# agent-charon/MinGraph-UNet

Hardware: AMD Instinct MI355X
Metric: segmented Mpix/sec, full MinGraph-UNet forward (U-Net + patch-graph GAT), 512x512 batch (higher is better)
Workload: dtype f32

## Files before the change

### mingraph-unet_amd/csrc/asm/gen_wino_cp.py

```python
#!/usr/bin/env python3
import sys

def vr(b, n=1):
    return f"v{b}" if n == 1 else f"v[{b}:{b + n - 1}]"

CFG = {"ntb": 2, "nc": None}
def NTB(): return CFG["ntb"]
def ACC(jj, nt, mi): return ((jj * 2 + nt) * 2 + mi) * 16 if CFG["ntb"] == 2 else (jj * 2 + mi) * 16
def WN(c, jj, p): return 64 + ((c * 2 + jj) * 3 + p) * 4
def HSET(setn, i): return (232 if setn == 0 else 160) + i * 4
def BX(jj, nt, p): return 128 + ((jj * 2 + nt) * 3 + p) * 4
def PC(slot, p): return 176 + (slot * 3 + p) * 4
def RAW(hf, k): return 200 + (hf * 4 + k) * 4
def HREG(i): return 232 + i * 4
VA, VB = 244, 245
VHST = [246, 247, 248]
VHOFF = [249, 250, 251]
VLANE16 = 252
VTID = 253
VT0, VT1 = 230, 231
def VMASK(): return 254 if CFG["ntb"] == 2 else 172
def VSGN(): return 255 if CFG["ntb"] == 2 else 173

S_IN, S_WU, S_OUT, S_SCALE, S_SHIFT, S_POOL = 4, 6, 8, 10, 12, 14
S_H, S_W, S_LDIN, S_LDOUT, S_LDPOOL, S_NC, S_RELU, S_TX, S_TY, S_TOTAL, S_PPB, S_NGROUPS = 16, 17, 18, 19, 20, 21, 22, 23, 24, 25, 26, 27
S_NITEMS, S_PERXCD, S_MGNG, S_MGTX, S_MGTXTY, S_PAD = 28, 29, 30, 31, 32, 33
S_NBLOCK, S_PBEGIN, S_NPATCH, S_LC, S_LP, S_PI, S_C, S_LC64 = 34, 35, 36, 37, 38, 39, 40, 41
S_N64X4 = 42
S_SUMOFF = 43
S_INR = 44
S_UR = 48
S_SGN, S_W1, S_MASK, S_PERM, S_NTSTRIDE, S_TXTY, S_IMGB, S_OOB = 52, 53, 54, 55, 56, 57, 58, 59
S_T = [60, 61, 62, 63, 64, 65, 66, 67]
S_WI, S_JP = 68, 69
S_P, S_IMG, S_REM, S_PY, S_PX, S_Y0, S_X0 = 70, 71, 72, 73, 74, 75, 72
S_X0 = 88
S_M = 76
S_WO = [[78, 79], [90, 91]]
S_OUTR = 80
S_POOLR = 84
S_OUTIMGB = 89
S_SCR = 92
S_SHR = 96
S_LD4, S_SW4 = 100, 101

S1F, S2F, S3F = 17 * 20, 20, 17 * 20 + 20
BUFX = 0x20000
RAWB = 8192 * 4
ZBIAS = 57472

out = []
def E(s=""): out.append("\t" + s if s and not s.endswith(":") else s)
def L(s): out.append(s + ":")
_lbl = [0]
def newlabel(p="L"):
    _lbl[0] += 1
    return f".{p}_{_lbl[0]}"


def divmod_magic(n, d, mg, q, r, t0, t1):
    E(f"s_mul_hi_u32 s{q}, s{n}, s{mg}")
    E(f"s_mul_i32 s{t0}, s{q}, s{d}")
    E(f"s_sub_u32 s{r}, s{n}, s{t0}")
    E(f"s_add_u32 s{t0}, s{q}, 1")
    E(f"s_sub_u32 s{t1}, s{r}, s{d}")
    E(f"s_cmp_ge_u32 s{r}, s{d}")
    E(f"s_cselect_b32 s{q}, s{t0}, s{q}")
    E(f"s_cselect_b32 s{r}, s{t1}, s{r}")


def patch_coords(p):
    divmod_magic(p, S_TXTY, S_MGTXTY, S_IMG, S_REM, S_T[6], S_T[7])
    divmod_magic(S_REM, S_TX, S_MGTX, S_PY, S_PX, S_T[6], S_T[7])
    E(f"s_lshl_b32 s{S_Y0}, s{S_PY}, 3")
    E(f"s_lshl_b32 s{S_X0}, s{S_PX}, 5")


S_VHST = S_PAD


def setup_load():
    E(f"s_add_u32 s{S_P}, s{S_PBEGIN}, s{S_LP}")
    patch_coords(S_P)
    E(f"s_mul_i32 s{S_T[6]}, s{S_IMG}, s{S_IMGB}")
    E(f"s_mul_hi_u32 s{S_T[7]}, s{S_IMG}, s{S_IMGB}")
    E(f"s_add_u32 s{S_INR}, s{S_IN}, s{S_T[6]}")
    E(f"s_addc_u32 s{S_INR + 1}, s{S_IN + 1}, s{S_T[7]}")
    ledge, lvalu, ldone = newlabel("edge"), newlabel("hofs"), newlabel("hdone")
    E(f"s_add_u32 s{S_M}, s{S_Y0}, 8")
    E(f"s_cmp_eq_u32 s{S_M}, s{S_H}")
    E(f"s_cselect_b32 s{S_M + 1}, 1, 0")
    E(f"s_cmp_eq_u32 s{S_Y0}, 0")
    E(f"s_cselect_b32 s{S_M + 1}, 1, s{S_M + 1}")
    E(f"s_add_u32 s{S_M}, s{S_X0}, 32")
    E(f"s_cmp_eq_u32 s{S_M}, s{S_W}")
    E(f"s_cselect_b32 s{S_M + 1}, 1, s{S_M + 1}")
    E(f"s_cmp_eq_u32 s{S_X0}, 0")
    E(f"s_cselect_b32 s{S_M + 1}, 1, s{S_M + 1}")
    E(f"s_sub_u32 s{S_T[6]}, s{S_Y0}, 1")
    E(f"s_sub_u32 s{S_T[7]}, s{S_X0}, 1")
    E(f"s_cmp_lg_u32 s{S_M + 1}, 0")
    E(f"s_cbranch_scc1 {ledge}")
    E(f"s_mul_i32 s{S_M}, s{S_T[6]}, s{S_W}")
    E(f"s_add_u32 s{S_M}, s{S_M}, s{S_T[7]}")
    E(f"s_mul_i32 s{S_M}, s{S_M}, s{S_LDIN}")
    E(f"s_lshl_b32 s{S_M}, s{S_M}, 2")
    E(f"s_add_u32 s{S_INR}, s{S_INR}, s{S_M}")
    E(f"s_addc_u32 s{S_INR + 1}, s{S_INR + 1}, 0")
    E(f"s_and_b32 s{S_INR + 1}, s{S_INR + 1}, 0xffff")
    E(f"s_cmp_eq_u32 s{S_VHST}, 1")
    E(f"s_cbranch_scc1 {ldone}")
    E(f"s_mov_b32 s{S_T[6]}, 0")
    E(f"s_mov_b32 s{S_T[7]}, 0")
    E(f"s_mov_b32 s{S_VHST}, 1")
    E(f"s_branch {lvalu}")
    L(ledge)
    E(f"s_and_b32 s{S_INR + 1}, s{S_INR + 1}, 0xffff")
    E(f"s_mov_b32 s{S_VHST}, 0")
    L(lvalu)
    for i in range(3):
        d = VHOFF[i]
        E(f"v_lshrrev_b32_e32 v{VT0}, 2, v{VTID}")
        if i:
            E(f"v_add_u32_e32 v{VT0}, {128 * i}, v{VT0}")
        E(f"v_mul_u32_u24_e32 v{VT1}, 0x788, v{VT0}")
        E(f"v_lshrrev_b32_e32 v{VT1}, 16, v{VT1}")
        E(f"v_mul_u32_u24_e32 v{d}, 34, v{VT1}")
        E(f"v_sub_u32_e32 v{d}, v{VT0}, v{d}")
        E(f"v_cmp_gt_u32_e32 vcc, 0x154, v{VT0}")
        E(f"v_add_u32_e32 v{VT1}, s{S_T[6]}, v{VT1}")
        E(f"v_add_u32_e32 v{d}, s{S_T[7]}, v{d}")
        E(f"v_cmp_gt_u32_e64 s[{S_M}:{S_M + 1}], s{S_H}, v{VT1}")
        E(f"s_and_b64 vcc, vcc, s[{S_M}:{S_M + 1}]")
        E(f"v_cmp_gt_u32_e64 s[{S_M}:{S_M + 1}], s{S_W}, v{d}")
        E(f"s_and_b64 vcc, vcc, s[{S_M}:{S_M + 1}]")
        E(f"v_mad_u32_u24 v{VT1}, v{VT1}, s{S_W}, v{d}")
        E(f"v_mul_lo_u32 v{VT1}, v{VT1}, s{S_LDIN}")
        E(f"v_and_b32_e32 v{VT0}, 3, v{VTID}")
        E(f"v_lshl_add_u32 v{VT1}, v{VT0}, 2, v{VT1}")
        E(f"v_lshlrev_b32_e32 v{VT1}, 2, v{VT1}")
        E(f"v_mov_b32_e32 v{d}, s{S_OOB}")
        E("s_nop 1")
        E(f"v_cndmask_b32_e32 v{d}, v{d}, v{VT1}, vcc")
    L(ldone)


def halo_loads(setn=0):
    for i in range(3):
        E(f"buffer_load_dwordx4 {vr(HSET(setn, i), 4)}, v{VHOFF[i]}, s[{S_INR}:{S_INR + 3}], s{S_LC64} offen")
    E(f"s_add_u32 s{S_LC}, s{S_LC}, 1")
    E(f"s_cmp_eq_u32 s{S_LC}, s{S_NC}")
    E(f"s_cselect_b32 s{S_LC}, 0, s{S_LC}")
    E(f"s_cmp_eq_u32 s{S_LC}, 0")
    E(f"s_addc_u32 s{S_LP}, s{S_LP}, 0")
    E(f"s_lshl_b32 s{S_LC64}, s{S_LC}, 6")


def halo_stores(setn=0):
    for i in range(3):
# ... 318 lines not shown
            E(f"v_max_f32_e32 v{Z(0, 0, 1) + e}, v{ya1 + e}, v{yb1 + e}")
        for e in range(4):
            E(f"v_max_f32_e32 v{pm + e}, v{pm + e}, v{Z(0, 0, 1) + e}")
        E(f"buffer_store_dwordx4 {vr(pm, 4)}, v{VPOOL}, s[{S_POOLR}:{S_POOLR + 3}], 0 offen offset:{nt * 128}")
        L(lnp)
        E("s_waitcnt lgkmcnt(0)")
        E("s_barrier")


def mfmas_n(jj, mi, slot, c):
    acc = vr(ACC(jj, 0, mi), 16)
    return [f"v_mfma_f32_32x32x16_bf16 {acc}, {vr(PC(slot, pa), 4)}, {vr(WN(c, jj, pb), 4)}, {'0' if (c == 0 and k == 0) else acc}"
            for k, (pa, pb) in enumerate(((2, 0), (0, 2), (1, 1), (1, 0), (0, 1), (0, 0)))]


def emit_step_n(jp, s, c):
    jj, mi = step_jm(s)
    slot = s & 1
    n1, n2 = (s + 1) & 3, (s + 2) & 3
    if s == 2:
        E("s_waitcnt lgkmcnt(0)")
        E("s_barrier")
    E("s_nop 1")
    mf = mfmas_n(jj, mi, slot, c)
    v0 = form_valu(jp, step_jm(n1)[0], slot ^ 1, 0)
    v1 = form_valu(jp, step_jm(n1)[0], slot ^ 1, 1)
    r1 = raw_reads(jp, *step_jm(n1), 1)
    r2 = raw_reads(jp, *step_jm(n2), 0)
    per0, per1 = -(-len(v0) // 2), -(-len(v1) // 3)
    extra = {}
    if s == 0:
        hs = (c + 1) & 1
        E("s_waitcnt vmcnt(3)")
        for i in range(3):
            extra.setdefault(i, []).append(f"ds_write_b128 v{VHST[i]}, {vr(HSET(hs, i), 4)}")
        extra.setdefault(3, []).extend([f"v_xor_b32_e32 v{VHST[i]}, 0x{BUFX:x}, v{VHST[i]}" for i in range(3)])
        for i in range(3):
            extra.setdefault(3 + i, []).append(f"buffer_load_dwordx4 {vr(HSET(hs, i), 4)}, v{VHOFF[i]}, s[{S_INR}:{S_INR + 3}], s{S_LC64} offen")
        extra.setdefault(5, []).extend([
            f"s_add_u32 s{S_LC}, s{S_LC}, 1", f"s_cmp_eq_u32 s{S_LC}, s{S_NC}", f"s_cselect_b32 s{S_LC}, 0, s{S_LC}",
            f"s_cmp_eq_u32 s{S_LC}, 0", f"s_addc_u32 s{S_LP}, s{S_LP}, 0", f"s_lshl_b32 s{S_LC64}, s{S_LC}, 6"])
    def take(lst, n):
        for _ in range(min(n, len(lst))):
            E(lst.pop(0))
    nlds = 0
    for k in range(6):
        E(mf[k])
        for x in extra.get(k, []):
            E(x)
            nlds += x.startswith("ds_")
        if k in (0, 1):
            nlds += min(2, len(r1))
            take(r1, 2)
        if k == 1:
            E(f"s_waitcnt lgkmcnt({nlds})")
        if k in (1, 2):
            take(v0, per0)
        if k == 3:
            E("s_waitcnt lgkmcnt(0)")
            if s == 2:
                E(f"v_xor_b32_e32 v{VA}, 0x{BUFX:x}, v{VA}")
                E(f"v_xor_b32_e32 v{VB}, 0x{BUFX:x}, v{VB}")
        if k in (3, 4):
            take(r2, 2)
        if k >= 3:
            take(v1, per1)
    assert not v0 and not v1 and not r1 and not r2


def emit_chunk_n(jp, c):
    lskip = newlabel("nosetup")
    E(f"s_cmp_lg_u32 s{S_LC}, 0")
    E(f"s_cbranch_scc1 {lskip}")
    E(f"s_cmp_ge_u32 s{S_LP}, s{S_NPATCH}")
    E(f"s_cbranch_scc1 {lskip}")
    setup_load()
    L(lskip)
    E("s_waitcnt lgkmcnt(0)")
    E("s_barrier")
    for s in range(4):
        emit_step_n(jp, s, c)


def emit_epilogue_n(jp):
    CQ, VT = 228, 229
    VZ0, VZ1, VOUT, VPOOL = 188, 189, 190, 191
    e0, e1, e2, e3 = 192, 193, 194, 195
    SC4, SH4 = 196, 212
    TMP = [216 + i for i in range(8)]
    E("s_nop 7")
    E("s_nop 7")
    E("s_nop 7")
    E(f"s_add_u32 s{S_P}, s{S_PBEGIN}, s{S_PI}")
    patch_coords(S_P)
    E(f"s_mul_i32 s{S_T[6]}, s{S_IMG}, s{S_OUTIMGB}")
    E(f"s_mul_hi_u32 s{S_T[7]}, s{S_IMG}, s{S_OUTIMGB}")
    E(f"s_add_u32 s{S_OUTR}, s{S_OUT}, s{S_T[6]}")
    E(f"s_addc_u32 s{S_OUTR + 1}, s{S_OUT + 1}, s{S_T[7]}")
    E(f"s_and_b32 s{S_OUTR + 1}, s{S_OUTR + 1}, 0xffff")
    E(f"s_lshr_b32 s{S_T[4]}, s{S_H}, 1")
    E(f"s_lshr_b32 s{S_T[5]}, s{S_W}, 1")
    E(f"s_mul_i32 s{S_T[4]}, s{S_T[4]}, s{S_T[5]}")
    E(f"s_mul_i32 s{S_T[4]}, s{S_T[4]}, s{S_LDPOOL}")
    E(f"s_lshl_b32 s{S_T[4]}, s{S_T[4]}, 2")
    E(f"s_mov_b32 s{S_POOLR + 2}, s{S_T[4]}")
    E(f"s_mul_i32 s{S_T[6]}, s{S_IMG}, s{S_T[4]}")
    E(f"s_mul_hi_u32 s{S_T[7]}, s{S_IMG}, s{S_T[4]}")
    E(f"s_add_u32 s{S_POOLR}, s{S_POOL}, s{S_T[6]}")
    E(f"s_addc_u32 s{S_POOLR + 1}, s{S_POOL + 1}, s{S_T[7]}")
    E(f"s_and_b32 s{S_POOLR + 1}, s{S_POOLR + 1}, 0xffff")
    E(f"v_and_b32_e32 v{CQ}, 7, v{VTID}")
    E(f"v_lshrrev_b32_e32 v{VT}, 3, v{VTID}")
    E(f"v_lshlrev_b32_e32 v{e0}, 4, v{CQ}")
    for (ptr, rs, reg, dflt) in ((S_SCALE, S_SCR, SC4, "1.0"), (S_SHIFT, S_SHR, SH4, "0")):
        ln, ldn = newlabel("nul"), newlabel("nud")
        E(f"s_cmp_eq_u64 s[{ptr}:{ptr + 1}], 0")
        E(f"s_cbranch_scc1 {ln}")
        E(f"buffer_load_dwordx4 {vr(reg, 4)}, v{e0}, s[{rs}:{rs + 3}], s{S_N64X4} offen")
        E(f"s_branch {ldn}")
        L(ln)
        for e in range(4):
            E(f"v_mov_b32_e32 v{reg + e}, {dflt}")
        L(ldn)
    E(f"v_and_b32_e32 v{e0}, 32, v{VT}")
    E(f"v_and_b32_e32 v{e1}, 3, v{VT}")
    E(f"v_bfe_u32 v{e2}, v{VT}, 3, 2")
    E(f"v_lshl_add_u32 v{e1}, v{e2}, 2, v{e1}")
    E(f"v_lshl_add_u32 v{e0}, v{e1}, 1, v{e0}")
    E(f"v_bfe_u32 v{e2}, v{VT}, 2, 1")
    E(f"v_add_u32_e32 v{e0}, v{e0}, v{e2}")
    E(f"v_lshlrev_b32_e32 v{e0}, 7, v{e0}")
    E(f"v_lshl_add_u32 v{VZ0}, v{CQ}, 4, v{e0}")
    E(f"v_add_u32_e32 v{VZ1}, 0x10000, v{VZ0}")
    E(f"v_lshrrev_b32_e32 v{e1}, 4, v{VT}")
    E(f"v_lshl_add_u32 v{e1}, v{e1}, 1, s{S_Y0}")
    E(f"v_and_b32_e32 v{e2}, 15, v{VT}")
    E(f"v_lshl_add_u32 v{e2}, v{e2}, 1, s{S_X0}")
    E(f"v_mad_u32_u24 v{e3}, v{e1}, s{S_W}, v{e2}")
    E(f"v_mul_lo_u32 v{e3}, v{e3}, s{S_LDOUT}")
    E(f"v_lshl_add_u32 v{e3}, v{CQ}, 2, v{e3}")
    E(f"v_lshlrev_b32_e32 v{VOUT}, 2, v{e3}")
    E(f"v_add_u32_e32 v{VOUT}, s{S_N64X4}, v{VOUT}")
    E(f"v_lshrrev_b32_e32 v{e1}, 1, v{e1}")
    E(f"v_lshrrev_b32_e32 v{e2}, 1, v{e2}")
    E(f"v_mad_u32_u24 v{e3}, v{e1}, s{S_T[5]}, v{e2}")
    E(f"v_mul_lo_u32 v{e3}, v{e3}, s{S_LDPOOL}")
    E(f"v_lshl_add_u32 v{e3}, v{CQ}, 2, v{e3}")
    E(f"v_lshlrev_b32_e32 v{VPOOL}, 2, v{e3}")
    E(f"v_add_u32_e32 v{VPOOL}, s{S_N64X4}, v{VPOOL}")
    E(f"s_lshl_b32 s{S_T[0]}, s{S_WI}, 13")
    if jp:
        E(f"s_add_u32 s{S_T[0]}, s{S_T[0]}, 0x{RAWB:x}")
    E(f"s_lshl_b32 s{S_T[1]}, s{S_WI}, 13")
    E(f"s_add_u32 s{S_T[1]}, s{S_T[1]}, 0x{(2 + jp) * RAWB - ZBIAS:x}")
    E("s_waitcnt lgkmcnt(0)")
    E("s_barrier")
    for q in range(2):
        E(f"s_mov_b32 m0, s{S_T[q]}")
        E("s_nop 0")
        g = 0
        for mi in range(2):
            for r0 in range(0, 16, 4):
                ts = TMP[(g & 1) * 4:(g & 1) * 4 + 4]
                g += 1
                src = []
                for k in (0, 2):
                    m0, m1 = ACC(0, 0, mi) + r0 + k, ACC(1, 0, mi) + r0 + k
                    if jp == 0 and q == 0:
                        E(pk2("add", ts[k], m0, m1))
                        src += [ts[k], ts[k] + 1]
                    elif jp == 0:
                        src += [m1, m1 + 1]
                    elif q == 0:
                        src += [m0, m0 + 1]
                    else:
                        E(pk2("add", ts[k], m0, m1, neg_a=True, neg_b=True))
                        src += [ts[k], ts[k] + 1]
                E("s_nop 0")
                for k in range(4):
                    off = (32 * mi + 2 * (r0 + k)) * 128 + (ZBIAS if q else 0)
                    E(f"ds_write_addtid_b32 v{src[k]} offset:{off}")
    E("s_waitcnt lgkmcnt(0)")
    E("s_barrier")
    zb = [ACC(0, 0, 0), ACC(0, 0, 1), ACC(1, 0, 0), ACC(1, 0, 1)]
    def Z(q, j, i):
        k = (q * 2 + j) * 4 + i
        return zb[k // 4] + (k % 4) * 4
    for q in range(2):
        for j in range(2):
            for i in range(4):
                E(f"ds_read_b128 {vr(Z(q, j, i), 4)}, v{VZ1 if q else VZ0} offset:{j * RAWB + i * 8192}")
    E("s_waitcnt vmcnt(0) lgkmcnt(8)")
    emit_finish_math(Z, 0, SC4, SH4)
    E("s_waitcnt lgkmcnt(0)")
    emit_finish_math(Z, 1, SC4, SH4)
    lnr = newlabel("norelu")
    E(f"s_cmp_eq_u32 s{S_RELU}, 0")
    E(f"s_cbranch_scc1 {lnr}")
    for q in range(2):
        for y in (Z(q, 1, 0), Z(q, 1, 1)):
            for e in range(4):
                E(f"v_max_f32_e32 v{y + e}, 0, v{y + e}")
    L(lnr)
    ya0, yb0, ya1, yb1 = Z(0, 1, 0), Z(0, 1, 1), Z(1, 1, 0), Z(1, 1, 1)
    E(f"buffer_store_dwordx4 {vr(ya0, 4)}, v{VOUT}, s[{S_OUTR}:{S_OUTR + 3}], 0 offen nt")
    E(f"buffer_store_dwordx4 {vr(ya1, 4)}, v{VOUT}, s[{S_OUTR}:{S_OUTR + 3}], s{S_LD4} offen nt")
    E(f"buffer_store_dwordx4 {vr(yb0, 4)}, v{VOUT}, s[{S_OUTR}:{S_OUTR + 3}], s{S_SW4} offen nt")
    E(f"buffer_store_dwordx4 {vr(yb1, 4)}, v{VOUT}, s[{S_OUTR}:{S_OUTR + 3}], s{S_SUMOFF} offen nt")
    lnp = newlabel("nopool")
    E(f"s_cmp_eq_u64 s[{S_POOL}:{S_POOL + 1}], 0")
    E(f"s_cbranch_scc1 {lnp}")
    pm = Z(0, 0, 0)
    for e in range(4):
        E(f"v_max_f32_e32 v{pm + e}, v{ya0 + e}, v{yb0 + e}")
    for e in range(4):
        E(f"v_max_f32_e32 v{Z(0, 0, 1) + e}, v{ya1 + e}, v{yb1 + e}")
    for e in range(4):
        E(f"v_max_f32_e32 v{pm + e}, v{pm + e}, v{Z(0, 0, 1) + e}")
    E(f"buffer_store_dwordx4 {vr(pm, 4)}, v{VPOOL}, s[{S_POOLR}:{S_POOLR + 3}], 0 offen")
    L(lnp)
    E("s_waitcnt lgkmcnt(0)")
    E("s_barrier")


def emit_patch_loop_n(jp):
    lp = newlabel("patch")
    L(lp)
    for c in range(CFG["nc"]):
        emit_chunk_n(jp, c)
    emit_epilogue_n(jp)
    E(f"s_add_u32 s{S_PI}, s{S_PI}, 1")
    E(f"s_cmp_lt_u32 s{S_PI}, s{S_NPATCH}")
    E(f"s_cbranch_scc1 {lp}")
    E(f"s_branch {END_LABEL}")


def emit_patch_loop(jp):
    lp, lc = newlabel("patch"), newlabel("chunk")
    L(lp)
    E(f"s_mov_b32 s{S_C}, 0")
    FIRST_CHUNK[0] = True
    emit_chunk(jp)
    FIRST_CHUNK[0] = False
    E(f"s_mov_b32 s{S_C}, 1")
    L(lc)
    emit_chunk(jp)
    E(f"s_add_u32 s{S_C}, s{S_C}, 1")
    E(f"s_cmp_lt_u32 s{S_C}, s{S_NC}")
    E(f"s_cbranch_scc1 {lc}")
    emit_epilogue(jp)
    E(f"s_add_u32 s{S_PI}, s{S_PI}, 1")
    E(f"s_cmp_lt_u32 s{S_PI}, s{S_NPATCH}")
    E(f"s_cbranch_scc1 {lp}")
    E(f"s_branch {END_LABEL}")


def emit_prologue():
    E("s_load_dwordx16 s[4:19], s[0:1], 0x0")
    E("s_load_dwordx8 s[20:27], s[0:1], 0x40")
    E("s_load_dwordx4 s[28:31], s[0:1], 0x60")
    E("s_load_dwordx2 s[32:33], s[0:1], 0x70")
    E(f"v_mov_b32_e32 v{VTID}, v0")
    E("s_waitcnt lgkmcnt(0)")
    t = S_T
    E(f"s_and_b32 s{t[0]}, s2, 7")
    E(f"s_mul_i32 s{t[0]}, s{t[0]}, s{S_PERXCD}")
    E(f"s_lshr_b32 s{t[1]}, s2, 3")
    E(f"s_add_u32 s{t[0]}, s{t[0]}, s{t[1]}")
    E(f"s_cmp_ge_u32 s{t[0]}, s{S_NITEMS}")
    E(f"s_cbranch_scc1 {END_LABEL}")
    divmod_magic(t[0], S_NGROUPS, S_MGNG, S_NBLOCK, t[1], t[2], t[3])
    E(f"s_mul_i32 s{S_PBEGIN}, s{t[1]}, s{S_PPB}")
    E(f"s_sub_i32 s{t[2]}, s{S_TOTAL}, s{S_PBEGIN}")
    E(f"s_min_i32 s{S_NPATCH}, s{S_PPB}, s{t[2]}")
    E(f"s_cmp_lt_i32 s{S_NPATCH}, 1")
    E(f"s_cbranch_scc1 {END_LABEL}")
    E(f"s_mov_b32 s{S_MASK}, 0xffff0000")
    E(f"s_mov_b32 s{S_PERM}, 0x07060302")
    E(f"s_mov_b32 s{S_OOB}, 0x7fff0000")
    E(f"s_mul_i32 s{S_TXTY}, s{S_TX}, s{S_TY}")
    E(f"s_mul_i32 s{S_IMGB}, s{S_H}, s{S_W}")
    E(f"s_mul_i32 s{S_OUTIMGB}, s{S_IMGB}, s{S_LDOUT}")
    E(f"s_lshl_b32 s{S_OUTIMGB}, s{S_OUTIMGB}, 2")
    E(f"s_mul_i32 s{S_IMGB}, s{S_IMGB}, s{S_LDIN}")
    E(f"s_lshl_b32 s{S_IMGB}, s{S_IMGB}, 2")
    E(f"s_mul_i32 s{S_NTSTRIDE}, s{S_NC}, 0xc000")
    E(f"s_lshl_b32 s{S_N64X4}, s{S_NBLOCK}, {8 if NTB() == 2 else 7}")
    E(f"s_lshl_b32 s{S_LD4}, s{S_LDOUT}, 2")
    E(f"s_mul_i32 s{S_SW4}, s{S_W}, s{S_LD4}")
    E(f"s_add_u32 s{S_SUMOFF}, s{S_SW4}, s{S_LD4}")
    E(f"s_mov_b32 s{S_INR + 2}, s{S_IMGB}")
    E(f"s_mov_b32 s{S_INR + 3}, 0x00020000")
    E(f"s_mov_b32 s{S_OUTR + 2}, s{S_OUTIMGB}")
    E(f"s_mov_b32 s{S_OUTR + 3}, 0x00020000")
    E(f"s_mov_b32 s{S_POOLR + 3}, 0x00020000")
    for (r, p) in ((S_SCR, S_SCALE), (S_SHR, S_SHIFT)):
        E(f"s_mov_b32 s{r}, s{p}")
        E(f"s_and_b32 s{r + 1}, s{p + 1}, 0xffff")
        E(f"s_mov_b32 s{r + 2}, 0x7ffffff0")
        E(f"s_mov_b32 s{r + 3}, 0x00020000")
    E(f"v_lshrrev_b32_e32 v0, 6, v{VTID}")
    E("s_nop 3")
    E("v_readfirstlane_b32 s60, v0")
    E("s_nop 3")
    E(f"s_and_b32 s{S_WI}, s60, 3")
    E(f"s_lshr_b32 s{S_JP}, s60, 2")
    E(f"s_lshl_b32 s61, s{S_WI}, 1")
    E("s_lshr_b32 s62, 0x64, s61")
    E("s_and_b32 s62, s62, 3")
    E("s_lshr_b32 s63, 0xda, s61")
    E("s_and_b32 s63, s63, 3")
    E(f"s_cmp_eq_u32 s{S_WI}, 1")
    E(f"s_cselect_b32 s{S_SGN}, 1.0, -1.0")
    E(f"s_lshl_b32 s64, s{S_NTSTRIDE}, {1 if NTB() == 2 else 0}")
    E(f"s_mul_i32 s65, s{S_NBLOCK}, s64")
    E(f"s_lshl_b32 s66, s{S_WI}, 2")
    E(f"s_lshl_b32 s67, s{S_JP}, 1")
    E("s_add_u32 s66, s66, s67")
    E("s_mul_i32 s66, s66, 0xc00")
    E("s_add_u32 s65, s65, s66")
    E(f"s_add_u32 s{S_UR}, s{S_WU}, s65")
    E(f"s_addc_u32 s{S_UR + 1}, s{S_WU + 1}, 0")
    E(f"s_and_b32 s{S_UR + 1}, s{S_UR + 1}, 0xffff")
    E(f"s_mov_b32 s{S_UR + 2}, s64")
    E(f"s_mov_b32 s{S_UR + 3}, 0x00020000")
    E(f"v_and_b32_e32 v1, 63, v{VTID}")
    E(f"v_lshlrev_b32_e32 v{VLANE16}, 4, v1")
    E("v_and_b32_e32 v2, 31, v1")
    E("v_lshrrev_b32_e32 v3, 5, v1")
    E("v_and_b32_e32 v4, 15, v2")
    E("v_lshrrev_b32_e32 v5, 4, v2")
    E("v_lshlrev_b32_e32 v5, 1, v5")
    E("v_mul_u32_u24_e32 v4, 0x50, v4")
    E("v_lshl_add_u32 v4, v3, 5, v4")
    for (dst, srow) in ((VA, 62), (VB, 63)):
        E(f"v_add_u32_e32 v6, s{srow}, v5")
        E("v_mul_u32_u24_e32 v6, 0xaa0, v6")
        E("v_add_u32_e32 v6, v6, v4")
        E(f"v_add_u32_e32 v{dst}, 0x{BUFX:x}, v6")
    for i in range(3):
        E(f"v_lshrrev_b32_e32 v1, 2, v{VTID}")
        if i:
            E(f"v_add_u32_e32 v1, {128 * i}, v1")
        E("v_mul_u32_u24_e32 v2, 0x788, v1")
        E("v_lshrrev_b32_e32 v2, 16, v2")
        E("v_mul_u32_u24_e32 v3, 34, v2")
        E("v_sub_u32_e32 v3, v1, v3")
        E("v_and_b32_e32 v4, 1, v3")
        E("v_lshl_add_u32 v4, v2, 1, v4")
        E("v_mul_u32_u24_e32 v4, 17, v4")
        E("v_lshrrev_b32_e32 v3, 1, v3")
        E("v_add_u32_e32 v4, v4, v3")
        E("v_mul_u32_u24_e32 v4, 0x50, v4")
        E(f"v_and_b32_e32 v5, 3, v{VTID}")
        E(f"v_lshl_add_u32 v{VHST[i]}, v5, 4, v4")
    E(f"v_mov_b32_e32 v{VMASK()}, s{S_MASK}")
    E(f"v_mov_b32_e32 v{VSGN()}, s{S_SGN}")
    E(f"s_mov_b32 s{S_LC}, 0")
    E(f"s_mov_b32 s{S_LP}, 0")
    E(f"s_mov_b32 s{S_PI}, 0")
    E(f"s_mov_b32 s{S_LC64}, 0")
    if NTB() == 1:
        for c in range(CFG["nc"]):
            for jj in range(2):
                E(f"s_mov_b32 s{S_WO[0][0]}, 0x{c * 0xc000 + jj * 0xc00:x}")
                for pp in range(3):
                    E(f"buffer_load_dwordx4 {vr(WN(c, jj, pp), 4)}, v{VLANE16}, s[{S_UR}:{S_UR + 3}], s{S_WO[0][0]} offen offset:{pp * 1024}")
        setup_load()
        halo_loads(0)
        for i in range(3):
            E(f"v_xor_b32_e32 v{VHST[i]}, 0x{BUFX:x}, v{VHST[i]}")
        E("s_waitcnt vmcnt(0)")
        halo_stores(0)
        for i in range(3):
            E(f"v_xor_b32_e32 v{VHST[i]}, 0x{BUFX:x}, v{VHST[i]}")
        for setn in (1, 0):
            lsk = newlabel("nosetup")
            E(f"s_cmp_lg_u32 s{S_LC}, 0")
            E(f"s_cbranch_scc1 {lsk}")
            E(f"s_cmp_ge_u32 s{S_LP}, s{S_NPATCH}")
            E(f"s_cbranch_scc1 {lsk}")
            setup_load()
            L(lsk)
            halo_loads(setn)
        E("s_waitcnt lgkmcnt(0)")
        E("s_barrier")
        return
    setup_load()
    halo_loads()
    for i in range(3):
        E(f"v_xor_b32_e32 v{VHST[i]}, 0x{BUFX:x}, v{VHST[i]}")
    E("s_waitcnt vmcnt(0)")
    halo_stores()
    for i in range(3):
        E(f"v_xor_b32_e32 v{VHST[i]}, 0x{BUFX:x}, v{VHST[i]}")
    lskip = newlabel("nosetup")
    E(f"s_cmp_lg_u32 s{S_LC}, 0")
    E(f"s_cbranch_scc1 {lskip}")
    E(f"s_cmp_ge_u32 s{S_LP}, s{S_NPATCH}")
    E(f"s_cbranch_scc1 {lskip}")
    setup_load()
    L(lskip)
    halo_loads()
    E(f"s_mov_b32 s{S_WO[0][0]}, 0")
    E(f"s_mov_b32 s{S_WO[0][1]}, s{S_NTSTRIDE}")
    E(f"s_mov_b32 s{S_WO[1][0]}, 0xc00")
    E(f"s_add_u32 s{S_WO[1][1]}, s{S_NTSTRIDE}, 0xc00")
    for jj in range(2):
        for nt in range(2):
            for p in range(3):
                E(weight_load(jj, nt, p))
    E("s_waitcnt lgkmcnt(0)")
    E("s_barrier")


def emit_first_form(jp):
    for r in raw_reads(jp, 0, 0, 0) + raw_reads(jp, 0, 0, 1):
        E(r)
    E("s_waitcnt lgkmcnt(0)")
    for hf in range(2):
        for x in form_valu(jp, 0, 0, hf):
            E(x)
    for r in raw_reads(jp, *step_jm(1), 0):
        E(r)


def emit_kernel(name):
    _lbl[0] += 1000
    end = f".Lend_{name}"
    jp1 = f".Ljp1_{name}"
    fe = f".Lfunc_end_{name}"
    hdr = f"""\t.text
\t.protected\t{name}
\t.globl\t{name}
\t.p2align\t8
\t.type\t{name},@function
{name}:"""
    out.append(hdr)
    global END_LABEL
    END_LABEL = end
    emit_prologue()
    E(f"s_cmp_lg_u32 s{S_JP}, 0")
    E(f"s_cbranch_scc1 {jp1}")
    emit_first_form(0)
    (emit_patch_loop if NTB() == 2 else emit_patch_loop_n)(0)
    L(jp1)
    emit_first_form(1)
    (emit_patch_loop if NTB() == 2 else emit_patch_loop_n)(1)
    L(end)
    E("s_endpgm")
    out.append(f"""\t.section\t.rodata,"a",@progbits
\t.p2align\t6, 0x0
\t.amdhsa_kernel {name}
\t\t.amdhsa_group_segment_fixed_size 163840
\t\t.amdhsa_private_segment_fixed_size 0
\t\t.amdhsa_kernarg_size 120
\t\t.amdhsa_user_sgpr_count 2
\t\t.amdhsa_user_sgpr_dispatch_ptr 0
\t\t.amdhsa_user_sgpr_queue_ptr 0
\t\t.amdhsa_user_sgpr_kernarg_segment_ptr 1
\t\t.amdhsa_user_sgpr_dispatch_id 0
\t\t.amdhsa_user_sgpr_kernarg_preload_length 0
\t\t.amdhsa_user_sgpr_kernarg_preload_offset 0
\t\t.amdhsa_user_sgpr_private_segment_size 0
\t\t.amdhsa_uses_dynamic_stack 0
\t\t.amdhsa_enable_private_segment 0
\t\t.amdhsa_system_sgpr_workgroup_id_x 1
\t\t.amdhsa_system_sgpr_workgroup_id_y 0
\t\t.amdhsa_system_sgpr_workgroup_id_z 0
\t\t.amdhsa_system_sgpr_workgroup_info 0
\t\t.amdhsa_system_vgpr_workitem_id 0
\t\t.amdhsa_next_free_vgpr 256
\t\t.amdhsa_next_free_sgpr 102
\t\t.amdhsa_accum_offset 256
\t\t.amdhsa_reserve_vcc 1
\t\t.amdhsa_float_round_mode_32 0
\t\t.amdhsa_float_round_mode_16_64 0
\t\t.amdhsa_float_denorm_mode_32 3
\t\t.amdhsa_float_denorm_mode_16_64 3
\t\t.amdhsa_dx10_clamp 1
\t\t.amdhsa_ieee_mode 1
\t\t.amdhsa_fp16_overflow 0
\t\t.amdhsa_tg_split 0
\t.end_amdhsa_kernel
\t.text
{fe}:
\t.size\t{name}, {fe}-{name}
""")
    META.append(f"""  - .agpr_count:     0
    .args:
      - .offset:         0
        .size:           120
        .value_kind:     by_value
    .group_segment_fixed_size: 163840
    .kernarg_segment_align: 8
    .kernarg_segment_size: 120
    .max_flat_workgroup_size: 512
    .name:           {name}
    .private_segment_fixed_size: 0
    .sgpr_count:     108
    .sgpr_spill_count: 0
    .symbol:         {name}.kd
    .uniform_work_group_size: 1
    .uses_dynamic_stack: false
    .vgpr_count:     256
    .vgpr_spill_count: 0
    .wavefront_size: 64""")


META = []
END_LABEL = ".Lend"


def main():
    path = sys.argv[1]
    out.append('\t.amdgcn_target "amdgcn-amd-amdhsa--gfx950"')
    CFG.update(ntb=2, nc=None)
    emit_kernel("mgu_wino_cp2_gfx950")
    for nc in (2, 4):
        CFG.update(ntb=1, nc=nc)
        emit_kernel(f"mgu_wino_cp1r{nc}_gfx950")
    out.append("\t.amdgpu_metadata\n---\namdhsa.kernels:")
    out.extend(META)
    out.append("""amdhsa.target:   amdgcn-amd-amdhsa--gfx950
amdhsa.version:
  - 1
  - 2
...

\t.end_amdgpu_metadata
""")
    with open(path, "w") as f:
        f.write("\n".join(out) + "\n")


if __name__ == "__main__":
    main()
```

### mingraph-unet_amd/csrc/asm/lint_wino_asm.py

```python
#!/usr/bin/env python3
import re
import sys


def regs(tok):
    tok = tok.strip().lstrip("-").strip("|")
    m = re.match(r"v\[(\d+):(\d+)\]$", tok)
    if m:
        return set(range(int(m.group(1)), int(m.group(2)) + 1))
    m = re.match(r"v(\d+)$", tok)
    return {int(m.group(1))} if m else set()


def parse(line):
    line = line.split(";")[0].strip()
    if not line or line.endswith(":") or line.startswith("."):
        return None
    parts = line.split(None, 1)
    op = parts[0]
    args = []
    if len(parts) > 1:
        a = re.split(r",\s*", parts[1])
        args = [x.split()[0] if x.split() else x for x in a]
    return op, args, line


def classify(op, args):
    if op.startswith("v_mfma"):
        return regs(args[0]), regs(args[1]) | regs(args[2]) | regs(args[3]), "mfma"
    if op.startswith("ds_read"):
        return regs(args[0]), regs(args[1]), "lds_load"
    if op.startswith("ds_write_addtid"):
        return set(), regs(args[0]), "lds_store_addtid"
    if op.startswith("ds_write"):
        s = set()
        for a in args:
            s |= regs(a)
        return set(), s, "lds_store"
    if op.startswith("buffer_load") or op.startswith("global_load"):
        return regs(args[0]), regs(args[1]), "vm_load"
    if op.startswith("buffer_store") or op.startswith("global_store"):
        return set(), regs(args[0]) | regs(args[1]), "vm_store"
    if op.startswith("v_readfirstlane"):
        return set(), regs(args[1]), "readlane"
    if op.startswith("v_cmp"):
        s = set()
        for a in args:
            s |= regs(a)
        return set(), s, "valu"
    if op.startswith("v_"):
        s = set()
        for a in args[1:]:
            s |= regs(a)
        return regs(args[0]), s, "valu"
    return set(), set(), "other"


def kernels(text):
    out, cur, name = {}, None, None
    for ln in text.split("\n"):
        m = re.match(r"^(mgu_\w+):\s*$", ln)
        if m:
            name, cur = m.group(1), []
            out[name] = cur
            continue
        if ln.startswith(".Lfunc_end"):
            cur = None
            continue
        if cur is not None:
            cur.append(ln)
    return out


def loop_bodies(lines):
    lab = {}
    for i, ln in enumerate(lines):
        m = re.match(r"^(\.\w+):", ln)
        if m:
            lab[m.group(1)] = i
    bodies = []
    for i, ln in enumerate(lines):
        m = re.match(r"\s*s_cbranch_scc1\s+(\.\w+)", ln)
        if m and m.group(1) in lab and lab[m.group(1)] < i:
            bodies.append((m.group(1), lines[lab[m.group(1)]:i]))
    return bodies


def replay(stream, errors, where, prime=()):
    vm, lg = [], []
    valu_age = {}
    mfma_age = {}
    prev = None
    m0_fresh = False
    held = {}
    writes = {}

    def age(n):
        for d in (valu_age, mfma_age):
            for r in list(d):
                d[r] += n
                if d[r] > 40:
                    del d[r]

    skip_to = None
    labels = {}
    for i, ln in enumerate(stream):
        m = re.match(r"^(\.\w+):", ln)
        if m:
            labels.setdefault(m.group(1), []).append(i)
    for i, ln in enumerate(stream):
        if skip_to is not None:
            if re.match(r"^" + re.escape(skip_to) + ":", ln):
                skip_to = None
            continue
        p = parse(ln)
        if p is None:
            continue
        op, args, text = p
        if op == "s_branch" and any(j > i for j in labels.get(args[0], [])):
            skip_to = args[0]
            continue
        if op == "s_nop":
            age(int(args[0]) + 1)
            prev = ("nop", set(), text)
            m0_fresh = False
            continue
        if op == "s_waitcnt":
            m = re.search(r"vmcnt\((\d+)\)", text)
            if m:
                del vm[:max(0, len(vm) - int(m.group(1)))]
            m = re.search(r"lgkmcnt\((\d+)\)", text)
            if m:
                del lg[:max(0, len(lg) - int(m.group(1)))]
            age(1)
            prev = ("wait", set(), text)
            continue
        dst, src, kind = classify(op, args)
        touched = dst | src
        for q, nm in ((vm, "buffer load"), (lg, "LDS read")):
            for (d, t) in q:
                if d & src:
                    errors.append(f"{where}: `{text}` reads v{sorted(d & src)[0]} while `{t}` ({nm}) is outstanding")
                if d & dst and kind not in ("vm_load", "lds_load"):
                    errors.append(f"{where}: `{text}` writes v{sorted(d & dst)[0]}, destination of outstanding `{t}`")
        if kind == "mfma":
            for r in src:
                if valu_age.get(r, 99) < 2:
                    errors.append(f"{where}: `{text}` reads v{r} {valu_age[r]} wait state(s) after a VALU write (2 required)")
        else:
            for r in touched if kind in ("valu", "lds_store", "lds_store_addtid", "vm_store", "readlane") else src:
                if r in src and mfma_age.get(r, 99) < 18:
                    errors.append(f"{where}: `{text}` reads MFMA result v{r} after {mfma_age[r]} wait states (18 required)")
        if kind == "valu" and prev and prev[0] in ("lds_store", "vm_store") and len(prev[1]) >= 4 and (dst & prev[1]):
            errors.append(f"{where}: `{text}` overwrites store data of the previous instruction `{prev[2]}`")
        if kind == "lds_store_addtid" and m0_fresh:
            errors.append(f"{where}: `{text}` directly behind the write of M0")
        if kind == "readlane" and any(valu_age.get(r, 99) < 1 for r in src):
            errors.append(f"{where}: `{text}` directly behind the VALU write of its source")
        if op in ("v_add_f32_e32", "v_sub_f32_e32"):
            hs = [held.get(r) for a in args[1:3] for r in sorted(regs(a))]
            if len(hs) == 2 and any(h and h[0] == "sum" for h in hs):
                if hs[0] and hs[1] and hs[0] != hs[1]:
                    o = hs[1] if hs[0][0] == "sum" else hs[0]
                    why = f"holds what `{o[1]}` wrote" if o[0] == "other" else \
                          "holds an LDS read, not an inner sum" if o[0] == "lds" else "holds an inner sum of another read base"
                    errors.append(f"{where}: `{text}` combines an inner sum with a register that {why}")
        age(1)
        if kind == "valu":
            for r in dst:
                valu_age[r] = 0
                mfma_age.pop(r, None)
        if kind == "mfma":
            for r in dst:
                mfma_age[r] = 0
                valu_age.pop(r, None)
        if kind == "lds_load":
            ver = min(writes.get(r, 0) for r in src) if src else 0
            for r in dst:
                held[r] = ("lds", ver)
        elif op == "v_fmac_f32_e32":
            for r in dst:
                h = held.get(r, ("",))
                held[r] = ("sum", h[1] if h[0] == "lds" else None)
        else:
            for r in dst:
                held[r] = ("other", text)
        for r in dst:
            writes[r] = writes.get(r, 0) + 1
        if kind == "vm_load":
            vm.append((dst, text))
        elif kind == "vm_store":
            vm.append((set(), text))
        elif kind == "lds_load":
            lg.append((dst, text))
        elif kind in ("lds_store", "lds_store_addtid"):
            lg.append((set(), text))
        m0_fresh = op == "s_mov_b32" and args and args[0] == "m0"
        data = set()
        if kind in ("lds_store", "vm_store"):
            data = regs(args[1]) if kind == "lds_store" else regs(args[0])
        prev = (kind, data, text)


def check(text):
    errors = []
    ks = kernels(text)
    for name, lines in ks.items():
        replay(lines, errors, f"{name} (straight line)")
        for lab, body in loop_bodies(lines):
            replay(body * 3, errors, f"{name} loop {lab}")
    return errors, len(ks)


if __name__ == "__main__":
    errs, n = check(open(sys.argv[1]).read())
    for e in errs[:40]:
        print(e)
    print(f"{n} kernels, {len(errs)} finding(s)")
    sys.exit(1 if errs else 0)
```

### mingraph-unet_amd/csrc/common.h

```cpp
#pragma once
#include <hip/hip_runtime.h>
#include <stdint.h>

#include "device.h"

namespace mgu {

inline int grid_for(int64_t work, int threads, int cap) {
  int64_t b = (work + threads - 1) / threads;
  if (b < 1) b = 1;
  if (b > cap) b = cap;
  return (int)b;
}
inline bool aligned16(const void* p) { return ((uintptr_t)p & 15) == 0; }

struct Tuning {
  bool first_mfma = true;
  bool use_wino = true;
  int wino_prec = 1;
  bool convt_frag = true;
  bool wino_cp = true;
  int wino_ppb_cap = 32;
  bool wgrad_halo = true;
  bool wino_wgrad = true;
  bool convt_dgrad_x3 = true;
  bool wgrad_x3 = true;
  bool wgrad_thin = true;
  bool wino_dgrad = true;
  bool gat_fused = true;
  bool wino_asm = true;
};
const Tuning& default_tuning();
hipError_t ensure_dyn_lds(const void* func, size_t bytes, bool (&done)[64]);

struct IgemmDesc {
  const Tuning* tn;
  const float* in;
  const float* w;
  const float* wu;
  const float* scale;
  const float* shift;
  float* out;
  int M;
  int H, W;
  int Cp;
  int ldin;
  int KS;
  int K;
  int Kp;
  int N;
  int ldout;
  int coff;
  int relu;
  int out_mode;
  int ct_cout;
  int Hout, Wout;
  float* pool;
  int ldpool;
  double* stat_slots;
  int split_n;
  float* out2;
  int ld2;
};

inline const Tuning& tun(const IgemmDesc& d) { return d.tn ? *d.tn : default_tuning(); }
enum class ConvKernel {
  None,
  WinoAsmWide, WinoAsmCp1r2, WinoAsmCp1r4,
  WinoCp2, WinoCp1, WinoCp2Stats, WinoCp1Stats,
  WinoF32Wide, WinoF32Narrow,
  WinoX3Wide, WinoX3Narrow,
  HaloF32, HaloBf16Np8, HaloBf16Np4,
  TilesF32, TilesBf16,
  ConvtX3, ConvtBf16f, ConvtX3Dgrad,
};
ConvKernel pick_conv(const IgemmDesc& d, int dtype);
hipError_t launch_conv(const IgemmDesc& d, ConvKernel k, int dtype, hipStream_t s);
inline hipError_t launch_igemm_f32(const IgemmDesc& d, hipStream_t s) { return launch_conv(d, pick_conv(d, 0), 0, s); }
inline hipError_t launch_igemm_bf16(const IgemmDesc& d, hipStream_t s) { return launch_conv(d, pick_conv(d, 1), 1, s); }
const char* conv_kernel_name(ConvKernel k, const IgemmDesc& d);
const char* conv_dgrad_name(ConvKernel k, const IgemmDesc& d);
struct ConvCost {
  double mfma;
  int pipe;
};
ConvCost conv_cost(ConvKernel k, const IgemmDesc& d);
inline bool conv_is_wino(ConvKernel k) { return k >= ConvKernel::WinoAsmWide && k <= ConvKernel::WinoX3Narrow; }
inline bool conv_fuses_pool(ConvKernel k) {
  return conv_is_wino(k) || (k >= ConvKernel::HaloF32 && k <= ConvKernel::HaloBf16Np4);
}
inline bool conv_reads_panel(ConvKernel k) {
  return !conv_is_wino(k) && k != ConvKernel::ConvtX3 && k != ConvKernel::ConvtBf16f && k != ConvKernel::ConvtX3Dgrad;
}
bool wino_layer(const Tuning& t, int KS, int Cp);
bool wino_dgrad_layer(const Tuning& t, int KS, int Cop);
bool convt_x3_layer(const Tuning& t, int Cin, int Cout);
bool convt_x3_dgrad_layer(const Tuning& t, int Cin, int Cout);
bool convt_bf16f_layer(const Tuning& t, int Cin, int Cout);
inline bool wino_wide(const IgemmDesc& d) { return d.N > 32; }
struct WinoPlan {
  int tiles_x, tiles_y, total, nblk, ppb, ngroups, per_xcd;
};
WinoPlan wino_plan(const IgemmDesc& d);
int wino_grid_blocks(const IgemmDesc& d);
size_t convt_x3_floats(int Cin, int Cout);
hipError_t launch_pack_convt_x3(const float* w, float* Wx, int Cin, int Cout, hipStream_t s);
hipError_t launch_convt_x3(const IgemmDesc& d, hipStream_t s);
size_t convt_bf16f_floats(int Cin, int Cout);
hipError_t launch_pack_convt_bf16f(const float* w, float* Wf, int Cin, int Cout, hipStream_t s);
hipError_t launch_convt_bf16f(const IgemmDesc& d, hipStream_t s);
size_t convt_x3_dgrad_floats(int Cin, int Cout);
hipError_t launch_pack_convt_x3_dgrad(const float* w, float* Wx, int Cin, int Cout, hipStream_t s);
hipError_t launch_convt_x3_dgrad(const IgemmDesc& d, hipStream_t s);
hipError_t launch_pack_first_w(const float* w, float* wf, int Cout, int Cin, hipStream_t s);
size_t first_mfma_floats();
bool first_mfma_applicable(int dtype, int Cin, int Cp, int Cout, int ldout, int coff, int64_t H, int64_t W);
hipError_t launch_pack_first_mfma(const float* w, float* wfm, int Cout, int Cin, hipStream_t s);
hipError_t launch_first_mfma(int dtype, const void* in, const float* wfm, const float* scale, const float* shift, void* out, int B, int H,
                             int W, int ldout, int coff, int relu, hipStream_t s);
hipError_t launch_first_mfma_direct(int dtype, const float* x, int64_t sn, int64_t sc, int64_t sh, int64_t sw, int cin, const float* wfm,
                                    const float* scale, const float* shift, void* out, int B, int H, int W, int ldout, int coff, int relu,
                                    hipStream_t s);
bool first_conv_applicable(int dtype, int Cin, int Cp, int Cout, int ldout, int coff);
hipError_t launch_first_conv(int dtype, const void* in, const float* wf, const float* scale, const float* shift, void* out, int B, int H, int W,
                             int Cin, int Cout, int ldout, int coff, int relu, hipStream_t s);
size_t wino_u_floats(int Cout, int Cp);
hipError_t launch_pack_wino_w(const float* w, float* U, int Cout, int Cin, int Cp, int dgrad, int prec, hipStream_t s);
enum { PACK_WINO = 0, PACK_FIRST_W = 1, PACK_CONVT_X3 = 2, PACK_BIAS_TILE = 3, PACK_DGRAD_W = 4, PACK_FIRST_MFMA = 5 };
struct WinoPackItem {
  const float* w;
  float* U;
  int Cout, Cin, Cp, Np, dgrad;
  unsigned blk0;
  int kind;
  int reserved;
};
static_assert(sizeof(WinoPackItem) == 48, "WinoPackItem must have no padding");
constexpr int WINO_PACK_MAX = 64;
struct WinoPackBatch {
  int n, prec;
  unsigned total_blocks;
  WinoPackItem it[WINO_PACK_MAX];
};
bool wino_pack_batch_prepare(WinoPackBatch& b);
hipError_t launch_pack_wino_w_multi(const WinoPackBatch* batch_dev, unsigned total_blocks, hipStream_t s);
hipError_t launch_wino_f32(const IgemmDesc& d, ConvKernel k, hipStream_t s);
hipError_t launch_wino_cp_asm(const IgemmDesc& d, ConvKernel k, hipStream_t s);

struct WgradDesc {
  const Tuning* tn;
  const float* z;
  int ldz, zoff;
  const float* in;
  int ldin, inoff, Cp;
  int KS;
  int M, H, W;
  int Hs, Ws;
  int N, K, Kp;
  float* dw;
  size_t dw_capacity;
  int groups;
  int rows_per_split;
};
inline const Tuning& tun(const WgradDesc& d) { return d.tn ? *d.tn : default_tuning(); }
enum class WgradKernel {
  Thin,
  WinoX3,
  Wino,
  Halo,
  Tiles,
};
WgradKernel pick_wgrad(const WgradDesc& d);
const char* wgrad_kernel_name(WgradKernel k);
struct WgradCost {
  double mfma;
  int pipe;
};
WgradCost wgrad_cost(WgradKernel k, double alg);
hipError_t launch_wgrad_f32(WgradDesc& d, hipStream_t s);
hipError_t launch_wino_wgrad_f32(WgradDesc& d, bool x3, hipStream_t s);
hipError_t launch_wgrad_thin(WgradDesc& d, hipStream_t s);

constexpr int STAT_ROWS = 576;
constexpr int CHAN_REDUCE_ROWS = 512;
size_t chan_reduce_work_bytes(int Cmax);
hipError_t launch_bn_stats(const float* z, int ldz, int64_t M, int C, double* work, double* sums, hipStream_t s);
hipError_t launch_bn_finalize(const double* sum, const double* sumsq, int64_t M, float eps, float momentum,
                              const float* gamma, const float* beta, float* mean, float* invstd, float* scale,
                              float* shift, float* run_mean, float* run_var, int C, hipStream_t s);
hipError_t launch_bn_finalize_slots(double* slots, int nrows, double* sums, int64_t M, float eps, float momentum, const float* gamma,
                                    const float* beta, float* mean, float* invstd, float* scale, float* shift, float* run_mean,
                                    float* run_var, int C, hipStream_t s);
hipError_t launch_bn_apply_relu(const float* z, const float* scale, const float* shift, float* y, int ldy, int64_t M, int C,
                                hipStream_t s);
hipError_t launch_bn_apply_relu_pool(const float* z, const float* scale, const float* shift, float* y, int ldy, float* pooled, int B, int H,
                                     int W, int C, hipStream_t s);
hipError_t launch_bn_bwd_reduce(const float* dy, int lddy, const float* fwd_scale, const float* fwd_shift, const float* z, int ldz,
                                const float* mean, const float* invstd, int64_t M, int C, double* work, double* sums,
                                float* dbeta, float* dgamma, hipStream_t s);
hipError_t launch_bn_bwd_apply(const float* dy, int lddy, const float* fwd_scale, const float* fwd_shift, const float* z, const float* mean,
                               const float* invstd, const float* gamma, const double* sums, int64_t M, int C, float* dz,
                               double* work, float* dbias, hipStream_t s);
hipError_t launch_bn_bwd_apply_deferred(const float* dy, int lddy, const float* fsc, const float* fsh, const float* z, const float* mean,
                                        const float* invstd, const float* gamma, const double* sums, int64_t M, int C, float* dz,
                                        double* work, int* rows, hipStream_t s);
hipError_t launch_colsum(const float* z, int ldz, int64_t M, int C, double* work, float* out, hipStream_t s);
hipError_t launch_maxpool2_bwd_add(const float* y, int ldy, const float* dpool, float* dskip, int ldd, int B, int H, int W,
                                   int C, hipStream_t s);
hipError_t launch_zero_pad_region(float* buf, int ld, int coff, int C, int B, int H, int W, int h2, int w2, hipStream_t s);
hipError_t launch_ce(const float* logits, const int64_t* labels, int64_t M, int C, long long ignore_index, float grad_scale,
                     float* dlogits, int ldd, double* acc, int* err_word, float* loss_out, hipStream_t s);
hipError_t launch_pack_dgrad_w(const float* w, float* wp, int Cout, int Cin, int Cop, int KS, int Kp, hipStream_t s);
hipError_t launch_pack_convt_dgrad_w(const float* w, float* wp, int Cin, int Cout, int Kp, hipStream_t s);
hipError_t launch_unpack_conv_grad(const float* dwp, int groups, size_t panel_stride, float* g, int Cout, int Cin, int Cp, int KS,
                                   int Kp, hipStream_t s, double* fold_slots = nullptr, int fold_rows = 0, int fold_n = 0, float* fold_out = nullptr);
hipError_t launch_unpack_convt_grad(const float* dwp, int groups, size_t panel_stride, float* g, int Cin, int Cout, int Kp, hipStream_t s);
hipError_t launch_sgd(float* p, const float* g, float* buf, int64_t n, float lr, float momentum, float wd, int step, float grad_scale,
                      hipStream_t s);
hipError_t launch_adam(float* p, const float* g, float* m, float* v, int64_t n, float lr, float b1, float b2, float eps,
                       float wd, int step, float grad_scale, hipStream_t s);

hipError_t launch_pack_input(const float* x, void* out, int dtype, int B, int C, int Cp, int H, int W, int64_t sn, int64_t sc,
                             int64_t sh, int64_t sw, hipStream_t s);
hipError_t launch_maxpool2(const void* in, int ldin, void* out, int dtype, int B, int H, int W, int C, hipStream_t s);
bool patch_mean_head_fusable(int dtype, int C, int ncls);
hipError_t launch_patch_mean(const void* feat, int dtype, float* out, int B, int H, int W, int C, int patch, hipStream_t s,
                             const float* head_w = nullptr, const float* head_b = nullptr, float* logits = nullptr, int ncls = 0);
hipError_t launch_pack_conv_w(const float* w_oihw, void* wp, int dtype, int Cout, int Cin, int Cp, int KS, int Kp, hipStream_t s);
hipError_t launch_pack_convt_w(const float* w_iohw, void* wp, int dtype, int Cin, int Cout, int Kp, hipStream_t s);
hipError_t launch_bn_fold(const float* bias, const float* gamma, const float* beta, const float* mean, const float* var,
// ... 25 lines not shown
```

### mingraph-unet_amd/csrc/ctx.h

```cpp
#pragma once
#include <stdarg.h>
#include <stdio.h>
#include <stdlib.h>
#include <string.h>

#include <map>
#include <string>
#include <vector>

#include "../../include/mgunet.h"
#include "common.h"

struct Layer {
  std::string prefix;
  std::string conv;
  std::string bn;
  int Cin = 0, Cp = 0, Cout = 0, KS = 3;
  bool convt = false;
  int K = 0, Kp = 0, N = 0, Np = 0;
  float *wp = nullptr, *scale = nullptr, *shift = nullptr;
  bool first = false;
  bool ctb = false;
  bool ctx3 = false;
  bool wino = false;
  mutable bool wp_dirty = false;
  float* wu = nullptr;
  float* wug = nullptr;
  mutable bool wug_valid = false;
  float* wf = nullptr;
  float* wfm = nullptr;
  float* wxg = nullptr;
  mutable bool wxg_valid = false;
  const float *w_src = nullptr, *b_src = nullptr, *gamma = nullptr, *beta = nullptr;
  float *run_mean = nullptr, *run_var = nullptr;
  int64_t off_w = 0, off_b = 0, off_gamma = 0, off_beta = 0;
  float *mean = nullptr, *invstd = nullptr, *tscale = nullptr, *tshift = nullptr;
  const float* t_in = nullptr;
  int t_ldin = 0;
  float* t_z = nullptr;
  float* t_y = nullptr;
  int t_ldy = 0;
  int t_B = 0, t_H = 0, t_W = 0;
  int level = 0;
};

struct Block {
  int up = -1;
  int conv1 = 0, conv2 = 0;
  int level = 0;
};

struct mgu_ctx {
  int device = 0;
  mgu::Tuning tn;
  std::string err;
  bool configured = false, loaded = false;
  std::vector<mgu::WinoPackBatch> pack_host;
  mgu::WinoPackBatch* pack_dev = nullptr;
  int pack_dev_cap = 0;
  bool want_train = false;
  bool fold_dirty = false;
  int* err_word = nullptr;
  void* redws = nullptr;
  size_t redws_bytes = 0;
  int last_stat_rows = 0;
  void* pm_out = nullptr;
  int pm_patch = 0;
  void* wuws = nullptr;
  size_t wuws_bytes = 0;
  unsigned long long* gmaxbuf = nullptr;
  int gmax_cap = 0;
  unsigned gmax_gen = 0;
  struct mgu_gat_weights* gat_tmp = nullptr;
  void* lossws = nullptr;
  size_t lossws_bytes = 0;
  void* imgws = nullptr;
  size_t imgws_bytes = 0;
  void* ncws = nullptr;
  size_t ncws_bytes = 0;
  void* objws = nullptr;
  size_t objws_bytes = 0;
  int in_ch = 0, ncls = 0, feat = 0, depth = 0, dtype = 0, Cp0 = 0;
  std::vector<Layer> layers;
  std::vector<Block> enc, dec;
  Block bott;
  int head = 0;
  int64_t nparams = 0;
  float* arena = nullptr;
  size_t arena_floats = 0;
  void* ws = nullptr;
  size_t ws_bytes = 0;
  void* gbws = nullptr;
  size_t gbws_bytes = 0;
  void* gws = nullptr;
  size_t gws_bytes = 0;
  void* tws = nullptr;
  size_t tws_bytes = 0;
  bool have_train_fwd = false;
  int tB = 0, tH = 0, tW = 0;
  std::vector<float*> t_cat, t_feat, t_pooled;
  float* t_logits = nullptr;
  void* comm = nullptr;
  int comm_world = 1, comm_rank = 0;
  hipStream_t comm_stream = nullptr;
  hipEvent_t comm_ev[16] = {};
  int comm_ev_next = 0;
  bool prof = false;
  std::vector<hipEvent_t> ev;
  struct ProfRec {
    const char* name;
    double alg, mfma;
    int pipe;
  };
  std::vector<ProfRec> prec;
  int ev_used = 0;
  hipEvent_t ev_total[2] = {nullptr, nullptr};
};

namespace mgud {

inline int rup(int v, int m) { return (v + m - 1) / m * m; }
extern std::string g_create_err;

inline int fail(mgu_ctx* c, int code, const char* fmt, ...) {
  char buf[512];
  va_list ap;
  va_start(ap, fmt);
  vsnprintf(buf, sizeof buf, fmt, ap);
  va_end(ap);
  if (c) c->err = buf; else g_create_err = buf;
  return code;
}

#define HIPCHK(c, call)                                                                                       \
  do {                                                                                                        \
    hipError_t e_ = (call);                                                                                   \
    if (e_ != hipSuccess) return mgud::fail(c, MGU_ERR_HIP, "%s failed: %s", #call, hipGetErrorString(e_));   \
  } while (0)

inline int ensure(mgu_ctx* c, void** p, size_t* have, size_t need) {
  if (*have >= need) return MGU_OK;
  if (*p) {
    HIPCHK(c, hipDeviceSynchronize());
    HIPCHK(c, hipFree(*p));
    *p = nullptr;
    *have = 0;
  }
  hipError_t e = hipMalloc(p, need);
  if (e != hipSuccess) return fail(c, MGU_ERR_NOMEM, "hipMalloc(%zu) failed: %s", need, hipGetErrorString(e));
  *have = need;
// ... 30 lines not shown
  int idx = -1;
  ProfScope(mgu_ctx* c_, hipStream_t s_, const char* name = "conv/GEMM", double alg = 0, double mfma = 0, int pipe = -1) : c(c_), s(s_) {
    if (!c || !c->prof) return;
    if ((size_t)c->ev_used >= c->prec.size()) c->prec.resize(c->ev_used + 1);
    c->prec[c->ev_used] = {name, alg, mfma, pipe};
    if ((size_t)(2 * c->ev_used + 2) > c->ev.size()) {
      hipEvent_t a, b;
      if (hipEventCreate(&a) != hipSuccess || hipEventCreate(&b) != hipSuccess) return;
      c->ev.push_back(a);
      c->ev.push_back(b);
    }
    idx = c->ev_used++;
    (void)hipEventRecord(c->ev[2 * idx], s);
  }
  ~ProfScope() {
    if (idx >= 0) (void)hipEventRecord(c->ev[2 * idx + 1], s);
  }
};

inline void level_dims(int H, int W, int depth, std::vector<int>& hs, std::vector<int>& wsz) {
  hs.assign(depth + 1, 0);
  wsz.assign(depth + 1, 0);
  hs[0] = H;
  wsz[0] = W;
  for (int i = 1; i <= depth; ++i) {
    hs[i] = hs[i - 1] / 2;
    wsz[i] = wsz[i - 1] / 2;
  }
}

inline mgu::IgemmDesc layer_desc(const mgu_ctx* c, const Layer& L, const void* in, int ldin, int B, int H, int W, void* out, int ldout, int coff) {
  mgu::IgemmDesc d;
  memset(&d, 0, sizeof d);
  d.tn = &c->tn;
  d.in = (const float*)in;
  d.w = L.wp, d.wu = L.wu, d.out = (float*)out;
  d.M = B * H * W, d.H = H, d.W = W;
  d.Cp = L.Cp, d.ldin = ldin, d.KS = L.KS, d.K = L.K, d.Kp = L.Kp;
  d.N = L.N, d.ldout = ldout, d.coff = coff;
  d.out_mode = L.convt ? 1 : 0, d.ct_cout = L.Cout;
  return d;
}
inline mgu::IgemmDesc dgrad_desc(const mgu_ctx* c, const Layer& L, const float* dz, int lddz, const float* panel, float* out, int ldout,
                            int Hout = 0, int Wout = 0) {
  const int KS = L.convt ? 2 : L.KS, Cop = rup(L.Cout, 4);
  mgu::IgemmDesc d;
  memset(&d, 0, sizeof d);
  d.tn = &c->tn;
  d.in = dz, d.w = panel, d.out = out;
  d.M = L.t_B * L.t_H * L.t_W, d.H = L.t_H, d.W = L.t_W;
  d.Cp = Cop, d.ldin = lddz, d.KS = KS, d.K = KS * KS * Cop, d.Kp = rup(d.K, 32);
  d.N = L.Cin, d.ldout = ldout, d.Hout = Hout, d.Wout = Wout;
  return d;
}
inline mgu::IgemmDesc gemm_desc(const mgu_ctx* c, const float* in, int M, int K, const float* panel, int Kp, int N, float* out, int ldout,
                           int split_n, float* out2, int ld2) {
  mgu::IgemmDesc d;
  memset(&d, 0, sizeof d);
  d.tn = &c->tn;
  d.in = in, d.w = panel, d.out = out;
  d.M = M, d.H = 1, d.W = M;
  d.Cp = K, d.ldin = K, d.KS = 1, d.K = K, d.Kp = Kp;
  d.N = N, d.ldout = ldout;
  d.split_n = split_n, d.out2 = out2, d.ld2 = ld2;
  return d;
}
inline mgu::WgradDesc wgrad_desc(const mgu_ctx* c, const float* z, int ldz, const float* in, int ldin, int inoff, int Cp, int KS, int B, int H,
                            int W, int Hs, int Ws, int N, float* dw, size_t dw_capacity) {
  mgu::WgradDesc d;
  memset(&d, 0, sizeof d);
  d.tn = &c->tn;
  d.z = z, d.ldz = ldz;
  d.in = in, d.ldin = ldin, d.inoff = inoff, d.Cp = Cp;
  d.KS = KS;
  d.M = B * H * W, d.H = H, d.W = W, d.Hs = Hs, d.Ws = Ws;
  d.N = N, d.K = KS * KS * Cp, d.Kp = rup(d.K, 32);
  d.dw = dw, d.dw_capacity = dw_capacity;
  return d;
}

int run_layer(mgu_ctx* c, const Layer& L, const void* in, int ldin, int B, int H, int W, void* out, int ldout, int coff,
              int relu, const float* scale, const float* shift, int Hout, int Wout, hipStream_t s,
              void* pool = nullptr, int ldpool = 0, bool* pool_fused = nullptr,
              double* stat_slots = nullptr, bool* stat_fused = nullptr);

void gat_destroy(mgu_ctx* c);
int gat_check_layer(mgu_ctx* c, const char* fn, int Fin, int heads, int Fh, bool train = false, int N = 0);
int gmax_buffer(mgu_ctx* c, const int32_t** graph_ptr, int* num_graphs, int heads, unsigned long long** buf, unsigned* gen);
size_t gat_panel_floats(int heads, int Fh, int Fin);
int gat_pack_panel(mgu_ctx* c, const float* W, const float* a, float* panel, int heads, int Fh, int Fin, bool clear, hipStream_t s);
int gat_prologue(mgu_ctx* c, const float* X, int N, int Fin, const float* panel, int heads, int Fh, const int32_t* rowptr, const int32_t* col,
                 int64_t E, const int32_t* gp, int G, float alpha, unsigned long long* gmax, unsigned gen, float* wh, float* st,
                 int32_t* node_graph, float* gm, bool record, hipStream_t s);

int comm_bucket(mgu_ctx* c, float* flat, int64_t lo, int64_t hi, hipStream_t s);
int comm_join(mgu_ctx* c, hipStream_t s);

int repack_weights(mgu_ctx* c, hipStream_t s);
struct BwdScratch {
  float *dwp = nullptr, *dgp = nullptr;
  size_t dwp_floats = 0, dgp_floats = 0;
  double *red = nullptr, *sums = nullptr;
  bool clear = false;
};
int conv_dgrad(mgu_ctx* c, const Layer& L, const float* dz, float* out, int ldout, const BwdScratch& w, bool record, hipStream_t s);
int convt_dgrad(mgu_ctx* c, const Layer& U, const float* dout, int ld_d, int Hout, int Wout, float* out, const BwdScratch& w, bool record,
                hipStream_t s);
int conv_wgrad(mgu_ctx* c, const Layer& L, const float* dz, float* dw, const BwdScratch& w, bool record, hipStream_t s,
               int* fold_rows = nullptr, float* dbias = nullptr);
int convt_wgrad(mgu_ctx* c, const Layer& U, const float* dout, int ld_d, int c_off, int Hout, int Wout, float* dw, const BwdScratch& w,
                hipStream_t s);
size_t train_ws_bytes(const mgu_ctx* c, int B, int H, int W);
int unet_forward_train(mgu_ctx* c, const float* x, int64_t xs_n, int64_t xs_c, int64_t xs_h, int64_t xs_w, int B, int H,
                       int W, float* logits, void* const* cat_dev, void* const* feat_dev, hipStream_t s);

}
```

### mingraph-unet_amd/csrc/igemm.hip

```cpp
#include "common.h"
#include <algorithm>
#include <type_traits>

namespace mgu {


const Tuning& default_tuning() {
  static const Tuning t;
  return t;
}

hipError_t ensure_dyn_lds(const void* func, size_t bytes, bool (&done)[64]) {
  if (bytes <= 65536) return hipSuccess;
  int dev = 0;
  hipError_t e = hipGetDevice(&dev);
  if (e != hipSuccess) return e;
  if (dev < 0 || dev >= 64) return hipFuncSetAttribute(func, hipFuncAttributeMaxDynamicSharedMemorySize, (int)bytes);
  if (done[dev]) return hipSuccess;
  e = hipFuncSetAttribute(func, hipFuncAttributeMaxDynamicSharedMemorySize, (int)bytes);
  if (e == hipSuccess) done[dev] = true;
  return e;
}

template <typename T> struct Elem;
// ... 529 lines not shown
        else store_patch(std::true_type{});
        w0 = interior ? 1 : 0;
      }
      pi += patch_done ? 1 : 0;
      c = patch_done ? 0 : c + 1;
    }
  };
  for (int item = 0; item < nitems; item += NSETH) {
    do_item(Set0{});
    if constexpr (DEEPH) {
      if (item + 1 < nitems) do_item(Set1{});
    }
  }
}

template <typename T, int NP, int TH, int WAVES_M, int WAVES_N, int WMT, int WNT, int TPS>
static hipError_t launch_halo(const IgemmDesc& d, hipStream_t s) {
  constexpr int BN = WAVES_N * WNT * 32;
  constexpr int HP = (TH + 2) * 18;
  const int tiles_x = (d.W + 15) / 16, tiles_y = (d.H + TH - 1) / TH;
  const int B = d.M / (d.H * d.W);
  const int total = tiles_x * tiles_y * B, ntn = (d.N + BN - 1) / BN;
  const int ppb = std::min(std::max((int)(((long)total * ntn) / (256 * 4)), 1), 16);
  dim3 grid((total + ppb - 1) / ppb, ntn);
  size_t lds = (size_t)(HP + 2 * TPS * BN) * (NP * 16 + 16);
  if (NP == 8 && BN % 32 == 0 && (size_t)HP * (NP * 16 + 16) + (size_t)3 * TPS * BN * NP * 16 <= 80 * 1024)
    lds = (size_t)HP * (NP * 16 + 16) + (size_t)3 * TPS * BN * NP * 16;
  static bool attr_done[64] = {};
  hipError_t ae = ensure_dyn_lds(reinterpret_cast<const void*>(&conv3x3_halo_kernel<T, NP, TH, WAVES_M, WAVES_N, WMT, WNT, TPS>), lds, attr_done);
  if (ae != hipSuccess) return ae;
  hipLaunchKernelGGL((conv3x3_halo_kernel<T, NP, TH, WAVES_M, WAVES_N, WMT, WNT, TPS>), grid, dim3(256), lds, s, d, tiles_x,
                     tiles_y, total, ppb);
  return hipGetLastError();
}

template <typename T>
static int halo_np(const IgemmDesc& d) {
  constexpr int VEC = Elem<T>::VEC;
  if (!(d.KS == 3 && d.out_mode == 0 && d.K == 9 * d.Cp && d.ldin == d.Cp && (long)d.H * d.W * d.ldin * (long)sizeof(T) < 0x7fff0000l &&
        (long)d.H * d.W * d.ldout * (long)sizeof(T) < 0x7ffffff0l))
    return 0;
  if (d.Cp % (8 * VEC) == 0) return 8;
  if (sizeof(T) == 2 && d.Cp % (4 * VEC) == 0) return 4;
  return 0;
}

template <typename T, int KS, int OUTMODE, int WAVES_M, int WAVES_N, int WMT, int WNT>
static hipError_t launch_cfg(const IgemmDesc& d, hipStream_t s) {
  constexpr int BM = WAVES_M * WMT * 32;
  constexpr int BN = WAVES_N * WNT * 32;
  dim3 grid((d.M + BM - 1) / BM, (d.N + BN - 1) / BN);
  const size_t lds = (size_t)(BM + BN) * 144;
  hipLaunchKernelGGL((igemm_kernel<T, KS, OUTMODE, WAVES_M, WAVES_N, WMT, WNT>), grid, dim3(256), lds, s, d);
  return hipGetLastError();
}

template <typename T, int KS, int OUTMODE>
static hipError_t launch_tiles(const IgemmDesc& d, hipStream_t s) {
  if (d.N > 64) return launch_cfg<T, KS, OUTMODE, 2, 2, 2, 2>(d, s);
  if (d.N > 32) return launch_cfg<T, KS, OUTMODE, 4, 1, 2, 2>(d, s);
  return launch_cfg<T, KS, OUTMODE, 4, 1, 2, 1>(d, s);
}

template <typename T, int NP>
static hipError_t launch_halo_tiles(const IgemmDesc& d, hipStream_t s) {
  if (d.N > 64) return launch_halo<T, NP, 8, 2, 2, 2, 2, 1>(d, s);
  if (d.N > 32) return launch_halo<T, NP, 16, 4, 1, 2, 2, 1>(d, s);
  return launch_halo<T, NP, 16, 4, 1, 2, 1, 3>(d, s);
}

bool wino_layer(const Tuning& t, int KS, int Cp) { return t.use_wino && KS == 3 && Cp % 16 == 0; }
bool wino_dgrad_layer(const Tuning& t, int KS, int Cop) { return t.wino_dgrad && wino_layer(t, KS, Cop); }
bool convt_x3_layer(const Tuning& t, int Cin, int Cout) { return t.wino_prec != 0 && t.convt_frag && Cin % 32 == 0 && Cout % 32 == 0; }
bool convt_x3_dgrad_layer(const Tuning& t, int Cin, int Cout) {
  return t.wino_prec != 0 && t.convt_dgrad_x3 && Cin % 64 == 0 && Cout % 32 == 0;
}
bool convt_bf16f_layer(const Tuning& t, int Cin, int Cout) { return t.convt_frag && Cin % 64 == 0 && Cout % 32 == 0; }

static bool wino_applicable(const IgemmDesc& d) {
  return wino_layer(tun(d), d.KS, d.Cp) && d.wu && d.out_mode == 0 && d.split_n == 0 && d.K == 9 * d.Cp && (d.ldin & 3) == 0 &&
         (long)d.H * d.W * d.ldin < (1l << 31) && (long)d.H * d.W * d.ldout < (1l << 31);
}

static bool wino_asm_applicable(const IgemmDesc& d) {
  if (!tun(d).wino_asm) return false;
  if (d.stat_slots) return false;
  if (wino_wide(d)) {
    if (d.N & 63) return false;
  } else {
    if (d.N != 32 || !(d.Cp == 32 || d.Cp == 64)) return false;
  }
  if ((d.H & 7) || (d.W & 31) || (d.Cp & 31) || (d.ldin & 3) || (d.ldout & 3) || (d.coff & 3)) return false;
  if (d.pool && ((d.ldpool & 3) || (d.H & 1) || (d.W & 1))) return false;
  if ((long)d.H * d.W * d.ldin * 4 >= 0x7fff0000l || (long)d.H * d.W * d.ldout * 4 >= 0x7fff0000l) return false;
  const WinoPlan p = wino_plan(d);
  if ((long)p.total * p.tiles_x * p.tiles_y >= (1l << 32) || (long)p.ngroups * p.nblk * p.ngroups >= (1l << 32)) return false;
  return true;
}

static bool convt_x3_applicable(const IgemmDesc& d) {
  return convt_x3_layer(tun(d), d.Cp, d.ct_cout) && d.wu && d.KS == 1 && d.K == d.Cp && d.N == 4 * d.ct_cout && (d.ldin & 3) == 0 &&
         !d.scale && !d.relu && !d.split_n && (9l * 128 + 8l * d.Wout) * d.ldout < (1l << 31);
}

static bool convt_bf16f_applicable(const IgemmDesc& d) {
  return convt_bf16f_layer(tun(d), d.Cp, d.ct_cout) && d.wu && d.KS == 1 && d.K == d.Cp && d.N == 4 * d.ct_cout && (d.ldin & 7) == 0 &&
         (d.ldout & 7) == 0 && (d.coff & 7) == 0 && !d.scale && !d.relu && !d.split_n &&
         (9l * 128 + 8l * d.Wout) * d.ldout < (1l << 31);
}

static bool convt_x3_dgrad_applicable(const IgemmDesc& d) {
  return convt_x3_dgrad_layer(tun(d), d.N, d.Cp) && d.KS == 2 && d.wu && d.K == 4 * d.Cp && (d.ldin & 3) == 0 && !d.scale && !d.shift &&
         !d.relu && !d.split_n && !d.pool && (long)d.M * d.ldout < (1l << 31) && (long)d.Hout * d.Wout * d.ldin < (1l << 31);
}

ConvKernel pick_conv(const IgemmDesc& d, int dtype) {
  using K = ConvKernel;
  if (d.M <= 0 || d.N <= 0) return K::None;
  if (dtype == 1) {
    if (d.out_mode == 1) return d.KS != 1 ? K::None : convt_bf16f_applicable(d) ? K::ConvtBf16f : K::TilesBf16;
    const int np = halo_np<__bf16>(d);
    if (np) return np == 8 ? K::HaloBf16Np8 : K::HaloBf16Np4;
    return d.KS == 3 || d.KS == 1 ? K::TilesBf16 : K::None;
  }
  if (d.out_mode == 1) return d.KS != 1 ? K::None : convt_x3_applicable(d) ? K::ConvtX3 : K::TilesF32;
  if (convt_x3_dgrad_applicable(d)) return K::ConvtX3Dgrad;
  if (wino_applicable(d)) {
    const Tuning& t = tun(d);
    const bool wide = wino_wide(d);
    if (!t.wino_prec) return wide ? K::WinoF32Wide : K::WinoF32Narrow;
    if (!t.wino_cp || (long)d.H * d.W * d.ldin * 4 >= 0x7fff0000l) return wide ? K::WinoX3Wide : K::WinoX3Narrow;
    if (d.stat_slots) return wide ? K::WinoCp2Stats : K::WinoCp1Stats;
    if (wino_asm_applicable(d)) return wide ? K::WinoAsmWide : d.Cp == 32 ? K::WinoAsmCp1r2 : K::WinoAsmCp1r4;
    return wide ? K::WinoCp2 : K::WinoCp1;
  }
  if (halo_np<float>(d) == 8) return K::HaloF32;
  return d.KS >= 1 && d.KS <= 3 ? K::TilesF32 : K::None;
}

const char* conv_kernel_name(ConvKernel k, const IgemmDesc& d) {
  switch (k) {
    case ConvKernel::WinoAsmWide: return "mgu_wino_cp2_gfx950 (asm form of wino3x3_cp_kernel<2>)";
    case ConvKernel::WinoAsmCp1r2: return "mgu_wino_cp1r2_gfx950 (asm form of wino3x3_cp_kernel<1>)";
    case ConvKernel::WinoAsmCp1r4: return "mgu_wino_cp1r4_gfx950 (asm form of wino3x3_cp_kernel<1>)";
    case ConvKernel::WinoCp2: case ConvKernel::WinoCp2Stats: return "wino3x3_cp_kernel<2>";
    case ConvKernel::WinoCp1: case ConvKernel::WinoCp1Stats: return "wino3x3_cp_kernel<1>";
    case ConvKernel::WinoF32Wide: return "wino3x3_f32_kernel<0,0>";
    case ConvKernel::WinoF32Narrow: return "wino3x3_f32_kernel<1,0>";
    case ConvKernel::WinoX3Wide: return "wino3x3_f32_kernel<0,1>";
    case ConvKernel::WinoX3Narrow: return "wino3x3_f32_kernel<1,1>";
    case ConvKernel::HaloF32: return "conv3x3_halo_kernel<f32>";
    case ConvKernel::HaloBf16Np8: case ConvKernel::HaloBf16Np4: return "conv3x3_halo_kernel<bf16>";
    case ConvKernel::TilesBf16: return d.out_mode == 1 ? "igemm_kernel<bf16> (ConvTranspose)" : "igemm_kernel<bf16>";
    case ConvKernel::ConvtX3: return "convt2x2_x3_kernel";
    case ConvKernel::ConvtBf16f: return "convt2x2_bf16_kernel";
    case ConvKernel::ConvtX3Dgrad: return "convt2x2_x3_kernel<dgrad>";
    case ConvKernel::TilesF32: case ConvKernel::None: break;
  }
  return d.out_mode == 1 ? "igemm_kernel<f32> (ConvTranspose)" : d.KS == 2 ? "igemm_kernel<f32> (ConvTranspose dgrad)" : "igemm_kernel<f32>";
}

const char* conv_dgrad_name(ConvKernel k, const IgemmDesc& d) {
  switch (k) {
    case ConvKernel::WinoAsmWide: case ConvKernel::WinoCp2: case ConvKernel::WinoCp2Stats: return "wino3x3_cp_kernel<2> (dgrad)";
    case ConvKernel::WinoAsmCp1r2: case ConvKernel::WinoAsmCp1r4: case ConvKernel::WinoCp1: case ConvKernel::WinoCp1Stats:
      return "wino3x3_cp_kernel<1> (dgrad)";
    case ConvKernel::WinoX3Wide: case ConvKernel::WinoX3Narrow: return "wino3x3_f32_kernel<*,1> (dgrad)";
    case ConvKernel::WinoF32Wide: case ConvKernel::WinoF32Narrow: return "wino3x3_f32_kernel<*,0> (dgrad)";
    case ConvKernel::ConvtX3Dgrad: return "convt2x2_x3_kernel (dgrad)";
    default: return d.KS == 2 ? "igemm_kernel<f32> (ConvTranspose dgrad)" : "igemm/halo (dgrad)";
  }
}

ConvCost conv_cost(ConvKernel k, const IgemmDesc& d) {
  const double direct = 2.0 * d.M * (double)d.K * d.N;
  switch (k) {
    case ConvKernel::WinoF32Wide: case ConvKernel::WinoF32Narrow:
      return {2.0 * (d.M / (d.H * d.W)) * ((d.H + 1) / 2) * ((d.W + 1) / 2) * 16.0 * d.Cp * d.N, 0};
    case ConvKernel::ConvtX3: case ConvKernel::ConvtX3Dgrad: return {6.0 * direct, 1};
    case ConvKernel::HaloBf16Np8: case ConvKernel::HaloBf16Np4: case ConvKernel::TilesBf16: case ConvKernel::ConvtBf16f: return {direct, 1};
    case ConvKernel::HaloF32: case ConvKernel::TilesF32: case ConvKernel::None: return {direct, 0};
    default:
      return {2.0 * (d.M / (d.H * d.W)) * ((d.H + 1) / 2) * ((d.W + 1) / 2) * 16.0 * d.Cp * d.N * 6.0, 1};
  }
}

hipError_t launch_conv(const IgemmDesc& d, ConvKernel k, int dtype, hipStream_t s) {
  if (d.M <= 0 || d.N <= 0) return hipSuccess;
  if (dtype == 1) {
    if ((d.Cp & 7) || (d.ldin & 7) || (d.Kp % 64) || d.K > d.Kp || d.split_n) return hipErrorInvalidValue;
  } else {
    if ((d.Cp & 3) || (d.ldin & 3) || (d.Kp % 32) || d.K > d.Kp) return hipErrorInvalidValue;
  }
  switch (k) {
    case ConvKernel::WinoAsmWide: case ConvKernel::WinoAsmCp1r2: case ConvKernel::WinoAsmCp1r4: return launch_wino_cp_asm(d, k, s);
    case ConvKernel::WinoCp2: case ConvKernel::WinoCp1: case ConvKernel::WinoCp2Stats: case ConvKernel::WinoCp1Stats:
    case ConvKernel::WinoF32Wide: case ConvKernel::WinoF32Narrow: case ConvKernel::WinoX3Wide: case ConvKernel::WinoX3Narrow:
      return launch_wino_f32(d, k, s);
    case ConvKernel::HaloF32: return launch_halo_tiles<float, 8>(d, s);
    case ConvKernel::HaloBf16Np8: return launch_halo_tiles<__bf16, 8>(d, s);
    case ConvKernel::HaloBf16Np4: return launch_halo_tiles<__bf16, 4>(d, s);
    case ConvKernel::TilesF32:
      if (d.out_mode == 1) return launch_tiles<float, 1, 1>(d, s);
      if (d.KS == 3) return launch_tiles<float, 3, 0>(d, s);
      if (d.KS == 1) return launch_tiles<float, 1, 0>(d, s);
      return launch_tiles<float, 2, 0>(d, s);
    case ConvKernel::TilesBf16:
      if (d.out_mode == 1) return launch_tiles<__bf16, 1, 1>(d, s);
      if (d.KS == 3) return launch_tiles<__bf16, 3, 0>(d, s);
      return launch_tiles<__bf16, 1, 0>(d, s);
    case ConvKernel::ConvtX3: return launch_convt_x3(d, s);
    case ConvKernel::ConvtBf16f: return launch_convt_bf16f(d, s);
    case ConvKernel::ConvtX3Dgrad: return launch_convt_x3_dgrad(d, s);
    case ConvKernel::None: break;
  }
  return hipErrorInvalidValue;
}

}
```

### mingraph-unet_amd/csrc/mgunet_api.hip

```cpp
#include "ctx.h"

#include <algorithm>

using namespace mgu;
using namespace mgud;

namespace mgud {
std::string g_create_err;
}

namespace {

struct WsPlan {
  size_t xin, tmp, bott, total;
  std::vector<size_t> pooled;
};

WsPlan plan_ws(const mgu_ctx* c, int B, int H, int W) {
  std::vector<int> hs, wsz;
  level_dims(H, W, c->depth, hs, wsz);
  auto out = [&](const Block& b, int l) { return (size_t)B * hs[l] * wsz[l] * c->layers[b.conv2].Cout; };
  WsPlan p;
  Carve k;
  const size_t es = c->dtype == MGU_DTYPE_BF16 ? 2 : 4;
  p.xin = k.take((size_t)B * H * W * c->Cp0 * es);
  size_t tmax = out(c->bott, c->bott.level);
  for (const Block& b : c->enc) tmax = std::max(tmax, out(b, b.level));
  p.tmp = k.take(tmax * es);
  for (const Block& b : c->enc) p.pooled.push_back(k.take(out(b, b.level + 1) * es));
  p.bott = k.take(out(c->bott, c->bott.level) * es);
  p.total = k.off;
  return p;
}

template <class F>
void weight_forms(const mgu_ctx* c, Layer& L, F form) {
  const int dtype = c->dtype;
  L.wino = dtype == MGU_DTYPE_F32 && !L.convt && wino_layer(c->tn, L.KS, L.Cp);
  L.ctx3 = dtype == MGU_DTYPE_F32 && L.convt && convt_x3_layer(c->tn, L.Cin, L.Cout);
  L.ctb = dtype == MGU_DTYPE_BF16 && L.convt && convt_bf16f_layer(c->tn, L.Cin, L.Cout);
  L.first = !L.convt && L.KS == 3 && first_conv_applicable(dtype, L.Cin, L.Cp, L.Cout, 8, 0);
  form(L.wp, (size_t)L.Np * L.Kp);
  form(L.scale, (size_t)L.Np);
  form(L.shift, (size_t)L.Np);
  if (L.wino) form(L.wu, wino_u_floats(L.Cout, L.Cp));
  if (L.wino && rup(L.Cout, 4) % 16 == 0) form(L.wug, wino_u_floats(L.Cin, rup(L.Cout, 4)));
  if (L.ctx3) form(L.wu, convt_x3_floats(L.Cin, L.Cout));
  if (L.ctb) form(L.wu, convt_bf16f_floats(L.Cin, L.Cout));
  if (L.ctx3) form(L.wxg, convt_x3_dgrad_floats(L.Cin, L.Cout));
  if (dtype == MGU_DTYPE_F32 && !L.convt && L.bn.empty())
    form(L.wxg, (size_t)rup(L.Cin, 128) * rup(L.KS * L.KS * rup(L.Cout, 4), 32));
  if (L.first) form(L.wf, 9 * 4 * (size_t)L.Cout);
  if (L.first) form(L.wfm, first_mfma_floats());
  if (!L.bn.empty()) {
    form(L.mean, (size_t)L.Np);
    form(L.invstd, (size_t)L.Np);
    form(L.tscale, (size_t)L.Np);
    form(L.tshift, (size_t)L.Np);
  }
}

}

extern "C" {

const char* mgu_version(void) { return "mgunet 0.2 (gfx950: fp32 Winograd / bf16 MFMA forward, fp32 training step, GAT, RCCL gradient exchange)"; }

int mgu_create(int device_id, mgu_ctx** out) {
  if (!out) return fail(nullptr, MGU_ERR_INVALID, "out == NULL");
  int n = 0;
  hipError_t e = hipGetDeviceCount(&n);
  if (e != hipSuccess || n <= 0)
    return fail(nullptr, MGU_ERR_HIP, "no HIP device available (%s): libmgunet has no CPU fallback",
                e != hipSuccess ? hipGetErrorString(e) : "device count 0");
  if (device_id < 0 || device_id >= n) return fail(nullptr, MGU_ERR_INVALID, "device %d out of range [0,%d)", device_id, n);
  e = hipSetDevice(device_id);
  if (e != hipSuccess) return fail(nullptr, MGU_ERR_HIP, "hipSetDevice: %s", hipGetErrorString(e));
  mgu_ctx* c = new mgu_ctx();
  c->device = device_id;
  auto flag = [](const char* name) { const char* v = getenv(name); return v && v[0] == '1'; };
  auto num = [](const char* name, int dflt) { const char* v = getenv(name); return v && v[0] ? atoi(v) : dflt; };
  Tuning& t = c->tn;
  t.first_mfma = !flag("MGU_NO_FIRST_MFMA");
  t.use_wino = !flag("MGU_NO_WINOGRAD");
  t.wino_prec = num("MGU_WINO_PREC", t.wino_prec) ? 1 : 0;
  t.wino_cp = !flag("MGU_NO_WINO_CP");
  t.convt_frag = !flag("MGU_NO_CONVT_FRAG");
  t.wino_ppb_cap = std::max(1, num("MGU_WINO_PPB_CAP", 32));
  t.wgrad_halo = !flag("MGU_NO_WGRAD_HALO");
  t.wino_wgrad = !flag("MGU_NO_WINO_WGRAD");
  t.wgrad_x3 = !flag("MGU_NO_WGRAD_X3");
  t.convt_dgrad_x3 = !flag("MGU_NO_CONVT_DGRAD_X3");
  t.wgrad_thin = !flag("MGU_NO_THIN_WGRAD");
  t.wino_dgrad = !flag("MGU_NO_WINO_DGRAD");
  t.gat_fused = !flag("MGU_NO_GAT_FUSED");
  t.wino_asm = num("MGU_WINO_ASM", 1) > 0;
  *out = c;
  return MGU_OK;
}

void mgu_destroy(mgu_ctx* c) {
  if (!c) return;
  (void)hipSetDevice(c->device);
  (void)hipDeviceSynchronize();
  (void)mgu_comm_destroy(c);
  if (c->arena) (void)hipFree(c->arena);
  if (c->ws) (void)hipFree(c->ws);
  if (c->gws) (void)hipFree(c->gws);
  if (c->gbws) (void)hipFree(c->gbws);
  if (c->pack_dev) (void)hipFree(c->pack_dev);
  if (c->tws) (void)hipFree(c->tws);
  if (c->redws) (void)hipFree(c->redws);
  if (c->wuws) (void)hipFree(c->wuws);
  if (c->ncws) (void)hipFree(c->ncws);
  if (c->objws) (void)hipFree(c->objws);
  if (c->lossws) (void)hipFree(c->lossws);
  if (c->imgws) (void)hipFree(c->imgws);
  gat_destroy(c);
  if (c->err_word) (void)hipHostFree(c->err_word);
  for (auto e : c->ev) (void)hipEventDestroy(e);
  for (auto e : c->ev_total)
    if (e) (void)hipEventDestroy(e);
  delete c;
}

const char* mgu_last_error(mgu_ctx* c) { return c ? c->err.c_str() : g_create_err.c_str(); }

int mgu_unet_configure(mgu_ctx* c, int in_ch, int ncls, int feat, int depth, int dtype) {
  if (!c) return MGU_ERR_INVALID;
  if (in_ch < 1 || ncls < 1 || feat < 4 || (feat & 3) || depth < 1 || depth > 8)
    return fail(c, MGU_ERR_INVALID, "unsupported UNet(%d,%d,%d,%d): init_features must be a positive multiple of 4, depth 1..8",
                in_ch, ncls, feat, depth);
  if (dtype != MGU_DTYPE_F32 && dtype != MGU_DTYPE_BF16) return fail(c, MGU_ERR_INVALID, "unknown dtype %d", dtype);
  if (dtype == MGU_DTYPE_BF16 && ((feat & 7) || ncls > 4))
    return fail(c, MGU_ERR_INVALID, "bf16 storage needs init_features %% 8 == 0 (16-byte lanes of 8 bf16) and <= 4 classes");
  HIPCHK(c, hipSetDevice(c->device));
  c->in_ch = in_ch, c->ncls = ncls, c->feat = feat, c->depth = depth, c->dtype = dtype;
  c->Cp0 = rup(in_ch, dtype == MGU_DTYPE_BF16 ? 8 : 4);
  c->layers.clear();
  c->enc.clear();
  c->dec.clear();
  auto add = [&](const std::string& prefix, const char* conv, const char* bn, int cin, int cp, int cout, int KS, bool convt, int level) {
    Layer L;
    L.prefix = prefix, L.conv = conv, L.bn = bn;
    L.Cin = cin, L.Cp = cp, L.Cout = cout, L.KS = KS, L.convt = convt, L.level = level;
    c->layers.push_back(L);
    return (int)c->layers.size() - 1;
  };
  auto add_block = [&](const std::string& prefix, int cin, int cp, int cout, int level, int up) {
    Block b;
    b.up = up, b.level = level;
    b.conv1 = add(prefix, "conv1", "bn1", cin, cp, cout, 3, false, level);
    b.conv2 = add(prefix, "conv2", "bn2", cout, cout, cout, 3, false, level);
    return b;
  };
  int cin = in_ch, cp = c->Cp0, f = feat;
  for (int i = 0; i < depth; ++i) {
    c->enc.push_back(add_block("encoder.encoder_blocks." + std::to_string(i) + ".", cin, cp, f, i, -1));
    cin = cp = f;
    f *= 2;
  }
  c->bott = add_block("encoder.bottleneck.", cin, cp, f, depth, -1);
  int prev = f;
  for (int b = 0; b < depth; ++b) {
    const int i = depth - 1 - b, ci = feat << i;
    const std::string prefix = "decoder.decoder_blocks." + std::to_string(b) + ".";
    const int up = add(prefix, "upsample", "", prev, prev, prev / 2, 1, true, i + 1);
    c->dec.push_back(add_block(prefix + "conv_block.", ci + prev / 2, ci + prev / 2, ci, i, up));
    prev = ci;
  }
  c->head = add("decoder.", "final_conv", "", prev, prev, ncls, 1, false, 0);
  for (auto& L : c->layers) {
    L.K = L.KS * L.KS * L.Cp;
    L.Kp = rup(L.K, dtype == MGU_DTYPE_BF16 ? 64 : 32);
    L.N = L.convt ? 4 * L.Cout : L.Cout;
    L.Np = rup(L.N, 128);
  }
  {
    int64_t off = 0;
    auto conv = [&](Layer& L) {
      L.off_w = off, off += (int64_t)L.Cout * L.Cin * L.KS * L.KS * (L.convt ? 4 : 1);
      L.off_b = off, off += L.Cout;
    };
    auto bn = [&](Layer& L) {
      L.off_gamma = off, off += L.Cout;
      L.off_beta = off, off += L.Cout;
    };
    auto block = [&](const Block& b) {
      if (b.up >= 0) conv(c->layers[b.up]);
      conv(c->layers[b.conv1]), conv(c->layers[b.conv2]);
      bn(c->layers[b.conv1]), bn(c->layers[b.conv2]);
// ... 97 lines not shown
  if (!c || !out) return MGU_ERR_INVALID;
  if (!c->configured) return fail(c, MGU_ERR_STATE, "not configured");
  *out = training ? train_ws_bytes(c, B, H, W) : plan_ws(c, B, H, W).total;
  return MGU_OK;
}

int mgu_unet_reserve(mgu_ctx* c, int B, int H, int W, int training) {
  size_t need = 0;
  int rc = mgu_unet_workspace_bytes(c, B, H, W, training, &need);
  if (rc) return rc;
  HIPCHK(c, hipSetDevice(c->device));
  return training ? ensure(c, &c->tws, &c->tws_bytes, need) : ensure(c, &c->ws, &c->ws_bytes, need);
}

}

int mgud::repack_weights(mgu_ctx* c, hipStream_t s) {
  std::vector<WinoPackItem> items;
  for (auto& L : c->layers) {
    const float *w = L.w_src, *b = L.b_src;
    L.wxg_valid = false;
    if (L.convt) {
      L.wp_dirty = L.ctx3;
      if (!L.ctx3) HIPCHK(c, launch_pack_convt_w(w, L.wp, c->dtype, L.Cin, L.Cout, L.Kp, s));
      if (L.ctb) HIPCHK(c, launch_pack_convt_bf16f(w, L.wu, L.Cin, L.Cout, s));
      if (L.ctx3) items.push_back(WinoPackItem{w, L.wu, L.Cout, L.Cin, 0, 0, 0, 0, PACK_CONVT_X3});
      items.push_back(WinoPackItem{b, L.shift, L.Cout, 4, 0, 0, 0, 0, PACK_BIAS_TILE});
      if (L.wxg && c->want_train && convt_x3_dgrad_layer(c->tn, L.Cin, L.Cout)) {
        items.push_back(WinoPackItem{w, L.wxg, L.Cout, L.Cin, 0, 0, 1, 0, PACK_CONVT_X3});
        L.wxg_valid = true;
      }
    } else {
      L.wp_dirty = true;
      if (L.wu) items.push_back(WinoPackItem{w, L.wu, L.Cout, L.Cin, L.Cp, 0, 0, 0, PACK_WINO});
      L.wug_valid = false;
      if (L.wug && c->want_train && wino_dgrad_layer(c->tn, L.KS, rup(L.Cout, 4))) {
        items.push_back(WinoPackItem{w, L.wug, L.Cin, L.Cout, rup(L.Cout, 4), 0, 1, 0, PACK_WINO});
        L.wug_valid = true;
      }
      const bool head_kernel = L.bn.empty() && c->ncls <= 4;
      if (!L.wu && !L.first && !head_kernel) {
        HIPCHK(c, launch_pack_conv_w(w, L.wp, c->dtype, L.Cout, L.Cin, L.Cp, L.KS, L.Kp, s));
        L.wp_dirty = false;
      }
      if (L.wf) items.push_back(WinoPackItem{w, L.wf, L.Cout, L.Cin, 0, 0, 0, 0, PACK_FIRST_W});
      if (L.wfm && L.Cout == 32 && L.Cin <= 3) items.push_back(WinoPackItem{w, L.wfm, L.Cout, L.Cin, 0, 0, 0, 0, PACK_FIRST_MFMA});
      if (!L.bn.empty()) c->fold_dirty = true;
      else items.push_back(WinoPackItem{b, L.shift, L.Cout, 1, 0, 0, 0, 0, PACK_BIAS_TILE});
      if (L.bn.empty() && L.wxg && c->want_train) {
        const int Cop = rup(L.Cout, 4);
        items.push_back(WinoPackItem{w, L.wxg, L.Cout, L.Cin, Cop, rup(L.KS * L.KS * Cop, 32), L.KS, 0, PACK_DGRAD_W});
        L.wxg_valid = true;
      }
    }
  }
  std::vector<WinoPackBatch> batches;
  for (size_t i0 = 0; i0 < items.size(); i0 += WINO_PACK_MAX) {
    WinoPackBatch b;
    memset(&b, 0, sizeof b);
    b.n = (int)std::min<size_t>(WINO_PACK_MAX, items.size() - i0), b.prec = c->tn.wino_prec;
    for (int i = 0; i < b.n; ++i) b.it[i] = items[i0 + i];
    if (!wino_pack_batch_prepare(b)) return fail(c, MGU_ERR_STATE, "internal: a Winograd layer is not packable");
    batches.push_back(b);
  }
  const bool same = batches.size() == c->pack_host.size() &&
                    (batches.empty() || memcmp(batches.data(), c->pack_host.data(), batches.size() * sizeof(WinoPackBatch)) == 0);
  if (!same) {
    if ((int)batches.size() > c->pack_dev_cap) {
      if (c->pack_dev) HIPCHK(c, hipFree(c->pack_dev));
      c->pack_dev = nullptr;
      HIPCHK(c, hipMalloc((void**)&c->pack_dev, batches.size() * sizeof(WinoPackBatch)));
      c->pack_dev_cap = (int)batches.size();
    }
    HIPCHK(c, hipStreamSynchronize(s));
    HIPCHK(c, hipMemcpy(c->pack_dev, batches.data(), batches.size() * sizeof(WinoPackBatch), hipMemcpyHostToDevice));
    c->pack_host = batches;
  }
  for (size_t k = 0; k < batches.size(); ++k) HIPCHK(c, launch_pack_wino_w_multi(c->pack_dev + k, batches[k].total_blocks, s));
  return MGU_OK;
}

int mgud::run_layer(mgu_ctx* c, const Layer& L, const void* in_v, int ldin, int B, int H, int W, void* out_v, int ldout,
                    int coff, int relu, const float* scale, const float* shift, int Hout, int Wout, hipStream_t s,
                    void* pool, int ldpool, bool* pool_fused, double* stat_slots, bool* stat_fused) {
  IgemmDesc d = layer_desc(c, L, in_v, ldin, B, H, W, out_v, ldout, coff);
  d.scale = scale, d.shift = shift, d.relu = relu, d.Hout = Hout, d.Wout = Wout;
  if (pool_fused) *pool_fused = false;
  if (stat_fused) *stat_fused = false;
  if (L.wfm && c->tn.first_mfma && ldin == L.Cp && first_mfma_applicable(c->dtype, L.Cin, L.Cp, L.Cout, ldout, coff, H, W)) {
    const double alg = 2.0 * d.M * 9.0 * L.Cin * L.Cout;
    ProfScope ps(c, s, "conv3x3_first_mfma_kernel", alg, 2.0 * d.M * 32.0 * 32.0 * (c->dtype == MGU_DTYPE_F32 ? 6.0 : 3.0), 1);
    HIPCHK(c, launch_first_mfma(c->dtype, in_v, L.wfm, scale, shift, out_v, B, H, W, ldout, coff, relu, s));
    return MGU_OK;
  }
  if (L.wf && ldin == L.Cp && first_conv_applicable(c->dtype, L.Cin, L.Cp, L.Cout, ldout, coff) &&
      (int64_t)B * H * W * std::max(ldout, 8) < (1ll << 31)) {
    ProfScope ps(c, s, "conv3x3_first_kernel", 2.0 * d.M * 9.0 * L.Cin * L.Cout, 0, -1);
    HIPCHK(c, launch_first_conv(c->dtype, in_v, L.wf, scale, shift, out_v, B, H, W, L.Cin, L.Cout, ldout, coff, relu, s));
    return MGU_OK;
  }
  ConvKernel k = pick_conv(d, c->dtype);
  if (stat_slots && conv_is_wino(k) && wino_grid_blocks(d) <= STAT_ROWS) {
    d.stat_slots = stat_slots;
    c->last_stat_rows = wino_grid_blocks(d);
    if (stat_fused) *stat_fused = true;
  }
  if (pool && conv_fuses_pool(k)) {
    d.pool = (float*)pool, d.ldpool = ldpool;
    if (pool_fused) *pool_fused = true;
  }
  if (d.stat_slots || d.pool) k = pick_conv(d, c->dtype);
  if (L.wp_dirty && conv_reads_panel(k)) {
    if (L.convt) HIPCHK(c, launch_pack_convt_w(L.w_src, L.wp, c->dtype, L.Cin, L.Cout, L.Kp, s));
    else HIPCHK(c, launch_pack_conv_w(L.w_src, L.wp, c->dtype, L.Cout, L.Cin, L.Cp, L.KS, L.Kp, s));
    L.wp_dirty = false;
  }
  const double alg = L.convt ? 2.0 * d.M * (double)L.Cin * L.Cout * 4.0 : 2.0 * d.M * (double)L.KS * L.KS * L.Cin * L.Cout;
  const ConvCost cost = conv_cost(k, d);
  ProfScope ps(c, s, conv_kernel_name(k, d), alg, cost.mfma, cost.pipe);
  HIPCHK(c, launch_conv(d, k, c->dtype, s));
  return MGU_OK;
}

static int run_conv(mgu_ctx* c, const Layer& L, const void* in, int ldin, int B, int H, int W, void* out, int ldout,
                    int coff, int relu, int Hout, int Wout, hipStream_t s, void* pool = nullptr, int ldpool = 0,
                    bool* pool_fused = nullptr) {
  return run_layer(c, L, in, ldin, B, H, W, out, ldout, coff, relu, L.bn.empty() ? nullptr : L.scale, L.shift, Hout, Wout, s,
                   pool, ldpool, pool_fused, nullptr, nullptr);
}

extern "C" {

int mgu_unet_forward(mgu_ctx* c, const void* x_dev, int B, int H, int W, int64_t xs_n, int64_t xs_c, int64_t xs_h,
                     int64_t xs_w, void* logits_dev, void* const* cat_dev, void* const* feat_dev, int training,
                     void* hip_stream) {
  if (!c) return MGU_ERR_INVALID;
  if (!c->configured || !c->loaded) return fail(c, MGU_ERR_STATE, "configure + load_weights must precede forward");
  if (!x_dev || !logits_dev || !cat_dev || !feat_dev) return fail(c, MGU_ERR_INVALID, "NULL buffer");
  const int depth = c->depth;
  if (B < 1 || H < (1 << depth) || W < (1 << depth))
    return fail(c, MGU_ERR_INVALID, "input %dx%dx%d too small for depth %d", B, H, W, depth);
  if ((int64_t)B * H * W >= (1ll << 31)) return fail(c, MGU_ERR_INVALID, "B*H*W must be < 2^31");
  for (int i = 0; i < depth; ++i)
    if (!cat_dev[i] || !feat_dev[i]) return fail(c, MGU_ERR_INVALID, "NULL cat/feat buffer %d", i);
  HIPCHK(c, hipSetDevice(c->device));
  hipStream_t s = (hipStream_t)hip_stream;
  if (training && c->dtype != MGU_DTYPE_F32)
    return fail(c, MGU_ERR_STATE, "training runs in fp32 only (bf16 storage is an inference mode)");
  if (training) {
    int rc = unet_forward_train(c, (const float*)x_dev, xs_n, xs_c, xs_h, xs_w, B, H, W, (float*)logits_dev, cat_dev, feat_dev, s);
    if (rc == MGU_OK && c->pm_out) {
      HIPCHK(c, launch_patch_mean(feat_dev[0], 0, (float*)c->pm_out, B, H, W, c->feat, c->pm_patch, s));
      c->pm_out = nullptr;
    }
    return rc;
  }
  const WsPlan plan = plan_ws(c, B, H, W);
  int rc = ensure(c, &c->ws, &c->ws_bytes, plan.total);
  if (rc) return rc;
  if (c->fold_dirty) {
    for (auto& L : c->layers)
      if (!L.bn.empty()) HIPCHK(c, launch_bn_fold(L.b_src, L.gamma, L.beta, L.run_mean, L.run_var, 1e-5f, L.scale, L.shift, L.Cout, s));
    c->fold_dirty = false;
  }
  char* ws = (char*)c->ws;
  const size_t es = c->dtype == MGU_DTYPE_BF16 ? 2 : 4;
  void* xin = ws + plan.xin;
  void* tmp = ws + plan.tmp;
  void* bott = ws + plan.bott;
  std::vector<int> hs, wsz;
  level_dims(H, W, depth, hs, wsz);

  if (c->prof) {
    for (auto& e : c->ev_total)
      if (!e) HIPCHK(c, hipEventCreate(&e));
    HIPCHK(c, hipEventRecord(c->ev_total[0], s));
  }

  for (const Block& b : c->enc) {
    const int i = b.level;
    if (2 * hs[i + 1] != hs[i] || 2 * wsz[i + 1] != wsz[i])
      HIPCHK(c, hipMemsetAsync(cat_dev[i], 0, (size_t)B * hs[i] * wsz[i] * 2 * c->layers[b.conv2].Cout * es, s));
  }

  const Layer& L0 = c->layers[c->enc[0].conv1];
  const bool first_direct = L0.wfm && c->tn.first_mfma && first_mfma_applicable(c->dtype, L0.Cin, L0.Cp, L0.Cout, c->feat, 0, H, W) &&
                            (int64_t)B * H * W < (1ll << 31);
  if (!first_direct) HIPCHK(c, launch_pack_input((const float*)x_dev, xin, c->dtype, B, c->in_ch, c->Cp0, H, W, xs_n, xs_c, xs_h, xs_w, s));

  const void* cur = xin;
  int cur_ld = c->Cp0;
  for (const Block& b : c->enc) {
    const int i = b.level, C = c->layers[b.conv1].Cout;
    if (&b == &c->enc.front() && first_direct) {
      if (c->fold_dirty) return fail(c, MGU_ERR_STATE, "internal: eval scale/shift not folded");
      const double alg = 2.0 * B * H * W * 9.0 * L0.Cin * L0.Cout;
      ProfScope ps(c, s, "conv3x3_first_mfma_kernel", alg, 2.0 * B * H * W * 32.0 * 32.0 * (c->dtype == MGU_DTYPE_F32 ? 6.0 : 3.0), 1);
      HIPCHK(c, launch_first_mfma_direct(c->dtype, (const float*)x_dev, xs_n, xs_c, xs_h, xs_w, c->in_ch, L0.wfm, L0.bn.empty() ? nullptr : L0.scale,
                                         L0.shift, tmp, B, H, W, C, 0, 1, s));
    } else if ((rc = run_conv(c, c->layers[b.conv1], cur, cur_ld, B, hs[i], wsz[i], tmp, C, 0, 1, 0, 0, s))) return rc;
    void* pooled = ws + plan.pooled[i];
    bool fused = false;
    if ((rc = run_conv(c, c->layers[b.conv2], tmp, C, B, hs[i], wsz[i], cat_dev[i], 2 * C, 0, 1, 0, 0, s, pooled, C, &fused))) return rc;
    if (!fused) HIPCHK(c, launch_maxpool2(cat_dev[i], 2 * C, pooled, c->dtype, B, hs[i], wsz[i], C, s));
    cur = pooled;
    cur_ld = C;
  }
  {
    const Block& b = c->bott;
    const int i = b.level, C = c->layers[b.conv1].Cout;
    if ((rc = run_conv(c, c->layers[b.conv1], cur, cur_ld, B, hs[i], wsz[i], tmp, C, 0, 1, 0, 0, s))) return rc;
    if ((rc = run_conv(c, c->layers[b.conv2], tmp, C, B, hs[i], wsz[i], bott, C, 0, 1, 0, 0, s))) return rc;
    cur = bott;
    cur_ld = C;
  }
  for (const Block& b : c->dec) {
    const int i = b.level, C = c->layers[b.conv1].Cout;
    if ((rc = run_conv(c, c->layers[b.up], cur, cur_ld, B, hs[i + 1], wsz[i + 1], cat_dev[i], 2 * C, C, 0, hs[i], wsz[i], s)))
      return rc;
    if ((rc = run_conv(c, c->layers[b.conv1], cat_dev[i], 2 * C, B, hs[i], wsz[i], tmp, C, 0, 1, 0, 0, s))) return rc;
    if ((rc = run_conv(c, c->layers[b.conv2], tmp, C, B, hs[i], wsz[i], feat_dev[i], C, 0, 1, 0, 0, s))) return rc;
    cur = feat_dev[i];
    cur_ld = C;
  }
  const Layer& F = c->layers[c->head];
  {
    const int pm_dtype = c->dtype;
    if (c->pm_out && F.w_src && F.b_src && patch_mean_head_fusable(pm_dtype, F.Cin, c->ncls) && F.Cin <= 256) {
      ProfScope ps(c, s, "patch_mean_kernel (1x1 head + patch means)", 2.0 * B * H * W * F.Cin * c->ncls, 0, -1);
      HIPCHK(c, launch_patch_mean(cur, pm_dtype, (float*)c->pm_out, B, H, W, F.Cin, c->pm_patch, s, F.w_src, F.b_src,
                                  (float*)logits_dev, c->ncls));
      c->pm_out = nullptr;
    } else if (c->ncls <= 4 && F.w_src && F.b_src) {
      ProfScope ps(c, s, "conv1x1_head_kernel", 2.0 * B * H * W * F.Cin * c->ncls, 0, -1);
      HIPCHK(c, launch_conv1x1_head(cur, c->dtype, cur_ld, F.Cin, F.w_src, F.b_src, (float*)logits_dev, c->ncls, c->ncls,
                                    (int64_t)B * H * W, s));
    } else if ((rc = run_conv(c, F, cur, cur_ld, B, H, W, logits_dev, c->ncls, 0, 0, 0, 0, s))) {
      return rc;
    }
  }
  if (c->pm_out) {
    HIPCHK(c, launch_patch_mean(cur, c->dtype, (float*)c->pm_out, B, H, W, F.Cin, c->pm_patch, s));
    c->pm_out = nullptr;
  }
  if (c->prof) HIPCHK(c, hipEventRecord(c->ev_total[1], s));
  return MGU_OK;
}

int mgu_unet_request_patch_mean(mgu_ctx* c, int patch, void* out_dev) {
  if (!c) return MGU_ERR_INVALID;
  if (!c->configured) return fail(c, MGU_ERR_STATE, "not configured");
  if (!out_dev) {
    c->pm_out = nullptr;
    return MGU_OK;
  }
  if (patch < 1) return fail(c, MGU_ERR_INVALID, "bad patch_mean request");
  const int C = c->layers[c->head].Cin, vec = c->dtype == MGU_DTYPE_BF16 ? 8 : 4;
  if ((C % vec) || C > 256) return fail(c, MGU_ERR_INVALID, "patch means need init_features %% %d == 0 and <= 256 (got %d)", vec, C);
  c->pm_patch = patch;
  c->pm_out = out_dev;
  return MGU_OK;
}

struct mgu_conv_weights {
  Layer L;
};

static Layer block_layer(int Cin, int Cout, int ksize, bool convt) {
  Layer L;
  L.Cin = L.Cp = Cin, L.Cout = Cout, L.KS = ksize, L.convt = convt;
  L.K = ksize * ksize * Cin, L.Kp = rup(L.K, 32), L.N = convt ? 4 * Cout : Cout, L.Np = rup(L.N, 128);
  return L;
}

static int conv2d_launch(mgu_ctx* c, const Layer& L, const void* in_dev, int B, int H, int W, const void* bias_dev, const void* scale_dev,
                         const void* shift_dev, int relu, void* out_dev, int ld_out, int c_off, hipStream_t s) {
  IgemmDesc d = layer_desc(c, L, in_dev, L.Cin, B, H, W, out_dev, ld_out, c_off);
  d.relu = relu;
  if (scale_dev && shift_dev) {
    d.scale = (const float*)scale_dev;
    d.shift = (const float*)shift_dev;
  } else if (bias_dev) {
    HIPCHK(c, launch_bias_tile((const float*)bias_dev, L.shift, L.Cout, 1, s));
    d.shift = L.shift;
  }
  const ConvKernel k = pick_conv(d, 0);
  ProfScope ps(c, s, conv_kernel_name(k, d));
  HIPCHK(c, launch_conv(d, k, 0, s));
  return MGU_OK;
}

int mgu_conv2d_prepare(mgu_ctx* c, const void* w_dev, int Cout, int Cin, int ksize, mgu_conv_weights** out, void* hip_stream) {
  if (!c) return MGU_ERR_INVALID;
  if (!w_dev || !out || Cout < 1 || (ksize != 1 && ksize != 3)) return fail(c, MGU_ERR_INVALID, "bad conv2d_prepare args (ksize must be 1 or 3)");
  if (Cin < 4 || (Cin & 3)) return fail(c, MGU_ERR_INVALID, "conv2d needs Cin %% 4 == 0 (got %d)", Cin);
  HIPCHK(c, hipSetDevice(c->device));
  hipStream_t s = (hipStream_t)hip_stream;
  mgu_conv_weights* p = new mgu_conv_weights();
  Layer& L = p->L;
  L = block_layer(Cin, Cout, ksize, false);
  const bool wino = wino_layer(c->tn, ksize, Cin);
  const size_t panel = (size_t)L.Np * L.Kp, total = panel + L.Np + (wino ? wino_u_floats(Cout, Cin) : 0);
  hipError_t e = hipMalloc((void**)&L.wp, total * sizeof(float));
  if (e != hipSuccess) {
    delete p;
    return fail(c, MGU_ERR_NOMEM, "hipMalloc(%zu) failed: %s", total * sizeof(float), hipGetErrorString(e));
  }
  L.shift = L.wp + panel;
  e = hipMemsetAsync(L.wp, 0, (panel + L.Np) * sizeof(float), s);
  if (e == hipSuccess) e = launch_pack_conv_w((const float*)w_dev, L.wp, 0, Cout, Cin, Cin, ksize, L.Kp, s);
  if (e == hipSuccess && wino) {
    L.wu = L.shift + L.Np;
    e = launch_pack_wino_w((const float*)w_dev, L.wu, Cout, Cin, Cin, 0, c->tn.wino_prec, s);
  }
  if (e != hipSuccess) {
    (void)hipFree(L.wp);
    delete p;
    return fail(c, MGU_ERR_HIP, "conv2d_prepare: %s", hipGetErrorString(e));
  }
  *out = p;
  return MGU_OK;
}

void mgu_conv2d_release(mgu_ctx* c, mgu_conv_weights* p) {
// ... 174 lines not shown
```

### mingraph-unet_amd/csrc/wino_asm.hip

```cpp
#include "common.h"
#include <mutex>

extern "C" const unsigned char mgu_wino_cp2_hsaco[];
extern "C" const unsigned mgu_wino_cp2_hsaco_len;

namespace mgu {

namespace {
struct WinoAsmArgs {
  const float* in;
  const void* wu;
  float* out;
  const float* scale;
  const float* shift;
  float* pool;
  int H, W, ldin, ldout;
  int ldpool, nC, relu, tiles_x;
  int tiles_y, total, ppb, ngroups;
  int nitems, per_xcd;
  unsigned mg_ngroups, mg_tx;
  unsigned mg_txty, pad;
};
static_assert(sizeof(WinoAsmArgs) == 120, "kernarg layout of mgu_wino_cp2_gfx950");

unsigned magic(unsigned d) { return d <= 1 ? 0xffffffffu : (unsigned)((1ull << 32) / d); }

const char* const kNames[3] = {"mgu_wino_cp2_gfx950", "mgu_wino_cp1r2_gfx950", "mgu_wino_cp1r4_gfx950"};
std::mutex g_mu;
hipModule_t g_mod[64] = {};
hipFunction_t g_fn[64][3] = {};
}

hipError_t launch_wino_cp_asm(const IgemmDesc& d, ConvKernel kind, hipStream_t s) {
  int dev = 0;
  hipError_t e = hipGetDevice(&dev);
  if (e != hipSuccess) return e;
  if (dev < 0 || dev >= 64) return hipErrorInvalidDevice;
  hipFunction_t fn;
  const int k = kind == ConvKernel::WinoAsmWide ? 0 : kind == ConvKernel::WinoAsmCp1r2 ? 1 : 2;
  {
    std::lock_guard<std::mutex> lk(g_mu);
    if (!g_mod[dev]) {
      e = hipModuleLoadData(&g_mod[dev], mgu_wino_cp2_hsaco);
      if (e != hipSuccess) return e;
    }
    if (!g_fn[dev][k]) {
      e = hipModuleGetFunction(&g_fn[dev][k], g_mod[dev], kNames[k]);
      if (e != hipSuccess) return e;
    }
    fn = g_fn[dev][k];
  }
  const WinoPlan p = wino_plan(d);
  WinoAsmArgs a;
  a.in = d.in, a.wu = d.wu, a.out = d.out + d.coff, a.scale = d.scale, a.shift = d.shift, a.pool = d.pool;
  a.H = d.H, a.W = d.W, a.ldin = d.ldin, a.ldout = d.ldout;
  a.ldpool = d.pool ? d.ldpool : 0, a.nC = d.Cp >> 4, a.relu = d.relu, a.tiles_x = p.tiles_x;
  a.tiles_y = p.tiles_y, a.total = p.total, a.ppb = p.ppb, a.ngroups = p.ngroups;
  a.nitems = p.ngroups * p.nblk, a.per_xcd = p.per_xcd;
  a.mg_ngroups = magic((unsigned)p.ngroups), a.mg_tx = magic((unsigned)p.tiles_x);
  a.mg_txty = magic((unsigned)(p.tiles_x * p.tiles_y)), a.pad = 0;
  size_t sz = sizeof(a);
  void* extra[] = {HIP_LAUNCH_PARAM_BUFFER_POINTER, &a, HIP_LAUNCH_PARAM_BUFFER_SIZE, &sz, HIP_LAUNCH_PARAM_END};
  return hipModuleLaunchKernel(fn, (unsigned)(8 * p.per_xcd), 1, 1, 512, 1, 1, 0, s, nullptr, extra);
}

}
```

### mingraph-unet_amd/csrc/wino_f32.hip

```cpp
#include "common.h"
#include "pack_small.h"
#include <algorithm>
#include <cstdlib>
#include <type_traits>

namespace mgu {



__device__ __forceinline__ float relu_1op(const float x) {
  float r;
  asm("v_max_f32_e32 %0, 0, %1" : "=v"(r) : "v"(x));
  return r;
}

template <int OFF>
__device__ __forceinline__ void lds_store4_addtid(const unsigned m0v, const float a, const float b, const float c, const float e) {
  static_assert(OFF >= 0 && OFF + 768 <= 65535 && (OFF & 3) == 0, "ds_write_addtid_b32 offset is 16 bits");
  asm volatile("s_mov_b32 m0, %4\n\ts_nop 0\n\t"
               "ds_write_addtid_b32 %0 offset:%5\n\t"
               "ds_write_addtid_b32 %1 offset:%6\n\t"
               "ds_write_addtid_b32 %2 offset:%7\n\t"
               "ds_write_addtid_b32 %3 offset:%8"
               :
// ... 535 lines not shown
      for (int k = 0; k < UPT; ++k) {
        const int u = tid + k * 512;
        const int T = u / QPT;
        const float* zp = Zx + T * ZP + cq * 4;
        const f32x4 z0 = *reinterpret_cast<const f32x4*>(zp);
        const f32x4 z1 = *reinterpret_cast<const f32x4*>(zp + 64 * ZP);
        const f32x4 z2 = *reinterpret_cast<const f32x4*>(zp + 128 * ZP);
        const f32x4 z3 = *reinterpret_cast<const f32x4*>(zp + 192 * ZP);
        f32x4 ya = (z0 + z1 + z2) * sc4 + sh4;
        f32x4 yb = (z1 - z2 - z3) * sc4 + sh4;
        if (d.relu) {
#pragma unroll
          for (int e = 0; e < 4; ++e) ya[e] = fmaxf(ya[e], 0.f), yb[e] = fmaxf(yb[e], 0.f);
        }
        const int oy = y0 + 2 * (T >> 4), ox = x0 + 2 * (T & 15) + q;
        if (d.stat_slots) {
          const float ma = (interior || (ox < d.W && oy < d.H)) ? 1.f : 0.f;
          const float mb = (interior || (ox < d.W && oy + 1 < d.H)) ? 1.f : 0.f;
          st1 += ma * ya + mb * yb;
          st2 += ma * ya * ya + mb * yb * yb;
        }
        const unsigned idx = (unsigned)((oy * d.W + ox) * d.ldout + n0);
        if (interior) {
          *reinterpret_cast<f32x4*>(img_out + idx) = ya;
          *reinterpret_cast<f32x4*>(img_out + idx + sW) = yb;
        } else if (ox < d.W) {
#pragma unroll
          for (int e = 0; e < 4; ++e)
            if (n0 + e < d.N) {
              if (oy < d.H) img_out[idx + e] = ya[e];
              if (oy + 1 < d.H) img_out[idx + sW + e] = yb[e];
            }
        }
        if (d.pool) {
          f32x4 m;
#pragma unroll
          for (int e = 0; e < 4; ++e) m[e] = fmaxf(ya[e], yb[e]);
          if (q == 0) {
            pmax[k] = m;
          } else {
#pragma unroll
            for (int e = 0; e < 4; ++e) m[e] = fmaxf(m[e], pmax[k][e]);
            const int py = oy >> 1, px = ox >> 1;
            if (oy + 1 < d.H && ox < d.W) {
              float* pp = pool_out + (size_t)(py * (d.W >> 1) + px) * d.ldpool + n0;
              if (fast_n) {
                *reinterpret_cast<f32x4*>(pp) = m;
              } else {
#pragma unroll
                for (int e = 0; e < 4; ++e)
                  if (n0 + e < d.N) pp[e] = m[e];
              }
            }
          }
        }
      }
      lds_barrier();
    }
#pragma unroll
    for (int j = 0; j < 4; ++j)
#pragma unroll
      for (int mi = 0; mi < MT; ++mi)
#pragma unroll
        for (int r = 0; r < 16; ++r) acc[j][mi][r] = 0.f;
  }
  if (d.stat_slots) {
    float* red = smem;
    lds_barrier();
    *reinterpret_cast<f32x4*>(red + tid * 8) = st1;
    *reinterpret_cast<f32x4*>(red + tid * 8 + 4) = st2;
    lds_barrier();
    if (tid < 8 * QPT) {
      const int which = tid / (4 * QPT), rem = tid - which * 4 * QPT, qd = rem >> 2, e = rem & 3;
      double sum = 0.0;
      for (int k = qd; k < 512; k += QPT) sum += (double)red[k * 8 + which * 4 + e];
      const int n = nblock * NC + qd * 4 + e;
      if (n < d.N) atomicAdd(d.stat_slots + (size_t)(blockIdx.x % STAT_ROWS) * 2 * d.N + which * d.N + n, sum);
    }
  }
}

constexpr int WINO_CP_RAWF = 8192;

template <int NTB, bool STATS, bool DEEP, bool URES = false>
__global__ __launch_bounds__(512) void wino3x3_cp_kernel(const IgemmDesc d, const int tiles_x, const int tiles_y, const int total_patches,
                        const int patches_per_block, const int ngroups, const int nitems, const int per_xcd) {
  constexpr int NWAVES = 8;
  constexpr int MT = 2;
  constexpr int NC = 32 * NTB;
  constexpr int ZP = 32;
  constexpr int RH = 10, RW = 34, HPIX = RH * RW;
  constexpr int PLD = 20;
  constexpr int HSTRIDE = NWAVES * 16;
  constexpr int HR = (HPIX + HSTRIDE - 1) / HSTRIDE;
  constexpr int S1 = 17 * PLD, S2 = PLD, S3 = 17 * PLD + PLD;
  constexpr int RAWF = WINO_CP_RAWF;
  static_assert(RAWF >= HR * HSTRIDE / RW * 34 * PLD + 34 * PLD && RAWF >= 4 * 64 * ZP, "raw buffer too small");
  extern __shared__ __attribute__((aligned(16))) float smem[];
  constexpr int BUFSTEP = 4 * RAWF;

  const int tid = threadIdx.x, lane = tid & 63;
  const int wave = __builtin_amdgcn_readfirstlane(tid >> 6);
  const int wi = wave & 3, jp = wave >> 2;
  const int lr = lane & 31, lh = lane >> 5;
  const int tx = lr & 15, ty = lr >> 4;
  const int item = (int)(blockIdx.x & 7) * per_xcd + (int)(blockIdx.x >> 3);
  if (item >= nitems) return;
  const int nblock = item / ngroups;
  const int p_begin = (item - nblock * ngroups) * patches_per_block;
  const int npatch = min(patches_per_block, total_patches - p_begin);
  if (npatch <= 0) return;
  const int ra = wi == 0 ? 0 : (wi == 2 ? 2 : 1);
  const int rb = wi == 0 ? 2 : (wi == 1 ? 2 : (wi == 2 ? 1 : 3));
  const float sgn = wi == 1 ? 1.f : -1.f;
  int offA[MT], offB[MT];
#pragma unroll
  for (int mi = 0; mi < MT; ++mi) {
    const int rowbase = 2 * (2 * mi + ty);
    offA[mi] = ((rowbase + ra) * 34 + tx) * PLD + lh * 8;
    offB[mi] = ((rowbase + rb) * 34 + tx) * PLD + lh * 8;
  }
  const int nC = d.Cp >> 4;
  const size_t u_base = ((size_t)(nblock * NTB) * nC * 16 + wi * 4 + 2 * jp) * 192 * sizeof(u32x4);
  const size_t u_bytes = (size_t)NTB * nC * 16 * 192 * sizeof(u32x4);
  const auto u_rsrc = __builtin_amdgcn_make_buffer_rsrc(const_cast<char*>(reinterpret_cast<const char*>(d.wu)) + u_base, 0,
                                                         (int)u_bytes, 0x00020000);
  const unsigned nt_stride = (unsigned)nC * 16 * 192 * (unsigned)sizeof(u32x4);
  const unsigned lane16 = (unsigned)lane * 16u;
  const int kq = tid & 3, hp0 = tid >> 2;
  int hoff[HR];
  unsigned hmask = 0u, hmask_next = 0u;
  auto in_rsrc = __builtin_amdgcn_make_buffer_rsrc(const_cast<float*>(d.in), 0, 0x7ffffff0, 0x00020000);
  const int img_bytes = d.H * d.W * d.ldin * (int)sizeof(float);
  auto setup_patch = [&](int p, int& img, int& y0, int& x0) {
    const int py = (p / tiles_x) % tiles_y;
    const int px = p % tiles_x;
    img = p / (tiles_x * tiles_y);
    y0 = py * 8;
    x0 = px * 32;
  };
  auto setup_load = [&](int p) {
    int img, y0, x0;
    setup_patch(p, img, y0, x0);
    in_rsrc = __builtin_amdgcn_make_buffer_rsrc(const_cast<float*>(d.in) + (size_t)img * d.H * d.W * d.ldin, 0, img_bytes, 0x00020000);
    unsigned mk = 0u;
#pragma unroll
    for (int i = 0; i < HR; ++i) {
      const int hp = hp0 + HSTRIDE * i;
      const int r = hp / RW, cc = hp - r * RW;
      const int y = y0 - 1 + r, x = x0 - 1 + cc;
      const bool ok = hp < HPIX && y >= 0 && y < d.H && x >= 0 && x < d.W;
      hoff[i] = (NTB == 1 && !ok) ? 0x7fff0000 : ((ok ? (y * d.W + x) * d.ldin : 0) + kq * 4) * (int)sizeof(float);
      mk |= ok ? (1u << i) : 0u;
    }
    hmask_next = mk;
  };
  constexpr int NSET = DEEP ? 2 : 1;
  f32x4 hreg[NSET][HR];
  unsigned hmask_set[NSET];
  (void)hmask;
  auto load_halo = [&](int c, auto set_c) {
    constexpr int set = decltype(set_c)::value;
    hmask_set[set] = hmask_next;
#pragma unroll
    for (int i = 0; i < HR; ++i)
      hreg[set][i] = __builtin_bit_cast(f32x4, __builtin_amdgcn_raw_buffer_load_b128(in_rsrc, hoff[i], c * 64, 0));
  };
  auto store_halo = [&](float* Hs, auto set_c) {
    constexpr int set = decltype(set_c)::value;
// ... 202 lines not shown
#pragma unroll
    for (int nt = 0; nt < NTB; ++nt) {
      const int n0 = nblock * NC + nt * 32 + cq * 4;
      {
        auto write_shares = [&](auto JP0) {
          constexpr bool jp0 = decltype(JP0)::value;
          auto share = [&](const int q, const int mi, const int r) {
            const float m0 = acc[0][nt][mi][r], m1 = acc[1][nt][mi][r];
            if constexpr (RSC) return q == 0 ? (jp0 ? m0 + m1 : m0) : (jp0 ? m1 : -m0 - m1);
            else return q == 0 ? (jp0 ? m0 + m1 : m0) * scw[nt] + shw[nt] : (jp0 ? m1 : -m0 - m1) * scw[nt] + shw[nt];
          };
          if (!(jp0 && top0)) {
            static_for<0, MT * 4>([&](auto G) {
              constexpr int mi = decltype(G)::value >> 2, r = 4 * (decltype(G)::value & 3);
              lds_store4_addtid<(32 * mi + 2 * r) * ZP * 4>(mz0, share(0, mi, r), share(0, mi, r + 1), share(0, mi, r + 2), share(0, mi, r + 3));
            });
          } else {
            float* const z0p = zreg0 + (wi * 64 + ((et >> 5) & 1)) * ZP + (et & 31);
#pragma unroll
            for (int mi = 0; mi < MT; ++mi)
#pragma unroll
              for (int r = 0; r < 16; ++r) z0p[(32 * mi + 2 * r) * ZP] = share(0, mi, r);
          }
          static_for<0, MT * 4>([&](auto G) {
            constexpr int mi = decltype(G)::value >> 2, r = 4 * (decltype(G)::value & 3);
            lds_store4_addtid<ZBIAS + (32 * mi + 2 * r) * ZP * 4>(mz1, share(1, mi, r), share(1, mi, r + 1), share(1, mi, r + 2), share(1, mi, r + 3));
          });
        };
        if (jp == 0) write_shares(std::true_type{});
        else write_shares(std::false_type{});
      }
      lds_barrier();
      f32x4 ya[2], yb[2];
      f32x4 zs[2][2][4];
#pragma unroll
      for (int q = 0; q < 2; ++q)
#pragma unroll
        for (int j = 0; j < 2; ++j)
#pragma unroll
          for (int i = 0; i < 4; ++i) zs[q][j][i] = *reinterpret_cast<const f32x4*>(zregion(q, j) + (i * 64 + Tslot) * ZP + cq * 4);
      __builtin_amdgcn_sched_barrier(0);
#pragma unroll
      for (int q = 0; q < 2; ++q) {
        const f32x4 z0 = zs[q][0][0] + zs[q][1][0];
        const f32x4 z1 = zs[q][0][1] + zs[q][1][1];
        const f32x4 z2 = zs[q][0][2] + zs[q][1][2];
        const f32x4 z3 = zs[q][0][3] + zs[q][1][3];
        ya[q] = z0 + z1 + z2;
        yb[q] = z1 - z2 - z3;
        if constexpr (RSC) ya[q] = ya[q] * sc4[nt] + sh4[nt], yb[q] = yb[q] * sc4[nt] + sh4[nt];
        if (d.relu) {
#pragma unroll
          for (int e = 0; e < 4; ++e) ya[q][e] = relu_1op(ya[q][e]), yb[q][e] = relu_1op(yb[q][e]);
        }
      }
      const int oy = y0 + 2 * (T >> 4), ox = x0 + 2 * (T & 15);
      if (STATS) {
#pragma unroll
        for (int q = 0; q < 2; ++q) {
          const float ma = (interior || (ox + q < d.W && oy < d.H)) ? 1.f : 0.f;
          const float mb = (interior || (ox + q < d.W && oy + 1 < d.H)) ? 1.f : 0.f;
          st1[nt] += ma * ya[q] + mb * yb[q];
          st2[nt] += ma * ya[q] * ya[q] + mb * yb[q] * yb[q];
        }
      }
      const unsigned idx = (unsigned)((oy * d.W + ox) * d.ldout + n0);
      if (interior) {
        __builtin_nontemporal_store(ya[0], reinterpret_cast<f32x4*>(img_out + idx));
        __builtin_nontemporal_store(ya[1], reinterpret_cast<f32x4*>(img_out + idx + d.ldout));
        __builtin_nontemporal_store(yb[0], reinterpret_cast<f32x4*>(img_out + idx + sW));
        __builtin_nontemporal_store(yb[1], reinterpret_cast<f32x4*>(img_out + idx + sW + d.ldout));
      } else {
#pragma unroll
        for (int q = 0; q < 2; ++q)
          if (ox + q < d.W) {
#pragma unroll
            for (int e = 0; e < 4; ++e)
              if (n0 + e < d.N) {
                if (oy < d.H) img_out[idx + q * d.ldout + e] = ya[q][e];
                if (oy + 1 < d.H) img_out[idx + q * d.ldout + sW + e] = yb[q][e];
              }
          }
      }
      if (d.pool) {
        f32x4 m;
#pragma unroll
        for (int e = 0; e < 4; ++e) m[e] = fmaxf(fmaxf(ya[0][e], yb[0][e]), fmaxf(ya[1][e], yb[1][e]));
        const int py = oy >> 1, px = ox >> 1;
        if (oy + 1 < d.H && ox + 1 < d.W) {
          float* pp = pool_out + (size_t)(py * (d.W >> 1) + px) * d.ldpool + n0;
          if (fast_n) {
            *reinterpret_cast<f32x4*>(pp) = m;
          } else {
#pragma unroll
            for (int e = 0; e < 4; ++e)
              if (n0 + e < d.N) pp[e] = m[e];
          }
        }
      }
      lds_barrier();
    }
#pragma unroll
    for (int jj = 0; jj < 2; ++jj)
#pragma unroll
      for (int nt = 0; nt < NTB; ++nt)
#pragma unroll
        for (int mi = 0; mi < MT; ++mi)
#pragma unroll
          for (int r = 0; r < 16; ++r) acc[jj][nt][mi][r] = 0.f;
  }
  if (STATS) {
    float* red = smem;
    lds_barrier();
#pragma unroll
    for (int nt = 0; nt < NTB; ++nt) {
      *reinterpret_cast<f32x4*>(red + (nt * 512 + tid) * 8) = st1[nt];
      *reinterpret_cast<f32x4*>(red + (nt * 512 + tid) * 8 + 4) = st2[nt];
    }
    lds_barrier();
    if (tid < 64 * NTB) {
      const int nt = tid >> 6, rem = tid & 63, which = rem >> 5, qd = (rem >> 2) & 7, e = rem & 3;
      double sum = 0.0;
      for (int k = qd; k < 512; k += 8) sum += (double)red[(nt * 512 + k) * 8 + which * 4 + e];
      const int n = nblock * NC + nt * 32 + qd * 4 + e;
      if (n < d.N) atomicAdd(d.stat_slots + (size_t)(blockIdx.x % STAT_ROWS) * 2 * d.N + which * d.N + n, sum);
    }
  }
}

WinoPlan wino_plan(const IgemmDesc& d) {
  WinoPlan p;
  p.tiles_x = (d.W + 31) / 32, p.tiles_y = (d.H + 7) / 8;
  const int B = d.M / (d.H * d.W);
  const int nc = wino_wide(d) ? 64 : 32;
  p.total = p.tiles_x * p.tiles_y * B, p.nblk = (d.N + nc - 1) / nc;
  p.ppb = std::min(std::max((int)(((long)p.total * p.nblk) / 256), 1), tun(d).wino_ppb_cap);
  p.ngroups = (p.total + p.ppb - 1) / p.ppb;
  p.per_xcd = (p.ngroups * p.nblk + 7) / 8;
  return p;
}

int wino_grid_blocks(const IgemmDesc& d) { return 8 * wino_plan(d).per_xcd; }

template <int NTB, bool STATS, bool DEEP = false, bool URES = false>
static hipError_t launch_wino_cp(const IgemmDesc& d, hipStream_t s) {
  constexpr int NWAVES = 8;
  const WinoPlan p = wino_plan(d);
  dim3 grid(8 * p.per_xcd, 1);
  if (d.stat_slots && grid.x > (unsigned)STAT_ROWS) return hipErrorInvalidValue;
  const size_t lds = (size_t)(5 * WINO_CP_RAWF) * sizeof(float);
  static bool attr_done[64] = {};
  hipError_t ae = ensure_dyn_lds(reinterpret_cast<const void*>(&wino3x3_cp_kernel<NTB, STATS, DEEP, URES>), lds, attr_done);
  if (ae != hipSuccess) return ae;
  hipLaunchKernelGGL((wino3x3_cp_kernel<NTB, STATS, DEEP, URES>), grid, dim3(64 * NWAVES), lds, s, d, p.tiles_x, p.tiles_y, p.total,
                     p.ppb, p.ngroups, p.ngroups * p.nblk, p.per_xcd);
  return hipGetLastError();
}

template <int MODE, int PREC>
static hipError_t launch_wino_mode(const IgemmDesc& d, hipStream_t s) {
  constexpr int NTB = MODE == 0 ? 2 : 1, NWAVES = 8;
  const WinoPlan p = wino_plan(d);
  dim3 grid(8 * p.per_xcd, 1);
  if (d.stat_slots && grid.x > (unsigned)STAT_ROWS) return hipErrorInvalidValue;
  constexpr int HSTRIDE = NWAVES * 16, HR = (340 + HSTRIDE - 1) / HSTRIDE;
  constexpr int RAWF = HR * HSTRIDE / 34 * 34 * 20 + 34 * 20;
  const size_t lds = (size_t)(2 * RAWF + 4 * 64 * (32 * NTB + 8)) * sizeof(float);
  static bool attr_done[64] = {};
  hipError_t ae = ensure_dyn_lds(reinterpret_cast<const void*>(&wino3x3_f32_kernel<MODE, PREC>), lds, attr_done);
  if (ae != hipSuccess) return ae;
  hipLaunchKernelGGL((wino3x3_f32_kernel<MODE, PREC>), grid, dim3(64 * NWAVES), lds, s, d, p.tiles_x, p.tiles_y, p.total, p.ppb,
                     p.ngroups, p.ngroups * p.nblk, p.per_xcd);
  return hipGetLastError();
}

hipError_t launch_wino_f32(const IgemmDesc& d, ConvKernel k, hipStream_t s) {
  switch (k) {
    case ConvKernel::WinoCp2Stats: return launch_wino_cp<2, true>(d, s);
    case ConvKernel::WinoCp1Stats: return launch_wino_cp<1, true>(d, s);
    case ConvKernel::WinoCp2: return launch_wino_cp<2, false>(d, s);
    case ConvKernel::WinoCp1: {
      const int nC = d.Cp >> 4;
      if (nC & 1) return launch_wino_cp<1, false>(d, s);
      return nC == 2 ? launch_wino_cp<1, false, true, true>(d, s) : launch_wino_cp<1, false, true>(d, s);
    }
    case ConvKernel::WinoX3Wide: return launch_wino_mode<0, 1>(d, s);
    case ConvKernel::WinoX3Narrow: return launch_wino_mode<1, 1>(d, s);
    case ConvKernel::WinoF32Wide: return launch_wino_mode<0, 0>(d, s);
    case ConvKernel::WinoF32Narrow: return launch_wino_mode<1, 0>(d, s);
    default: return hipErrorInvalidValue;
  }
}

}
```

Before: 789.2.

## Fuse 1x1 segmentation head and patch-sum pooling into final Winograd conv epilogue

Adds head-fused variants of the last 3x3 Winograd conv, in both the hand-written gfx950 assembly and the HIP kernel. In the epilogue each wave computes the 1x1 classifier logits with a cross-lane shuffle/DPP reduction and writes per-row partial patch sums for the graph nodes. A small combine kernel then averages those partials into node features. This is meant to avoid re-reading the full-resolution decoder output for a separate head conv and patch-pooling pass. The cost is extra epilogue ALU and LDS-permute work, more register pressure, and added host plumbing for a second asm module and a larger kernarg block.

```diff
diff --git a/mingraph-unet_amd/csrc/asm/gen_wino_cp.py b/mingraph-unet_amd/csrc/asm/gen_wino_cp.py
--- a/mingraph-unet_amd/csrc/asm/gen_wino_cp.py
+++ b/mingraph-unet_amd/csrc/asm/gen_wino_cp.py
@@ -4,8 +4,9 @@
 def vr(b, n=1):
     return f"v{b}" if n == 1 else f"v[{b}:{b + n - 1}]"
 
-CFG = {"ntb": 2, "nc": None}
+CFG = {"ntb": 2, "nc": None, "head": False}
 def NTB(): return CFG["ntb"]
+def HEAD(): return CFG["head"]
 def ACC(jj, nt, mi): return ((jj * 2 + nt) * 2 + mi) * 16 if CFG["ntb"] == 2 else (jj * 2 + mi) * 16
 def WN(c, jj, p): return 64 + ((c * 2 + jj) * 3 + p) * 4
 def HSET(setn, i): return (232 if setn == 0 else 160) + i * 4
@@ -75,6 +76,17 @@
     E(f"s_lshl_b32 s{S_Y0}, s{S_PY}, 3")
     E(f"s_lshl_b32 s{S_X0}, s{S_PX}, 5")
 
+
+def WQ(k, e): return 112 + k * 4 + e
+def BL(k): return 128 + k
+def DL(k, p): return 132 + k * 4 + p
+def SS(j): return 148 + j
+VLG, VPS, VBP16, VBP32 = 156, 157, 158, 159
+S_LOGP = 14
+S_LGR = 84
+S_PSR = 48
+S_NCLS, S_NCLS4, S_WNCLS4, S_LOGIMGB, S_NPW, S_NPIMG, S_NODE0 = 40, 52, 53, 54, 56, 78, 79
+HEAD_KERNARG = 160
 
 S_VHST = S_PAD
 
@@ -559,6 +571,71 @@
         emit_step_n(jp, s, c)
 
 
+def emit_head_math(Y, P, Q, CQ):
+    def fold_add():
+        E("s_waitcnt lgkmcnt(0)")
+        for e in (0, 2):
+            E(pk2("add", P + e, P + e, Q + e))
+    def fold_issue(vb):
+        for e in range(4):
+            E(f"ds_bpermute_b32 v{Q + e}, v{vb}, v{P + e}")
+    for e in (0, 2):
+        E(pk2("add", P + e, Y[0] + e, Y[1] + e))
+    for e in (0, 2):
+        E(pk2("add", Q + e, Y[2] + e, Y[3] + e))
+    for e in (0, 2):
+        E(pk2("add", P + e, P + e, Q + e))
+    E("s_nop 1")
+    for e in range(4):
+        E(f"v_add_f32_dpp v{P + e}, v{P + e}, v{P + e} row_ror:8 row_mask:0xf bank_mask:0xf")
+    fold_issue(VBP16)
+    lst = newlabel("hstore")
+    for k in range(4):
+        if k:
+            E(f"s_cmp_lt_u32 s{S_NCLS}, {k + 1}")
+            E(f"s_cbranch_scc1 {lst}")
+        for p in range(4):
+            E(f"v_fma_f32 v{DL(k, p)}, v{Y[p]}, v{WQ(k, 0)}, v{BL(k)}")
+        for e in range(1, 4):
+            for p in range(4):
+                E(f"v_fmac_f32_e32 v{DL(k, p)}, v{Y[p] + e}, v{WQ(k, e)}")
+        for ctl in ("quad_perm:[1,0,3,2]", "quad_perm:[2,3,0,1]", "row_half_mirror"):
+            for p in range(4):
+                E(f"v_add_f32_dpp v{DL(k, p)}, v{DL(k, p)}, v{DL(k, p)} {ctl} row_mask:0xf bank_mask:0xf")
+        if k == 0:
+            fold_add()
+            fold_issue(VBP32)
+    L(lst)
+    E(f"v_cmp_eq_u32_e32 vcc, 1, v{CQ}")
+    ldone = newlabel("hdone")
+    for n in range(1, 5):
+        lnext = newlabel("hn")
+        if n < 4:
+            E(f"s_cmp_lg_u32 s{S_NCLS}, {n}")
+            E(f"s_cbranch_scc1 {lnext}")
+        for pp in range(2):
+            for k in range(n):
+                E(f"v_cndmask_b32_e32 v{SS(pp * (4 if n == 3 else n) + k)}, v{DL(k, pp)}, v{DL(k, 2 + pp)}, vcc")
+        d = f"v{VLG}, s[{S_LGR}:{S_LGR + 3}], 0 offen"
+        if n == 1:
+            E(f"buffer_store_dwordx2 {vr(SS(0), 2)}, {d}")
+        elif n == 2:
+            E(f"buffer_store_dwordx4 {vr(SS(0), 4)}, {d}")
+        elif n == 3:
+            E(f"buffer_store_dwordx3 {vr(SS(0), 3)}, {d}")
+            E(f"buffer_store_dwordx3 {vr(SS(4), 3)}, {d} offset:12")
+        else:
+            E(f"buffer_store_dwordx4 {vr(SS(0), 4)}, {d}")
+            E(f"buffer_store_dwordx4 {vr(SS(4), 4)}, {d} offset:16")
+        if n < 4:
+            E(f"s_branch {ldone}")
+            L(lnext)
+    L(ldone)
+    fold_add()
+    E("s_nop 0")
+    E(f"buffer_store_dwordx4 {vr(P, 4)}, v{VPS}, s[{S_PSR}:{S_PSR + 3}], 0 offen")
+
+
 def emit_epilogue_n(jp):
     CQ, VT = 228, 229
     VZ0, VZ1, VOUT, VPOOL = 188, 189, 190, 191
@@ -575,17 +652,29 @@
     E(f"s_add_u32 s{S_OUTR}, s{S_OUT}, s{S_T[6]}")
     E(f"s_addc_u32 s{S_OUTR + 1}, s{S_OUT + 1}, s{S_T[7]}")
     E(f"s_and_b32 s{S_OUTR + 1}, s{S_OUTR + 1}, 0xffff")
-    E(f"s_lshr_b32 s{S_T[4]}, s{S_H}, 1")
-    E(f"s_lshr_b32 s{S_T[5]}, s{S_W}, 1")
-    E(f"s_mul_i32 s{S_T[4]}, s{S_T[4]}, s{S_T[5]}")
-    E(f"s_mul_i32 s{S_T[4]}, s{S_T[4]}, s{S_LDPOOL}")
-    E(f"s_lshl_b32 s{S_T[4]}, s{S_T[4]}, 2")
-    E(f"s_mov_b32 s{S_POOLR + 2}, s{S_T[4]}")
-    E(f"s_mul_i32 s{S_T[6]}, s{S_IMG}, s{S_T[4]}")
-    E(f"s_mul_hi_u32 s{S_T[7]}, s{S_IMG}, s{S_T[4]}")
-    E(f"s_add_u32 s{S_POOLR}, s{S_POOL}, s{S_T[6]}")
-    E(f"s_addc_u32 s{S_POOLR + 1}, s{S_POOL + 1}, s{S_T[7]}")
-    E(f"s_and_b32 s{S_POOLR + 1}, s{S_POOLR + 1}, 0xffff")
+    if HEAD():
+        E("; only-head {")
+        E(f"s_mul_i32 s{S_T[6]}, s{S_IMG}, s{S_LOGIMGB}")
+        E(f"s_mul_hi_u32 s{S_T[7]}, s{S_IMG}, s{S_LOGIMGB}")
+        E(f"s_add_u32 s{S_LGR}, s{S_LOGP}, s{S_T[6]}")
+        E(f"s_addc_u32 s{S_LGR + 1}, s{S_LOGP + 1}, s{S_T[7]}")
+        E(f"s_and_b32 s{S_LGR + 1}, s{S_LGR + 1}, 0xffff")
+        E(f"s_mul_i32 s{S_NODE0}, s{S_IMG}, s{S_NPIMG}")
+        E("; }")
+    else:
+        E("; only-plain {")
+        E(f"s_lshr_b32 s{S_T[4]}, s{S_H}, 1")
+        E(f"s_lshr_b32 s{S_T[5]}, s{S_W}, 1")
+        E(f"s_mul_i32 s{S_T[4]}, s{S_T[4]}, s{S_T[5]}")
+        E(f"s_mul_i32 s{S_T[4]}, s{S_T[4]}, s{S_LDPOOL}")
+        E(f"s_lshl_b32 s{S_T[4]}, s{S_T[4]}, 2")
+        E(f"s_mov_b32 s{S_POOLR + 2}, s{S_T[4]}")
+        E(f"s_mul_i32 s{S_T[6]}, s{S_IMG}, s{S_T[4]}")
+        E(f"s_mul_hi_u32 s{S_T[7]}, s{S_IMG}, s{S_T[4]}")
+        E(f"s_add_u32 s{S_POOLR}, s{S_POOL}, s{S_T[6]}")
+        E(f"s_addc_u32 s{S_POOLR + 1}, s{S_POOL + 1}, s{S_T[7]}")
+        E(f"s_and_b32 s{S_POOLR + 1}, s{S_POOLR + 1}, 0xffff")
+        E("; }")
     E(f"v_and_b32_e32 v{CQ}, 7, v{VTID}")
     E(f"v_lshrrev_b32_e32 v{VT}, 3, v{VTID}")
     E(f"v_lshlrev_b32_e32 v{e0}, 4, v{CQ}")
@@ -614,17 +703,46 @@
     E(f"v_and_b32_e32 v{e2}, 15, v{VT}")
     E(f"v_lshl_add_u32 v{e2}, v{e2}, 1, s{S_X0}")
     E(f"v_mad_u32_u24 v{e3}, v{e1}, s{S_W}, v{e2}")
+    if HEAD():
+        E("; only-head {")
+        E(f"v_mul_lo_u32 v{VLG}, v{e3}, s{S_NCLS4}")
+        E("; }")
     E(f"v_mul_lo_u32 v{e3}, v{e3}, s{S_LDOUT}")
     E(f"v_lshl_add_u32 v{e3}, v{CQ}, 2, v{e3}")
     E(f"v_lshlrev_b32_e32 v{VOUT}, 2, v{e3}")
     E(f"v_add_u32_e32 v{VOUT}, s{S_N64X4}, v{VOUT}")
-    E(f"v_lshrrev_b32_e32 v{e1}, 1, v{e1}")
-    E(f"v_lshrrev_b32_e32 v{e2}, 1, v{e2}")
-    E(f"v_mad_u32_u24 v{e3}, v{e1}, s{S_T[5]}, v{e2}")
-    E(f"v_mul_lo_u32 v{e3}, v{e3}, s{S_LDPOOL}")
-    E(f"v_lshl_add_u32 v{e3}, v{CQ}, 2, v{e3}")
-    E(f"v_lshlrev_b32_e32 v{VPOOL}, 2, v{e3}")
-    E(f"v_add_u32_e32 v{VPOOL}, s{S_N64X4}, v{VPOOL}")
+    if HEAD():
+        E("; only-head {")
+        E(f"v_mul_u32_u24_e32 v{VPS}, s{S_WNCLS4}, v{CQ}")
+        E(f"v_add_u32_e32 v{VLG}, v{VLG}, v{VPS}")
+        E(f"v_cmp_gt_u32_e32 vcc, 2, v{CQ}")
+        E(f"v_mov_b32_e32 v{VPS}, s{S_OOB}")
+        E("s_nop 1")
+        E(f"v_cndmask_b32_e32 v{VLG}, v{VPS}, v{VLG}, vcc")
+        E(f"v_lshrrev_b32_e32 v{e3}, 4, v{e1}")
+        E(f"v_lshrrev_b32_e32 v{VPS}, 4, v{e2}")
+        E(f"v_mad_u32_u24 v{e3}, v{e3}, s{S_NPW}, v{VPS}")
+        E(f"v_add_u32_e32 v{e3}, s{S_NODE0}, v{e3}")
+        E(f"v_bfe_u32 v{VPS}, v{e1}, 1, 3")
+        E(f"v_lshl_add_u32 v{e3}, v{e3}, 3, v{VPS}")
+        E(f"v_lshl_add_u32 v{e3}, v{e3}, 3, v{CQ}")
+        E(f"v_lshlrev_b32_e32 v{e3}, 4, v{e3}")
+        E(f"v_and_b32_e32 v{VPS}, 7, v{VT}")
+        E(f"v_cmp_eq_u32_e32 vcc, 0, v{VPS}")
+        E(f"v_mov_b32_e32 v{VPS}, s{S_OOB}")
+        E("s_nop 1")
+        E(f"v_cndmask_b32_e32 v{VPS}, v{VPS}, v{e3}, vcc")
+        E("; }")
+    else:
+        E("; only-plain {")
+        E(f"v_lshrrev_b32_e32 v{e1}, 1, v{e1}")
+        E(f"v_lshrrev_b32_e32 v{e2}, 1, v{e2}")
+        E(f"v_mad_u32_u24 v{e3}, v{e1}, s{S_T[5]}, v{e2}")
+        E(f"v_mul_lo_u32 v{e3}, v{e3}, s{S_LDPOOL}")
+        E(f"v_lshl_add_u32 v{e3}, v{CQ}, 2, v{e3}")
+        E(f"v_lshlrev_b32_e32 v{VPOOL}, 2, v{e3}")
+        E(f"v_add_u32_e32 v{VPOOL}, s{S_N64X4}, v{VPOOL}")
+        E("; }")
     E(f"s_lshl_b32 s{S_T[0]}, s{S_WI}, 13")
     if jp:
         E(f"s_add_u32 s{S_T[0]}, s{S_T[0]}, 0x{RAWB:x}")
@@ -684,18 +802,25 @@
     E(f"buffer_store_dwordx4 {vr(ya1, 4)}, v{VOUT}, s[{S_OUTR}:{S_OUTR + 3}], s{S_LD4} offen nt")
     E(f"buffer_store_dwordx4 {vr(yb0, 4)}, v{VOUT}, s[{S_OUTR}:{S_OUTR + 3}], s{S_SW4} offen nt")
     E(f"buffer_store_dwordx4 {vr(yb1, 4)}, v{VOUT}, s[{S_OUTR}:{S_OUTR + 3}], s{S_SUMOFF} offen nt")
-    lnp = newlabel("nopool")
-    E(f"s_cmp_eq_u64 s[{S_POOL}:{S_POOL + 1}], 0")
-    E(f"s_cbranch_scc1 {lnp}")
-    pm = Z(0, 0, 0)
-    for e in range(4):
-        E(f"v_max_f32_e32 v{pm + e}, v{ya0 + e}, v{yb0 + e}")
-    for e in range(4):
-        E(f"v_max_f32_e32 v{Z(0, 0, 1) + e}, v{ya1 + e}, v{yb1 + e}")
-    for e in range(4):
-        E(f"v_max_f32_e32 v{pm + e}, v{pm + e}, v{Z(0, 0, 1) + e}")
-    E(f"buffer_store_dwordx4 {vr(pm, 4)}, v{VPOOL}, s[{S_POOLR}:{S_POOLR + 3}], 0 offen")
-    L(lnp)
+    if HEAD():
+        E("; only-head {")
+        emit_head_math([ya0, ya1, yb0, yb1], Z(0, 0, 0), Z(0, 0, 1), CQ)
+        E("; }")
+    else:
+        E("; only-plain {")
+        lnp = newlabel("nopool")
+        E(f"s_cmp_eq_u64 s[{S_POOL}:{S_POOL + 1}], 0")
+        E(f"s_cbranch_scc1 {lnp}")
+        pm = Z(0, 0, 0)
+        for e in range(4):
+            E(f"v_max_f32_e32 v{pm + e}, v{ya0 + e}, v{yb0 + e}")
+        for e in range(4):
+            E(f"v_max_f32_e32 v{Z(0, 0, 1) + e}, v{ya1 + e}, v{yb1 + e}")
+        for e in range(4):
+            E(f"v_max_f32_e32 v{pm + e}, v{pm + e}, v{Z(0, 0, 1) + e}")
+        E(f"buffer_store_dwordx4 {vr(pm, 4)}, v{VPOOL}, s[{S_POOLR}:{S_POOLR + 3}], 0 offen")
+        L(lnp)
+        E("; }")
     E("s_waitcnt lgkmcnt(0)")
     E("s_barrier")
 
@@ -860,6 +985,10 @@
             setup_load()
             L(lsk)
             halo_loads(setn)
+        if HEAD():
+            E("; only-head {")
+            emit_head_prologue()
+            E("; }")
         E("s_waitcnt lgkmcnt(0)")
         E("s_barrier")
         return
@@ -891,6 +1020,49 @@
     E("s_barrier")
 
 
+def emit_head_prologue():
+    t = S_T
+    E(f"s_load_dwordx4 s[{t[0]}:{t[3]}], s[0:1], 0x78")
+    E(f"s_load_dwordx2 s[{S_LOGP}:{S_LOGP + 1}], s[0:1], 0x88")
+    E(f"s_load_dwordx2 s[{S_PSR}:{S_PSR + 1}], s[0:1], 0x90")
+    E(f"s_load_dword s{S_NCLS}, s[0:1], 0x98")
+    E(f"s_load_dword s{S_PSR + 2}, s[0:1], 0x9c")
+    E("s_waitcnt lgkmcnt(0)")
+    E(f"s_mov_b32 s{t[4]}, s{t[0]}")
+    E(f"s_and_b32 s{t[5]}, s{t[1]}, 0xffff")
+    E(f"s_lshl_b32 s{t[6]}, s{S_NCLS}, 7")
+    E(f"s_mov_b32 s{t[7]}, 0x00020000")
+    E(f"v_and_b32_e32 v1, 7, v{VTID}")
+    E("v_lshlrev_b32_e32 v2, 4, v1")
+    for k in range(4):
+        E(f"buffer_load_dwordx4 {vr(WQ(k, 0), 4)}, v2, s[{t[4]}:{t[7]}], 0 offen offset:{k * 128}")
+    E(f"s_mov_b32 s{t[4]}, s{t[2]}")
+    E(f"s_and_b32 s{t[5]}, s{t[3]}, 0xffff")
+    E(f"s_lshl_b32 s{t[6]}, s{S_NCLS}, 2")
+    E("v_cmp_eq_u32_e32 vcc, 0, v1")
+    E(f"v_mov_b32_e32 v2, s{S_OOB}")
+    E("v_mov_b32_e32 v3, 0")
+    E("s_nop 1")
+    E("v_cndmask_b32_e32 v2, v2, v3, vcc")
+    for k in range(4):
+        E(f"buffer_load_dword v{BL(k)}, v2, s[{t[4]}:{t[7]}], 0 offen offset:{k * 4}")
+    E(f"s_lshl_b32 s{S_NCLS4}, s{S_NCLS}, 2")
+    E(f"s_mul_i32 s{S_WNCLS4}, s{S_W}, s{S_NCLS4}")
+    E(f"s_mul_i32 s{S_LOGIMGB}, s{S_H}, s{S_WNCLS4}")
+    E(f"s_mov_b32 s{S_LGR + 2}, s{S_LOGIMGB}")
+    E(f"s_mov_b32 s{S_LGR + 3}, 0x00020000")
+    E(f"s_lshr_b32 s{S_NPW}, s{S_W}, 4")
+    E(f"s_lshr_b32 s{S_NPIMG}, s{S_H}, 4")
+    E(f"s_mul_i32 s{S_NPIMG}, s{S_NPIMG}, s{S_NPW}")
+    E(f"s_and_b32 s{S_PSR + 1}, s{S_PSR + 1}, 0xffff")
+    E(f"s_mov_b32 s{S_PSR + 3}, 0x00020000")
+    E(f"v_and_b32_e32 v1, 63, v{VTID}")
+    E("v_xor_b32_e32 v2, 16, v1")
+    E(f"v_lshlrev_b32_e32 v{VBP16}, 2, v2")
+    E("v_xor_b32_e32 v2, 32, v1")
+    E(f"v_lshlrev_b32_e32 v{VBP32}, 2, v2")
+
+
 def emit_first_form(jp):
     for r in raw_reads(jp, 0, 0, 0) + raw_reads(jp, 0, 0, 1):
         E(r)
@@ -931,7 +1103,7 @@
 \t.amdhsa_kernel {name}
 \t\t.amdhsa_group_segment_fixed_size 163840
 \t\t.amdhsa_private_segment_fixed_size 0
-\t\t.amdhsa_kernarg_size 120
+\t\t.amdhsa_kernarg_size {HEAD_KERNARG if HEAD() else 120}
 \t\t.amdhsa_user_sgpr_count 2
 \t\t.amdhsa_user_sgpr_dispatch_ptr 0
 \t\t.amdhsa_user_sgpr_queue_ptr 0
@@ -967,11 +1139,11 @@
     META.append(f"""  - .agpr_count:     0
     .args:
       - .offset:         0
-        .size:           120
+        .size:           {HEAD_KERNARG if HEAD() else 120}
         .value_kind:     by_value
     .group_segment_fixed_size: 163840
     .kernarg_segment_align: 8
-    .kernarg_segment_size: 120
+    .kernarg_segment_size: {HEAD_KERNARG if HEAD() else 120}
     .max_flat_workgroup_size: 512
     .name:           {name}
     .private_segment_fixed_size: 0
@@ -990,13 +1162,18 @@
 
 
 def main():
-    path = sys.argv[1]
+    head = sys.argv[1] == "--head"
+    path = sys.argv[2 if head else 1]
     out.append('\t.amdgcn_target "amdgcn-amd-amdhsa--gfx950"')
-    CFG.update(ntb=2, nc=None)
-    emit_kernel("mgu_wino_cp2_gfx950")
-    for nc in (2, 4):
-        CFG.update(ntb=1, nc=nc)
-        emit_kernel(f"mgu_wino_cp1r{nc}_gfx950")
+    if head:
+        CFG.update(ntb=1, nc=2, head=True)
+        emit_kernel("mgu_wino_cp1r2h_gfx950")
+    else:
+        CFG.update(ntb=2, nc=None)
+        emit_kernel("mgu_wino_cp2_gfx950")
+        for nc in (2, 4):
+            CFG.update(ntb=1, nc=nc)
+            emit_kernel(f"mgu_wino_cp1r{nc}_gfx950")
     out.append("\t.amdgpu_metadata\n---\namdhsa.kernels:")
     out.extend(META)
     out.append("""amdhsa.target:   amdgcn-amd-amdhsa--gfx950
diff --git a/mingraph-unet_amd/csrc/asm/lint_wino_asm.py b/mingraph-unet_amd/csrc/asm/lint_wino_asm.py
--- a/mingraph-unet_amd/csrc/asm/lint_wino_asm.py
+++ b/mingraph-unet_amd/csrc/asm/lint_wino_asm.py
@@ -30,6 +30,8 @@
         return regs(args[0]), regs(args[1]) | regs(args[2]) | regs(args[3]), "mfma"
     if op.startswith("ds_read"):
         return regs(args[0]), regs(args[1]), "lds_load"
+    if op.startswith("ds_bpermute") or op.startswith("ds_swizzle"):
+        return regs(args[0]), set().union(*[regs(a) for a in args[1:]]), "lds_load"
     if op.startswith("ds_write_addtid"):
         return set(), regs(args[0]), "lds_store_addtid"
     if op.startswith("ds_write"):
@@ -151,6 +153,10 @@
             for r in touched if kind in ("valu", "lds_store", "lds_store_addtid", "vm_store", "readlane") else src:
                 if r in src and mfma_age.get(r, 99) < 18:
                     errors.append(f"{where}: `{text}` reads MFMA result v{r} after {mfma_age[r]} wait states (18 required)")
+        if op.endswith("_dpp"):
+            for r in src:
+                if valu_age.get(r, 99) < 2:
+                    errors.append(f"{where}: `{text}` (DPP) reads v{r} {valu_age[r]} wait state(s) after a VALU write (2 required)")
         if kind == "valu" and prev and prev[0] in ("lds_store", "vm_store") and len(prev[1]) >= 4 and (dst & prev[1]):
             errors.append(f"{where}: `{text}` overwrites store data of the previous instruction `{prev[2]}`")
         if kind == "lds_store_addtid" and m0_fresh:
diff --git a/mingraph-unet_amd/csrc/common.h b/mingraph-unet_amd/csrc/common.h
--- a/mingraph-unet_amd/csrc/common.h
+++ b/mingraph-unet_amd/csrc/common.h
@@ -28,6 +28,7 @@
   bool wgrad_thin = true;
   bool wino_dgrad = true;
   bool gat_fused = true;
+  bool head_fused = true;
   bool wino_asm = true;
 };
 const Tuning& default_tuning();
@@ -63,19 +64,32 @@
   int ld2;
 };
 
+struct WinoHead {
+  const float* w;
+  const float* b;
+  float* logits;
+  float* psum;
+  int ncls;
+  int psum_bytes;
+};
+inline size_t wino_head_psum_bytes(int B, int H, int W) { return (size_t)B * (H / 16) * (W / 16) * 8 * 32 * sizeof(float); }
+
 inline const Tuning& tun(const IgemmDesc& d) { return d.tn ? *d.tn : default_tuning(); }
 enum class ConvKernel {
   None,
   WinoAsmWide, WinoAsmCp1r2, WinoAsmCp1r4,
+  WinoAsmCp1r2Head,
   WinoCp2, WinoCp1, WinoCp2Stats, WinoCp1Stats,
+  WinoCp1Head,
   WinoF32Wide, WinoF32Narrow,
   WinoX3Wide, WinoX3Narrow,
   HaloF32, HaloBf16Np8, HaloBf16Np4,
   TilesF32, TilesBf16,
   ConvtX3, ConvtBf16f, ConvtX3Dgrad,
 };
-ConvKernel pick_conv(const IgemmDesc& d, int dtype);
-hipError_t launch_conv(const IgemmDesc& d, ConvKernel k, int dtype, hipStream_t s);
+ConvKernel pick_conv(const IgemmDesc& d, int dtype, const WinoHead* head = nullptr);
+hipError_t launch_conv(const IgemmDesc& d, ConvKernel k, int dtype, hipStream_t s, const WinoHead* head = nullptr);
+inline bool conv_fuses_head(ConvKernel k) { return k == ConvKernel::WinoAsmCp1r2Head || k == ConvKernel::WinoCp1Head; }
 inline hipError_t launch_igemm_f32(const IgemmDesc& d, hipStream_t s) { return launch_conv(d, pick_conv(d, 0), 0, s); }
 inline hipError_t launch_igemm_bf16(const IgemmDesc& d, hipStream_t s) { return launch_conv(d, pick_conv(d, 1), 1, s); }
 const char* conv_kernel_name(ConvKernel k, const IgemmDesc& d);
@@ -97,6 +111,7 @@
 bool convt_x3_layer(const Tuning& t, int Cin, int Cout);
 bool convt_x3_dgrad_layer(const Tuning& t, int Cin, int Cout);
 bool convt_bf16f_layer(const Tuning& t, int Cin, int Cout);
+bool wino_head_layer(const Tuning& t, int dtype, int Cin, int ncls, int patch, int B, int H, int W);
 inline bool wino_wide(const IgemmDesc& d) { return d.N > 32; }
 struct WinoPlan {
   int tiles_x, tiles_y, total, nblk, ppb, ngroups, per_xcd;
@@ -144,8 +159,9 @@
 };
 bool wino_pack_batch_prepare(WinoPackBatch& b);
 hipError_t launch_pack_wino_w_multi(const WinoPackBatch* batch_dev, unsigned total_blocks, hipStream_t s);
-hipError_t launch_wino_f32(const IgemmDesc& d, ConvKernel k, hipStream_t s);
-hipError_t launch_wino_cp_asm(const IgemmDesc& d, ConvKernel k, hipStream_t s);
+hipError_t launch_wino_f32(const IgemmDesc& d, ConvKernel k, hipStream_t s, const WinoHead* head = nullptr);
+hipError_t launch_patch_sum_combine(const float* psum, float* out, int nodes, hipStream_t s);
+hipError_t launch_wino_cp_asm(const IgemmDesc& d, ConvKernel k, hipStream_t s, const WinoHead* head = nullptr);
 
 struct WgradDesc {
   const Tuning* tn;
diff --git a/mingraph-unet_amd/csrc/ctx.h b/mingraph-unet_amd/csrc/ctx.h
--- a/mingraph-unet_amd/csrc/ctx.h
+++ b/mingraph-unet_amd/csrc/ctx.h
@@ -66,6 +66,8 @@
   int last_stat_rows = 0;
   void* pm_out = nullptr;
   int pm_patch = 0;
+  void* pmws = nullptr;
+  size_t pmws_bytes = 0;
   void* wuws = nullptr;
   size_t wuws_bytes = 0;
   unsigned long long* gmaxbuf = nullptr;
@@ -262,7 +264,8 @@
 int run_layer(mgu_ctx* c, const Layer& L, const void* in, int ldin, int B, int H, int W, void* out, int ldout, int coff,
               int relu, const float* scale, const float* shift, int Hout, int Wout, hipStream_t s,
               void* pool = nullptr, int ldpool = 0, bool* pool_fused = nullptr,
-              double* stat_slots = nullptr, bool* stat_fused = nullptr);
+              double* stat_slots = nullptr, bool* stat_fused = nullptr,
+              const mgu::WinoHead* head = nullptr, bool* head_fused = nullptr);
 
 void gat_destroy(mgu_ctx* c);
 int gat_check_layer(mgu_ctx* c, const char* fn, int Fin, int heads, int Fh, bool train = false, int N = 0);
diff --git a/mingraph-unet_amd/csrc/igemm.hip b/mingraph-unet_amd/csrc/igemm.hip
--- a/mingraph-unet_amd/csrc/igemm.hip
+++ b/mingraph-unet_amd/csrc/igemm.hip
@@ -635,8 +635,7 @@
          (long)d.H * d.W * d.ldin < (1l << 31) && (long)d.H * d.W * d.ldout < (1l << 31);
 }
 
-static bool wino_asm_applicable(const IgemmDesc& d) {
-  if (!tun(d).wino_asm) return false;
+static bool wino_asm_shape(const IgemmDesc& d) {
   if (d.stat_slots) return false;
   if (wino_wide(d)) {
     if (d.N & 63) return false;
@@ -651,6 +650,20 @@
   return true;
 }
 
+static bool wino_asm_applicable(const IgemmDesc& d) { return tun(d).wino_asm && wino_asm_shape(d); }
+
+bool wino_head_layer(const Tuning& t, int dtype, int Cin, int ncls, int patch, int B, int H, int W) {
+  if (!t.head_fused || dtype != 0 || Cin != 32 || ncls < 1 || ncls > 4 || patch != 16 || B < 1 || (H & 15) || (W & 31)) return false;
+  return (long)H * W * ncls * 4 < 0x7fff0000l && wino_head_psum_bytes(B, H, W) < 0x7fff0000ul;
+}
+
+static bool wino_head_applicable(const IgemmDesc& d, const WinoHead& h) {
+  const int B = (int)(d.M / ((long)d.H * d.W));
+  if (!wino_head_layer(tun(d), 0, d.Cp, h.ncls, 16, B, d.H, d.W)) return false;
+  if (!wino_asm_shape(d) || wino_wide(d) || d.pool || d.ldout != 32 || d.coff) return false;
+  return h.w && h.b && h.logits && h.psum && (size_t)h.psum_bytes == wino_head_psum_bytes(B, d.H, d.W);
+}
+
 static bool convt_x3_applicable(const IgemmDesc& d) {
   return convt_x3_layer(tun(d), d.Cp, d.ct_cout) && d.wu && d.KS == 1 && d.K == d.Cp && d.N == 4 * d.ct_cout && (d.ldin & 3) == 0 &&
          !d.scale && !d.relu && !d.split_n && (9l * 128 + 8l * d.Wout) * d.ldout < (1l << 31);
@@ -667,7 +680,7 @@
          !d.relu && !d.split_n && !d.pool && (long)d.M * d.ldout < (1l << 31) && (long)d.Hout * d.Wout * d.ldin < (1l << 31);
 }
 
-ConvKernel pick_conv(const IgemmDesc& d, int dtype) {
+ConvKernel pick_conv(const IgemmDesc& d, int dtype, const WinoHead* head) {
   using K = ConvKernel;
   if (d.M <= 0 || d.N <= 0) return K::None;
   if (dtype == 1) {
@@ -684,6 +697,7 @@
     if (!t.wino_prec) return wide ? K::WinoF32Wide : K::WinoF32Narrow;
     if (!t.wino_cp || (long)d.H * d.W * d.ldin * 4 >= 0x7fff0000l) return wide ? K::WinoX3Wide : K::WinoX3Narrow;
     if (d.stat_slots) return wide ? K::WinoCp2Stats : K::WinoCp1Stats;
+    if (head && wino_head_applicable(d, *head)) return t.wino_asm ? K::WinoAsmCp1r2Head : K::WinoCp1Head;
     if (wino_asm_applicable(d)) return wide ? K::WinoAsmWide : d.Cp == 32 ? K::WinoAsmCp1r2 : K::WinoAsmCp1r4;
     return wide ? K::WinoCp2 : K::WinoCp1;
   }
@@ -696,6 +710,8 @@
     case ConvKernel::WinoAsmWide: return "mgu_wino_cp2_gfx950 (asm form of wino3x3_cp_kernel<2>)";
     case ConvKernel::WinoAsmCp1r2: return "mgu_wino_cp1r2_gfx950 (asm form of wino3x3_cp_kernel<1>)";
     case ConvKernel::WinoAsmCp1r4: return "mgu_wino_cp1r4_gfx950 (asm form of wino3x3_cp_kernel<1>)";
+    case ConvKernel::WinoAsmCp1r2Head: return "mgu_wino_cp1r2h_gfx950 (asm form of wino3x3_cp_kernel<1, head>: + 1x1 head + patch sums)";
+    case ConvKernel::WinoCp1Head: return "wino3x3_cp_kernel<1, head> (+ 1x1 head + patch sums)";
     case ConvKernel::WinoCp2: case ConvKernel::WinoCp2Stats: return "wino3x3_cp_kernel<2>";
     case ConvKernel::WinoCp1: case ConvKernel::WinoCp1Stats: return "wino3x3_cp_kernel<1>";
     case ConvKernel::WinoF32Wide: return "wino3x3_f32_kernel<0,0>";
@@ -717,6 +733,7 @@
   switch (k) {
     case ConvKernel::WinoAsmWide: case ConvKernel::WinoCp2: case ConvKernel::WinoCp2Stats: return "wino3x3_cp_kernel<2> (dgrad)";
     case ConvKernel::WinoAsmCp1r2: case ConvKernel::WinoAsmCp1r4: case ConvKernel::WinoCp1: case ConvKernel::WinoCp1Stats:
+    case ConvKernel::WinoAsmCp1r2Head: case ConvKernel::WinoCp1Head:
       return "wino3x3_cp_kernel<1> (dgrad)";
     case ConvKernel::WinoX3Wide: case ConvKernel::WinoX3Narrow: return "wino3x3_f32_kernel<*,1> (dgrad)";
     case ConvKernel::WinoF32Wide: case ConvKernel::WinoF32Narrow: return "wino3x3_f32_kernel<*,0> (dgrad)";
@@ -738,15 +755,18 @@
   }
 }
 
-hipError_t launch_conv(const IgemmDesc& d, ConvKernel k, int dtype, hipStream_t s) {
+hipError_t launch_conv(const IgemmDesc& d, ConvKernel k, int dtype, hipStream_t s, const WinoHead* head) {
   if (d.M <= 0 || d.N <= 0) return hipSuccess;
   if (dtype == 1) {
     if ((d.Cp & 7) || (d.ldin & 7) || (d.Kp % 64) || d.K > d.Kp || d.split_n) return hipErrorInvalidValue;
   } else {
     if ((d.Cp & 3) || (d.ldin & 3) || (d.Kp % 32) || d.K > d.Kp) return hipErrorInvalidValue;
   }
+  if (conv_fuses_head(k) != (head != nullptr)) return hipErrorInvalidValue;
   switch (k) {
     case ConvKernel::WinoAsmWide: case ConvKernel::WinoAsmCp1r2: case ConvKernel::WinoAsmCp1r4: return launch_wino_cp_asm(d, k, s);
+    case ConvKernel::WinoAsmCp1r2Head: return launch_wino_cp_asm(d, k, s, head);
+    case ConvKernel::WinoCp1Head: return launch_wino_f32(d, k, s, head);
     case ConvKernel::WinoCp2: case ConvKernel::WinoCp1: case ConvKernel::WinoCp2Stats: case ConvKernel::WinoCp1Stats:
     case ConvKernel::WinoF32Wide: case ConvKernel::WinoF32Narrow: case ConvKernel::WinoX3Wide: case ConvKernel::WinoX3Narrow:
       return launch_wino_f32(d, k, s);
diff --git a/mingraph-unet_amd/csrc/mgunet_api.hip b/mingraph-unet_amd/csrc/mgunet_api.hip
--- a/mingraph-unet_amd/csrc/mgunet_api.hip
+++ b/mingraph-unet_amd/csrc/mgunet_api.hip
@@ -95,6 +95,7 @@
   t.wino_dgrad = !flag("MGU_NO_WINO_DGRAD");
   t.gat_fused = !flag("MGU_NO_GAT_FUSED");
   t.wino_asm = num("MGU_WINO_ASM", 1) > 0;
+  t.head_fused = num("MGU_HEAD_FUSED", 1) > 0;
   *out = c;
   return MGU_OK;
 }
@@ -107,6 +108,7 @@
   if (c->arena) (void)hipFree(c->arena);
   if (c->ws) (void)hipFree(c->ws);
   if (c->gws) (void)hipFree(c->gws);
+  if (c->pmws) (void)hipFree(c->pmws);
   if (c->gbws) (void)hipFree(c->gbws);
   if (c->pack_dev) (void)hipFree(c->pack_dev);
   if (c->tws) (void)hipFree(c->tws);
@@ -370,8 +372,10 @@
 
 int mgud::run_layer(mgu_ctx* c, const Layer& L, const void* in_v, int ldin, int B, int H, int W, void* out_v, int ldout,
                     int coff, int relu, const float* scale, const float* shift, int Hout, int Wout, hipStream_t s,
-                    void* pool, int ldpool, bool* pool_fused, double* stat_slots, bool* stat_fused) {
+                    void* pool, int ldpool, bool* pool_fused, double* stat_slots, bool* stat_fused, const WinoHead* head,
+                    bool* head_fused) {
   IgemmDesc d = layer_desc(c, L, in_v, ldin, B, H, W, out_v, ldout, coff);
+  if (head_fused) *head_fused = false;
   d.scale = scale, d.shift = shift, d.relu = relu, d.Hout = Hout, d.Wout = Wout;
   if (pool_fused) *pool_fused = false;
   if (stat_fused) *stat_fused = false;
@@ -387,7 +391,7 @@
     HIPCHK(c, launch_first_conv(c->dtype, in_v, L.wf, scale, shift, out_v, B, H, W, L.Cin, L.Cout, ldout, coff, relu, s));
     return MGU_OK;
   }
-  ConvKernel k = pick_conv(d, c->dtype);
+  ConvKernel k = pick_conv(d, c->dtype, head);
   if (stat_slots && conv_is_wino(k) && wino_grid_blocks(d) <= STAT_ROWS) {
     d.stat_slots = stat_slots;
     c->last_stat_rows = wino_grid_blocks(d);
@@ -397,24 +401,27 @@
     d.pool = (float*)pool, d.ldpool = ldpool;
     if (pool_fused) *pool_fused = true;
   }
-  if (d.stat_slots || d.pool) k = pick_conv(d, c->dtype);
+  if (d.stat_slots || d.pool) k = pick_conv(d, c->dtype, head);
+  if (!conv_fuses_head(k)) head = nullptr;
+  else if (head_fused) *head_fused = true;
   if (L.wp_dirty && conv_reads_panel(k)) {
     if (L.convt) HIPCHK(c, launch_pack_convt_w(L.w_src, L.wp, c->dtype, L.Cin, L.Cout, L.Kp, s));
     else HIPCHK(c, launch_pack_conv_w(L.w_src, L.wp, c->dtype, L.Cout, L.Cin, L.Cp, L.KS, L.Kp, s));
     L.wp_dirty = false;
   }
-  const double alg = L.convt ? 2.0 * d.M * (double)L.Cin * L.Cout * 4.0 : 2.0 * d.M * (double)L.KS * L.KS * L.Cin * L.Cout;
+  double alg = L.convt ? 2.0 * d.M * (double)L.Cin * L.Cout * 4.0 : 2.0 * d.M * (double)L.KS * L.KS * L.Cin * L.Cout;
+  if (head) alg += 2.0 * d.M * (double)L.Cout * head->ncls;
   const ConvCost cost = conv_cost(k, d);
   ProfScope ps(c, s, conv_kernel_name(k, d), alg, cost.mfma, cost.pipe);
-  HIPCHK(c, launch_conv(d, k, c->dtype, s));
+  HIPCHK(c, launch_conv(d, k, c->dtype, s, head));
   return MGU_OK;
 }
 
 static int run_conv(mgu_ctx* c, const Layer& L, const void* in, int ldin, int B, int H, int W, void* out, int ldout,
                     int coff, int relu, int Hout, int Wout, hipStream_t s, void* pool = nullptr, int ldpool = 0,
-                    bool* pool_fused = nullptr) {
+                    bool* pool_fused = nullptr, const WinoHead* head = nullptr, bool* head_fused = nullptr) {
   return run_layer(c, L, in, ldin, B, H, W, out, ldout, coff, relu, L.bn.empty() ? nullptr : L.scale, L.shift, Hout, Wout, s,
-                   pool, ldpool, pool_fused, nullptr, nullptr);
+                   pool, ldpool, pool_fused, nullptr, nullptr, head, head_fused);
 }
 
 extern "C" {
@@ -438,6 +445,7 @@
   if (training) {
     int rc = unet_forward_train(c, (const float*)x_dev, xs_n, xs_c, xs_h, xs_w, B, H, W, (float*)logits_dev, cat_dev, feat_dev, s);
     if (rc == MGU_OK && c->pm_out) {
+      ProfScope ps(c, s, "patch_mean_kernel", 0, 0, -1);
       HIPCHK(c, launch_patch_mean(feat_dev[0], 0, (float*)c->pm_out, B, H, W, c->feat, c->pm_patch, s));
       c->pm_out = nullptr;
     }
@@ -446,6 +454,14 @@
   const WsPlan plan = plan_ws(c, B, H, W);
   int rc = ensure(c, &c->ws, &c->ws_bytes, plan.total);
   if (rc) return rc;
+  const Layer& F = c->layers[c->head];
+  WinoHead head_args{};
+  bool head_done = false;
+  const bool head_wanted = c->pm_out && F.w_src && F.b_src && wino_head_layer(c->tn, c->dtype, F.Cin, c->ncls, c->pm_patch, B, H, W);
+  if (head_wanted) {
+    if ((rc = ensure(c, &c->pmws, &c->pmws_bytes, wino_head_psum_bytes(B, H, W)))) return rc;
+    head_args = WinoHead{F.w_src, F.b_src, (float*)logits_dev, (float*)c->pmws, c->ncls, (int)wino_head_psum_bytes(B, H, W)};
+  }
   if (c->fold_dirty) {
     for (auto& L : c->layers)
       if (!L.bn.empty()) HIPCHK(c, launch_bn_fold(L.b_src, L.gamma, L.beta, L.run_mean, L.run_var, 1e-5f, L.scale, L.shift, L.Cout, s));
@@ -504,17 +520,23 @@
   }
   for (const Block& b : c->dec) {
     const int i = b.level, C = c->layers[b.conv1].Cout;
+    const bool last = head_wanted && i == 0;
     if ((rc = run_conv(c, c->layers[b.up], cur, cur_ld, B, hs[i + 1], wsz[i + 1], cat_dev[i], 2 * C, C, 0, hs[i], wsz[i], s)))
       return rc;
     if ((rc = run_conv(c, c->layers[b.conv1], cat_dev[i], 2 * C, B, hs[i], wsz[i], tmp, C, 0, 1, 0, 0, s))) return rc;
-    if ((rc = run_conv(c, c->layers[b.conv2], tmp, C, B, hs[i], wsz[i], feat_dev[i], C, 0, 1, 0, 0, s))) return rc;
+    if ((rc = run_conv(c, c->layers[b.conv2], tmp, C, B, hs[i], wsz[i], feat_dev[i], C, 0, 1, 0, 0, s, nullptr, 0, nullptr,
+                       last ? &head_args : nullptr, last ? &head_done : nullptr)))
+      return rc;
     cur = feat_dev[i];
     cur_ld = C;
   }
-  const Layer& F = c->layers[c->head];
   {
     const int pm_dtype = c->dtype;
-    if (c->pm_out && F.w_src && F.b_src && patch_mean_head_fusable(pm_dtype, F.Cin, c->ncls) && F.Cin <= 256) {
+    if (head_done) {
+      ProfScope ps(c, s, "patch_sum_combine_kernel", 0, 0, -1);
+      HIPCHK(c, launch_patch_sum_combine((const float*)c->pmws, (float*)c->pm_out, B * (H / 16) * (W / 16), s));
+      c->pm_out = nullptr;
+    } else if (c->pm_out && F.w_src && F.b_src && patch_mean_head_fusable(pm_dtype, F.Cin, c->ncls) && F.Cin <= 256) {
       ProfScope ps(c, s, "patch_mean_kernel (1x1 head + patch means)", 2.0 * B * H * W * F.Cin * c->ncls, 0, -1);
       HIPCHK(c, launch_patch_mean(cur, pm_dtype, (float*)c->pm_out, B, H, W, F.Cin, c->pm_patch, s, F.w_src, F.b_src,
                                   (float*)logits_dev, c->ncls));
@@ -528,6 +550,7 @@
     }
   }
   if (c->pm_out) {
+    ProfScope ps(c, s, "patch_mean_kernel", 0, 0, -1);
     HIPCHK(c, launch_patch_mean(cur, c->dtype, (float*)c->pm_out, B, H, W, F.Cin, c->pm_patch, s));
     c->pm_out = nullptr;
   }
diff --git a/mingraph-unet_amd/csrc/wino_asm.hip b/mingraph-unet_amd/csrc/wino_asm.hip
--- a/mingraph-unet_amd/csrc/wino_asm.hip
+++ b/mingraph-unet_amd/csrc/wino_asm.hip
@@ -1,8 +1,11 @@
 #include "common.h"
+#include <cstddef>
 #include <mutex>
 
 extern "C" const unsigned char mgu_wino_cp2_hsaco[];
 extern "C" const unsigned mgu_wino_cp2_hsaco_len;
+extern "C" const unsigned char mgu_wino_cp1r2h_hsaco[];
+extern "C" const unsigned mgu_wino_cp1r2h_hsaco_len;
 
 namespace mgu {
 
@@ -22,36 +25,48 @@
   unsigned mg_txty, pad;
 };
 static_assert(sizeof(WinoAsmArgs) == 120, "kernarg layout of mgu_wino_cp2_gfx950");
+struct WinoAsmHeadArgs {
+  WinoAsmArgs a;
+  const float* head_w;
+  const float* head_b;
+  float* logits;
+  float* psum;
+  int ncls, psum_bytes;
+};
+static_assert(sizeof(WinoAsmHeadArgs) == 160 && offsetof(WinoAsmHeadArgs, head_w) == 120, "kernarg layout of mgu_wino_cp1r2h_gfx950");
 
 unsigned magic(unsigned d) { return d <= 1 ? 0xffffffffu : (unsigned)((1ull << 32) / d); }
 
-const char* const kNames[3] = {"mgu_wino_cp2_gfx950", "mgu_wino_cp1r2_gfx950", "mgu_wino_cp1r4_gfx950"};
+const char* const kNames[4] = {"mgu_wino_cp2_gfx950", "mgu_wino_cp1r2_gfx950", "mgu_wino_cp1r4_gfx950", "mgu_wino_cp1r2h_gfx950"};
 std::mutex g_mu;
-hipModule_t g_mod[64] = {};
-hipFunction_t g_fn[64][3] = {};
+hipModule_t g_mod[64][2] = {};
+hipFunction_t g_fn[64][4] = {};
 }
 
-hipError_t launch_wino_cp_asm(const IgemmDesc& d, ConvKernel kind, hipStream_t s) {
+hipError_t launch_wino_cp_asm(const IgemmDesc& d, ConvKernel kind, hipStream_t s, const WinoHead* head) {
   int dev = 0;
   hipError_t e = hipGetDevice(&dev);
   if (e != hipSuccess) return e;
   if (dev < 0 || dev >= 64) return hipErrorInvalidDevice;
   hipFunction_t fn;
-  const int k = kind == ConvKernel::WinoAsmWide ? 0 : kind == ConvKernel::WinoAsmCp1r2 ? 1 : 2;
+  const int k = kind == ConvKernel::WinoAsmWide ? 0 : kind == ConvKernel::WinoAsmCp1r2 ? 1 : kind == ConvKernel::WinoAsmCp1r4 ? 2 : 3;
+  if ((k == 3) != (head != nullptr)) return hipErrorInvalidValue;
+  const int m = k == 3 ? 1 : 0;
   {
     std::lock_guard<std::mutex> lk(g_mu);
-    if (!g_mod[dev]) {
-      e = hipModuleLoadData(&g_mod[dev], mgu_wino_cp2_hsaco);
+    if (!g_mod[dev][m]) {
+      e = hipModuleLoadData(&g_mod[dev][m], m ? mgu_wino_cp1r2h_hsaco : mgu_wino_cp2_hsaco);
       if (e != hipSuccess) return e;
     }
     if (!g_fn[dev][k]) {
-      e = hipModuleGetFunction(&g_fn[dev][k], g_mod[dev], kNames[k]);
+      e = hipModuleGetFunction(&g_fn[dev][k], g_mod[dev][m], kNames[k]);
       if (e != hipSuccess) return e;
     }
     fn = g_fn[dev][k];
   }
   const WinoPlan p = wino_plan(d);
-  WinoAsmArgs a;
+  WinoAsmHeadArgs ha;
+  WinoAsmArgs& a = ha.a;
   a.in = d.in, a.wu = d.wu, a.out = d.out + d.coff, a.scale = d.scale, a.shift = d.shift, a.pool = d.pool;
   a.H = d.H, a.W = d.W, a.ldin = d.ldin, a.ldout = d.ldout;
   a.ldpool = d.pool ? d.ldpool : 0, a.nC = d.Cp >> 4, a.relu = d.relu, a.tiles_x = p.tiles_x;
@@ -60,7 +75,12 @@
   a.mg_ngroups = magic((unsigned)p.ngroups), a.mg_tx = magic((unsigned)p.tiles_x);
   a.mg_txty = magic((unsigned)(p.tiles_x * p.tiles_y)), a.pad = 0;
   size_t sz = sizeof(a);
-  void* extra[] = {HIP_LAUNCH_PARAM_BUFFER_POINTER, &a, HIP_LAUNCH_PARAM_BUFFER_SIZE, &sz, HIP_LAUNCH_PARAM_END};
+  if (head) {
+    ha.head_w = head->w, ha.head_b = head->b, ha.logits = head->logits, ha.psum = head->psum;
+    ha.ncls = head->ncls, ha.psum_bytes = head->psum_bytes;
+    sz = sizeof(ha);
+  }
+  void* extra[] = {HIP_LAUNCH_PARAM_BUFFER_POINTER, &ha, HIP_LAUNCH_PARAM_BUFFER_SIZE, &sz, HIP_LAUNCH_PARAM_END};
   return hipModuleLaunchKernel(fn, (unsigned)(8 * p.per_xcd), 1, 1, 512, 1, 1, 0, s, nullptr, extra);
 }
 
diff --git a/mingraph-unet_amd/csrc/wino_f32.hip b/mingraph-unet_amd/csrc/wino_f32.hip
--- a/mingraph-unet_amd/csrc/wino_f32.hip
+++ b/mingraph-unet_amd/csrc/wino_f32.hip
@@ -641,9 +641,14 @@
 
 constexpr int WINO_CP_RAWF = 8192;
 
-template <int NTB, bool STATS, bool DEEP, bool URES = false>
+__device__ inline WinoHead wino_head_of() { return WinoHead{}; }
+__device__ inline WinoHead wino_head_of(const WinoHead& h) { return h; }
+template <int NTB, bool STATS, bool DEEP, bool URES = false, typename... HD>
 __global__ __launch_bounds__(512) void wino3x3_cp_kernel(const IgemmDesc d, const int tiles_x, const int tiles_y, const int total_patches,
-                        const int patches_per_block, const int ngroups, const int nitems, const int per_xcd) {
+                        const int patches_per_block, const int ngroups, const int nitems, const int per_xcd, const HD... hd_args) {
+  constexpr bool HEAD = sizeof...(HD) == 1;
+  const WinoHead hd = wino_head_of(hd_args...);
+  static_assert(!HEAD || (NTB == 1 && !STATS && URES), "the head-fused finishing pass belongs to the 2-chunk narrow inference kernel");
   constexpr int NWAVES = 8;
   constexpr int MT = 2;
   constexpr int NC = 32 * NTB;
@@ -1012,6 +1017,44 @@
               }
           }
       }
+      if constexpr (HEAD) {
+        const f32x4 Y[4] = {ya[0], ya[1], yb[0], yb[1]};
+        float lg[4][4];
+#pragma unroll
+        for (int k = 0; k < 4; ++k) {
+          if (k >= hd.ncls) break;
+          const f32x4 wq = *reinterpret_cast<const f32x4*>(hd.w + k * 32 + cq * 4);
+          const float bl = cq == 0 ? hd.b[k] : 0.f;
+#pragma unroll
+          for (int p = 0; p < 4; ++p) {
+            float ds = __builtin_fmaf(Y[p][0], wq[0], bl);
+            ds = __builtin_fmaf(Y[p][1], wq[1], ds);
+            ds = __builtin_fmaf(Y[p][2], wq[2], ds);
+            ds = __builtin_fmaf(Y[p][3], wq[3], ds);
+            ds += __shfl_xor(ds, 1);
+            ds += __shfl_xor(ds, 2);
+            ds += __shfl_xor(ds, 4);
+            lg[k][p] = ds;
+          }
+        }
+        if (cq < 2) {
+          float* lp = hd.logits + ((size_t)(img * d.H + oy + cq) * d.W + ox) * hd.ncls;
+#pragma unroll
+          for (int pp = 0; pp < 2; ++pp)
+#pragma unroll
+            for (int k = 0; k < 4; ++k)
+              if (k < hd.ncls) lp[pp * hd.ncls + k] = cq ? lg[k][2 + pp] : lg[k][pp];
+        }
+        f32x4 ps = (Y[0] + Y[1]) + (Y[2] + Y[3]);
+#pragma unroll
+        for (int o = 8; o < 64; o <<= 1)
+#pragma unroll
+          for (int e = 0; e < 4; ++e) ps[e] += __shfl_xor(ps[e], o);
+        if ((T & 7) == 0) {
+          const int node = (img * (d.H >> 4) + (oy >> 4)) * (d.W >> 4) + (ox >> 4);
+          *reinterpret_cast<f32x4*>(hd.psum + ((size_t)(node * 8 + ((oy >> 1) & 7)) * 32 + cq * 4)) = ps;
+        }
+      }
       if (d.pool) {
         f32x4 m;
 #pragma unroll
@@ -1072,18 +1115,44 @@
 
 int wino_grid_blocks(const IgemmDesc& d) { return 8 * wino_plan(d).per_xcd; }
 
-template <int NTB, bool STATS, bool DEEP = false, bool URES = false>
-static hipError_t launch_wino_cp(const IgemmDesc& d, hipStream_t s) {
+__global__ __launch_bounds__(256) void patch_sum_combine_kernel(const float* __restrict__ psum, float* __restrict__ out, const int n) {
+  const int i = blockIdx.x * 256 + threadIdx.x;
+  if (i >= n) return;
+  const float* p = psum + (size_t)(i >> 5) * 256 + (i & 31);
+  float sum = p[0];
+#pragma unroll
+  for (int r = 1; r < 8; ++r) sum += p[r * 32];
+  out[i] = sum / 256.f;
+}
+
+hipError_t launch_patch_sum_combine(const float* psum, float* out, int nodes, hipStream_t s) {
+  const int n = nodes * 32;
+  if (n <= 0) return hipSuccess;
+  hipLaunchKernelGGL(patch_sum_combine_kernel, dim3((n + 255) / 256), dim3(256), 0, s, psum, out, n);
+  return hipGetLastError();
+}
+
+template <int NTB, bool STATS, bool DEEP = false, bool URES = false, bool HEAD = false>
+static hipError_t launch_wino_cp(const IgemmDesc& d, hipStream_t s, const WinoHead* head = nullptr) {
+  static_assert(!HEAD || (NTB == 1 && !STATS && DEEP && URES), "the head-fused entry point is the 2-chunk narrow inference kernel");
   constexpr int NWAVES = 8;
   const WinoPlan p = wino_plan(d);
   dim3 grid(8 * p.per_xcd, 1);
   if (d.stat_slots && grid.x > (unsigned)STAT_ROWS) return hipErrorInvalidValue;
   const size_t lds = (size_t)(5 * WINO_CP_RAWF) * sizeof(float);
   static bool attr_done[64] = {};
-  hipError_t ae = ensure_dyn_lds(reinterpret_cast<const void*>(&wino3x3_cp_kernel<NTB, STATS, DEEP, URES>), lds, attr_done);
-  if (ae != hipSuccess) return ae;
-  hipLaunchKernelGGL((wino3x3_cp_kernel<NTB, STATS, DEEP, URES>), grid, dim3(64 * NWAVES), lds, s, d, p.tiles_x, p.tiles_y, p.total,
-                     p.ppb, p.ngroups, p.ngroups * p.nblk, p.per_xcd);
+  if (HEAD != (head != nullptr)) return hipErrorInvalidValue;
+  if constexpr (HEAD) {
+    hipError_t ae = ensure_dyn_lds(reinterpret_cast<const void*>(&wino3x3_cp_kernel<NTB, STATS, DEEP, URES, WinoHead>), lds, attr_done);
+    if (ae != hipSuccess) return ae;
+    hipLaunchKernelGGL((wino3x3_cp_kernel<NTB, STATS, DEEP, URES, WinoHead>), grid, dim3(64 * NWAVES), lds, s, d, p.tiles_x, p.tiles_y,
+                       p.total, p.ppb, p.ngroups, p.ngroups * p.nblk, p.per_xcd, *head);
+  } else {
+    hipError_t ae = ensure_dyn_lds(reinterpret_cast<const void*>(&wino3x3_cp_kernel<NTB, STATS, DEEP, URES>), lds, attr_done);
+    if (ae != hipSuccess) return ae;
+    hipLaunchKernelGGL((wino3x3_cp_kernel<NTB, STATS, DEEP, URES>), grid, dim3(64 * NWAVES), lds, s, d, p.tiles_x, p.tiles_y, p.total,
+                       p.ppb, p.ngroups, p.ngroups * p.nblk, p.per_xcd);
+  }
   return hipGetLastError();
 }
 
@@ -1104,8 +1173,9 @@
   return hipGetLastError();
 }
 
-hipError_t launch_wino_f32(const IgemmDesc& d, ConvKernel k, hipStream_t s) {
+hipError_t launch_wino_f32(const IgemmDesc& d, ConvKernel k, hipStream_t s, const WinoHead* head) {
   switch (k) {
+    case ConvKernel::WinoCp1Head: return launch_wino_cp<1, false, true, true, true>(d, s, head);
     case ConvKernel::WinoCp2Stats: return launch_wino_cp<2, true>(d, s);
     case ConvKernel::WinoCp1Stats: return launch_wino_cp<1, true>(d, s);
     case ConvKernel::WinoCp2: return launch_wino_cp<2, false>(d, s);
```

Measured after the change: 804.3, median of 6. 1.02x the previous value.
